# tiborcamargo/KinectPy

Measured on AMD Instinct MI355X. Metric: Mpoints/sec end-to-end (unproject+filter+ICP), 4-sensor frame, higher is better.
Workload: dtype f64 decisions / f32 storage

## Files before the change

### include/kinectpx.h

```cpp
#ifndef KINECTPX_H
#define KINECTPX_H

#include <stddef.h>
#include <stdint.h>

#ifdef __cplusplus
extern "C" {
#endif

#define KPX_VERSION 100

typedef enum {
    KPX_OK = 0,
    KPX_ERR_INVALID = -1,
    KPX_ERR_WORKSPACE = -2,
    KPX_ERR_RANGE = -3,
    KPX_ERR_HIP = -4,
    KPX_RETRY = 1
} kpx_status;

const char *kpx_last_error(void);
int kpx_version(void);


int kpx_unproject_u16(const uint16_t *depth, const float *xy_table, int64_t n_px, int32_t frames,
                      int16_t *xyz, void *stream);

size_t kpx_median_workspace_bytes(int32_t frames);
int kpx_median_i16(const int16_t *v, int64_t n, int64_t stride, int32_t frames, double *d_median,
                   void *ws, size_t ws_bytes, void *stream);

#define KPX_COMPACT_COLOR_MASK 1
#define KPX_COMPACT_DEPTH_GATE 2
size_t kpx_compact_workspace_bytes(int64_t n, int32_t frames);
int kpx_rgbd_compact(const int16_t *xyz, const uint8_t *rgb, int64_t n, int32_t frames, int32_t flags,
                     const double *d_median, double gate, float *pts, float *col, int32_t *idx,
                     int32_t *d_count, void *ws, size_t ws_bytes, void *stream);

size_t kpx_depth_to_cloud_workspace_bytes(int64_t n_px, int32_t frames);
int kpx_depth_to_cloud(const uint16_t *depth, const float *xy_table, const uint8_t *rgb, int64_t n_px,
                       int32_t frames, int32_t flags, double gate, float *pts, float *col, int32_t *idx,
                       int32_t *d_count, void *ws, size_t ws_bytes, void *stream);


int kpx_transform(const float *pts, int64_t n, const double *h_T, float *out, void *stream);
int kpx_rotate(const float *nrm, int64_t n, const double *h_T, float *out, void *stream);
int kpx_joints_affine_f64(const double *x, int64_t rows, const double *h_A, const double *h_t, double *out,
                          void *stream);

#define KPX_SELECT_GATHER 0
#define KPX_SELECT_INVERT 1
#define KPX_SELECT_MASK 2
size_t kpx_select_workspace_bytes(int64_t n);
int kpx_select_by_index(const float *a0, const float *a1, const float *a2, int64_t n, const int32_t *idx,
                        int64_t n_idx, int32_t invert, float *o0, float *o1, float *o2, int32_t *d_count,
                        void *ws, size_t ws_bytes, void *stream);

int kpx_select_by_index_bounds(const float *a0, const float *a1, const float *a2, int64_t n, const int32_t *idx, int64_t n_idx,
                               float *o0, float *o1, float *o2, double *d_bbox6, void *ws, size_t ws_bytes, void *stream);
size_t kpx_bounds_workspace_bytes(void);
int kpx_bounds(const float *pts, int64_t n, double *d_bbox6, void *ws, size_t ws_bytes, void *stream);

size_t kpx_sort_pairs_u32_workspace_bytes(int64_t n);
int kpx_sort_pairs_u32(const uint32_t *keys_in, const int32_t *vals_in, int64_t n, int32_t end_bit, uint32_t *keys_out,
                       int32_t *vals_out, void *ws, size_t ws_bytes, void *stream);

int kpx_halfspace_select(const float *pts, int64_t n, const double *h_plane, int32_t *idx, int32_t *d_count,
                         void *ws, size_t ws_bytes, void *stream);
int kpx_slab_split(const float *pts, int64_t n, double slab, int32_t *lower_idx, int32_t *d_lower,
                   int32_t *upper_idx, int32_t *d_upper, void *ws, size_t ws_bytes, void *stream);
int kpx_slab_split_bounded(const float *pts, int64_t n, double slab, const double *d_bbox6, int32_t *lower_idx, int32_t *d_lower,
                           int32_t *upper_idx, int32_t *d_upper, void *ws, size_t ws_bytes, void *stream);


size_t kpx_voxel_workspace_bytes(int64_t n);
int kpx_voxel_downsample(const float *pts, const float *col, const float *nrm, int64_t n, double voxel,
                         float *opts, float *ocol, float *onrm, int32_t *d_count, void *ws, size_t ws_bytes,
                         void *stream);

size_t kpx_voxel_batch_workspace_bytes(int32_t count, const int64_t *h_n);
int kpx_voxel_downsample_batch(int32_t count, const float *const *h_pts, const float *const *h_col, const int64_t *h_n,
                               double voxel, float *const *h_opts, float *const *h_ocol, int32_t *d_counts, void *ws,
                               size_t ws_bytes, void *stream);

size_t kpx_fuse_voxel_workspace_bytes(int64_t total_points);
int kpx_fuse_voxel_downsample(int32_t count, const float *const *h_pts, const float *const *h_col, const int64_t *h_n,
                              const double *h_T, double voxel, float *opts, float *ocol, int32_t *d_count, void *ws,
                              size_t ws_bytes, void *stream);

#define KPX_SOR_MAX_K 4096
#define KPX_SOR_LDS_K 288
size_t kpx_sor_workspace_bytes(int64_t n, int32_t nb_neighbors);
int kpx_sor(const float *pts, int64_t n, int32_t nb_neighbors, double std_ratio, int32_t *keep_idx,
            int32_t *d_count, double *d_stats, double *d_avg, void *ws, size_t ws_bytes, void *stream);

int kpx_sor_select(const float *pts, const float *attr, int64_t n, int32_t nb_neighbors, double std_ratio, float *out_pts,
                   float *out_attr, int32_t *keep_idx, int32_t *d_count, double *d_stats, void *ws, size_t ws_bytes, void *stream);

int kpx_sor_partial(const float *pts, int64_t n, int32_t nb_neighbors, int64_t q_begin, int64_t q_end, double *d_avg_sorted,
                    int32_t *d_order, void *ws, size_t ws_bytes, void *stream);
size_t kpx_sor_finish_workspace_bytes(int64_t n);
int kpx_sor_finish(const double *d_avg_sorted, const int32_t *d_order, int64_t n, double std_ratio, int32_t *keep_idx,
                   int32_t *d_count, double *d_stats, double *d_avg, void *ws, size_t ws_bytes, void *stream);

size_t kpx_dbscan_workspace_bytes(int64_t n);
int kpx_cluster_dbscan(const float *pts, int64_t n, double eps, int32_t min_points, int32_t *labels ,
                       int32_t *d_nclusters, void *ws, size_t ws_bytes, void *stream);

size_t kpx_radius_outlier_workspace_bytes(int64_t n);
int kpx_remove_radius_outlier(const float *pts, int64_t n, int32_t nb_points, double radius, int32_t *keep_idx,
                              int32_t *d_count, void *ws, size_t ws_bytes, void *stream);

size_t kpx_iss_workspace_bytes(int64_t n);
int kpx_iss_saliency(const float *pts, int64_t n, double salient_radius, double gamma_21, double gamma_32, int32_t min_neighbors,
                     double *saliency , void *ws, size_t ws_bytes, void *stream);
int kpx_iss_nonmax(const float *pts, int64_t n, const double *saliency , double non_max_radius, int32_t min_neighbors,
                   int32_t *keep_idx, int32_t *d_count, void *ws, size_t ws_bytes, void *stream);
int kpx_iss_keypoints(const float *pts, int64_t n, double salient_radius, double non_max_radius, double gamma_21, double gamma_32,
                      int32_t min_neighbors, double *saliency , int32_t *keep_idx, int32_t *d_count, void *ws, size_t ws_bytes,
                      void *stream);
int kpx_mean_nn_distance(const double *d2, const int32_t *count, int64_t m, int32_t stride, double *d_mean, void *ws, size_t ws_bytes,
                         void *stream);

#define KPX_FPS_BLOCK_THREADS 1024
#define KPX_FPS_REG_N 12288
#define KPX_FPS_LDS_N 19456
#define KPX_FPS_BLOCK_MAX_N 24576
#define KPX_FPS_BATCH_BLOCK_MAX_N 65536
#define KPX_FPS_BATCH_MIN_CLOUDS 4
size_t kpx_fps_workspace_bytes(int32_t count, int64_t n_max);
int kpx_farthest_point_sample(const float *pts, int64_t n, int32_t k, int32_t start_index, int32_t *sel ,
                              double *cover , void *ws, size_t ws_bytes, void *stream);
int kpx_farthest_point_sample_batch(int32_t count, const float *const *h_pts, const int64_t *h_n, int32_t k, int32_t start_index,
                                    int32_t *const *h_sel, double *const *h_cover, void *ws, size_t ws_bytes, void *stream);

#define KPX_NORMALS_MAX_NN 4096
#define KPX_NORMALS_LDS_NN 128
size_t kpx_normals_workspace_bytes(int64_t n, int32_t max_nn);
int kpx_estimate_normals(const float *pts, int64_t n, double radius, int32_t max_nn, float *normals,
                         void *ws, size_t ws_bytes, void *stream);
size_t kpx_covariances_workspace_bytes(int64_t n, int32_t max_nn);
int kpx_estimate_covariances(const float *pts, int64_t n, double radius, int32_t max_nn, double *cov,
                             void *ws, size_t ws_bytes, void *stream);

size_t kpx_search_index_bytes(int64_t n);
int kpx_search_index_build(const float *pts, int64_t n, void *index, size_t index_bytes, void *ws, size_t ws_bytes, void *stream);
size_t kpx_search_workspace_bytes(int64_t m, int32_t k);
int kpx_search_knn(const void *index, size_t index_bytes, const float *queries, int64_t m, int32_t k, double radius, int32_t *idx ,
                   double *d2 , int32_t *count , void *ws, size_t ws_bytes, void *stream);
int kpx_search_radius_count(const void *index, size_t index_bytes, const float *queries, int64_t m, double radius, int64_t *offsets ,
                            void *ws, size_t ws_bytes, void *stream);
int kpx_search_radius_fill(const void *index, size_t index_bytes, const float *queries, int64_t m, double radius, const int64_t *offsets,
                           int64_t total, int32_t *idx , double *d2 , void *ws, size_t ws_bytes, void *stream);

size_t kpx_segment_plane_workspace_bytes(int64_t n, int32_t ransac_n, int32_t num_iterations);
int kpx_segment_plane(const float *pts, int64_t n, double distance_threshold, int32_t ransac_n,
                      int32_t num_iterations, double probability, uint64_t seed, double *d_plane,
                      int32_t *inlier_idx, int32_t *d_count, void *ws, size_t ws_bytes, void *stream);


size_t kpx_nn_workspace_bytes(int64_t n_src, int64_t n_tgt);
int kpx_nn_search(const float *src, int64_t n_src, const float *tgt, int64_t n_tgt, const double *d_T,
                  int32_t *idx, double *d2, void *ws, size_t ws_bytes, void *stream);

size_t kpx_registration_eval_workspace_bytes(int64_t n_src, int64_t n_tgt);
int kpx_registration_eval(const float *src, int64_t n_src, const float *tgt, int64_t n_tgt, const double *d_T,
                          double max_dist, double *d_result, int32_t *idx, double *d2, void *ws, size_t ws_bytes,
                          void *stream);

size_t kpx_kabsch_workspace_bytes(int64_t n_corr);
int kpx_kabsch(const float *src, const float *tgt, const int32_t *corr, int64_t n_corr, double *d_T, void *ws,
               size_t ws_bytes, void *stream);

#define KPX_ICP_POINT_TO_POINT 0
#define KPX_ICP_POINT_TO_PLANE 1
#define KPX_ICP_FIXED 2
size_t kpx_icp_workspace_bytes(int64_t n_src, int64_t n_tgt);
int kpx_icp(const float *src, int64_t n_src, const float *tgt, const float *tgt_normals, int64_t n_tgt,
            double max_dist, const double *h_init, int32_t mode, int32_t max_iteration, double relative_fitness,
            double relative_rmse, int32_t poll_interval, double *d_result, int32_t *idx, double *d2, void *ws,
            size_t ws_bytes, void *stream);


size_t kpx_fpfh_workspace_bytes(int64_t n, int32_t max_nn);
int kpx_fpfh(const float *pts, const float *normals, int64_t n, double radius, int32_t max_nn, double *fpfh, void *ws,
             size_t ws_bytes, void *stream);

size_t kpx_feature_nn_workspace_bytes(int64_t na, int64_t nb);
int kpx_feature_nn(const double *fa, int64_t na, const double *fb, int64_t nb, int32_t *idx, void *ws, size_t ws_bytes,
                   void *stream);

size_t kpx_ransac_workspace_bytes(int64_t n_src, int64_t n_tgt);
int kpx_ransac_corres(const float *src, int64_t n_src, const float *tgt, int64_t n_tgt, const int32_t *corres, int64_t n_corres,
                      double max_dist, int32_t ransac_n, double edge_similarity, int32_t max_iteration, double confidence,
                      uint64_t seed, double *h_result, void *ws, size_t ws_bytes, void *stream);

size_t kpx_fgr_workspace_bytes(int64_t n_corres);
int kpx_fgr_tuple_test(const float *src, int64_t n_src, const float *tgt, int64_t n_tgt, const int32_t *corres, int64_t n_corres,
                       double tuple_scale, int32_t maximum_tuple_count, uint64_t seed, int32_t *d_pairs, int32_t *d_count,
                       void *ws, size_t ws_bytes, void *stream);
int kpx_fgr_optimize(const float *src, int64_t n_src, const float *tgt, int64_t n_tgt, const int32_t *corres, int64_t n_corres,
                     double division_factor, int32_t use_absolute_scale, int32_t decrease_mu, double maximum_correspondence_distance,
                     int32_t iteration_number, double *h_result, void *ws, size_t ws_bytes, void *stream);

size_t kpx_icp_batch_workspace_bytes(int32_t count, const int64_t *h_n_src, int64_t n_tgt);
int kpx_icp_batch(int32_t count, const float *const *h_src, const int64_t *h_n_src, const float *tgt,
                  const float *tgt_normals, int64_t n_tgt, double max_dist, const double *h_init, int32_t mode,
                  int32_t max_iteration, double relative_fitness, double relative_rmse, double *d_results, void *ws,
                  size_t ws_bytes, void *stream);

#define KPX_NN_ENGINE_CULLED 0
#define KPX_NN_ENGINE_DENSE 1
#define KPX_NN_ENGINE_DENSE_FP64 2
int kpx_nn_engine(int32_t engine);

size_t kpx_sample_workspace_bytes(int64_t n);
int kpx_sample_points(const float *pts, int64_t n, int64_t k, uint64_t seed, float *out_pts, int32_t *out_idx, void *ws,
                      size_t ws_bytes, void *stream);

size_t kpx_obb_workspace_bytes(int32_t count, int64_t n);
int kpx_obb_batch(const void *pts, int32_t pts_f64, int32_t count, int64_t n, double *d_obb, uint8_t *d_is_vertex, void *ws,
                  size_t ws_bytes, void *stream);

#define KPX_NORM_OBB 0
#define KPX_NORM_OBB_ROT_TRANS 1
#define KPX_NORM_TRANSLATE 2
#define KPX_NORM_OBB_ROT 3
int kpx_normalize_batch(const double *x, int32_t count, int64_t rows, const double *d_obb, int32_t mode, const double *h_M,
                        double *out, void *stream);

size_t kpx_color_gradient_workspace_bytes(int64_t n, int32_t max_nn);
int kpx_color_gradient(const float *pts, const float *normals, const float *colors, int64_t n, double radius, int32_t max_nn,
                       double *grad, void *ws, size_t ws_bytes, void *stream);
size_t kpx_colored_icp_workspace_bytes(int64_t n_src, int64_t n_tgt);
int kpx_colored_icp(const float *src, const float *src_colors, int64_t n_src, const float *tgt, const float *tgt_colors,
                    const float *tgt_normals, const double *tgt_gradient, int64_t n_tgt, double max_dist, const double *h_init,
                    double lambda_geometric, int32_t max_iteration, double relative_fitness, double relative_rmse,
                    int32_t poll_interval, double *d_result, void *ws, size_t ws_bytes, void *stream);

int kpx_gicp_covariances(const float *normals, int64_t n, double epsilon, double *cov, void *stream);
int kpx_rotate_covariances(const double *cov, int64_t n, const double *h_T, double *out, void *stream);
size_t kpx_generalized_icp_workspace_bytes(int64_t n_src, int64_t n_tgt);
int kpx_generalized_icp(const float *src, const double *src_cov, int64_t n_src, const float *tgt, const double *tgt_cov, int64_t n_tgt,
                        double max_dist, const double *h_init, int32_t max_iteration, double relative_fitness, double relative_rmse,
                        int32_t poll_interval, double *d_result, int32_t *idx, double *d2, void *ws, size_t ws_bytes, void *stream);

#define KPX_LOSS_L2 0
#define KPX_LOSS_L1 1
#define KPX_LOSS_HUBER 2
#define KPX_LOSS_CAUCHY 3
#define KPX_LOSS_GM 4
#define KPX_LOSS_TUKEY 5
int kpx_icp_robust(const float *src, int64_t n_src, const float *tgt, const float *tgt_normals, int64_t n_tgt,
                   double max_dist, const double *h_init, int32_t mode, int32_t max_iteration, double relative_fitness,
                   double relative_rmse, int32_t poll_interval, double *d_result, int32_t *idx, double *d2, void *ws,
                   size_t ws_bytes, void *stream, int32_t loss, double loss_k);
int kpx_colored_icp_robust(const float *src, const float *src_colors, int64_t n_src, const float *tgt, const float *tgt_colors,
                           const float *tgt_normals, const double *tgt_gradient, int64_t n_tgt, double max_dist, const double *h_init,
                           double lambda_geometric, int32_t max_iteration, double relative_fitness, double relative_rmse,
                           int32_t poll_interval, double *d_result, void *ws, size_t ws_bytes, void *stream, int32_t loss,
                           double loss_k);
int kpx_generalized_icp_robust(const float *src, const double *src_cov, int64_t n_src, const float *tgt, const double *tgt_cov,
                               int64_t n_tgt, double max_dist, const double *h_init, int32_t max_iteration, double relative_fitness,
                               double relative_rmse, int32_t poll_interval, double *d_result, int32_t *idx, double *d2, void *ws,
                               size_t ws_bytes, void *stream, int32_t loss, double loss_k);

int kpx_fuse_skeletons(const double *skeletons, int32_t cams, int64_t frames, int32_t joints, double alpha, double beta,
                       int32_t initial_frame, double *out, void *stream);

typedef struct {
    double reg_voxel;
    double icp_max_dist;
    double filt_voxel;
    double filt_ratio;
    double gate;
    int32_t normals_nn;
    int32_t icp_mode;
    int32_t icp_max_iteration;
    int32_t filt_k;
} kpx_frame_params;
size_t kpx_frame_step_workspace_bytes(int32_t sensors, int64_t n_px);
int kpx_frame_step(const uint16_t *depth, const uint8_t *rgb, const float *xy_table, int64_t n_px, int32_t sensors,
                   const double *h_init, const kpx_frame_params *params, float *out_pts, float *out_col, int32_t *h_count,
                   double *h_T, int32_t *h_info, void *ws, size_t ws_bytes, void *stream);
size_t kpx_frame_step_host_workspace_bytes(int32_t sensors, int64_t n_px);
int kpx_frame_step_host(const uint16_t *h_depth, const uint8_t *h_rgb, const float *xy_table, int64_t n_px, int32_t sensors,
                        const double *h_init, const kpx_frame_params *params, float *out_pts, float *out_col, int32_t *h_count,
                        double *h_T, int32_t *h_info, void *ws, size_t ws_bytes, void *stream);

typedef struct kpx_comm kpx_comm;
typedef int (*kpx_bcast_fn)(void *user, void *d_buf, size_t bytes, int32_t root, void *stream);
typedef int (*kpx_allgather_fn)(void *user, const void *d_send, void *d_recv, size_t bytes_per_rank, void *stream);
int kpx_rccl_load(const char *path);
int kpx_rccl_unique_id(void *id128);
int kpx_comm_create_rccl(const void *id128, int32_t rank, int32_t world, kpx_comm **out);
int kpx_comm_create_callbacks(int32_t rank, int32_t world, kpx_bcast_fn bcast, kpx_allgather_fn allgather, void *user, kpx_comm **out);
int kpx_comm_create_replay(int32_t rank, int32_t world, int32_t frames, int32_t first_frame, int32_t stride, int32_t per_frame,
                           const void *const *d_payloads, const size_t *bytes, kpx_comm **out);
int kpx_comm_destroy(kpx_comm *comm);
int kpx_comm_rank(const kpx_comm *comm);
int kpx_comm_world(const kpx_comm *comm);
int kpx_comm_broadcast(kpx_comm *comm, void *d_buf, size_t bytes, int32_t root, void *stream);
int kpx_comm_allgather(kpx_comm *comm, const void *d_send, void *d_recv, size_t bytes_per_rank, void *stream);
int kpx_copy_bytes(void *dst, const void *src, size_t bytes, void *stream, int32_t wait);

typedef struct kpx_order kpx_order;
int kpx_order_create(int32_t depth, kpx_order **out);
int kpx_order_destroy(kpx_order *order);
int kpx_order_submit(kpx_order *order, int64_t *frame);
int kpx_order_block(kpx_order *order, int64_t frame);
int kpx_order_turn_begin(kpx_order *order, int64_t frame, int32_t stage);
int kpx_order_turn_end(kpx_order *order, int64_t frame, int32_t stage);
int kpx_order_skip(kpx_order *order, int64_t frame, int32_t stage);
int kpx_order_finish(kpx_order *order, int64_t frame);
int kpx_order_log(kpx_order *order, int64_t *out, int64_t cap, int64_t *count);

size_t kpx_frame_step_sharded_workspace_bytes(int32_t sensors, int32_t rank, int32_t world, int64_t n_px, int32_t host_input);
int kpx_frame_step_sharded(kpx_comm *comm, kpx_order *order, int64_t frame, const uint16_t *depth, const uint8_t *rgb, int32_t host_input,
                           const float *xy_table, int64_t n_px, int32_t sensors, const double *h_init, const kpx_frame_params *params,
                           int32_t fused_filter, float *out_pts, float *out_col, int32_t *h_count, double *h_T, int32_t *h_info, void *ws,
                           size_t ws_bytes, void *stream);

typedef struct kpx_stream kpx_stream;
size_t kpx_stream_workspace_bytes(int32_t sensors, int32_t rank, int32_t world, int64_t n_px, int32_t depth);
int kpx_stream_create(const float *xy_table, int64_t n_px, int32_t sensors, const double *h_init, const kpx_frame_params *params,
                      int32_t depth, kpx_comm *const *comms, int32_t fused_filter, void *ws, size_t ws_bytes, kpx_stream **out);
int kpx_stream_submit(kpx_stream *stream, const void *depth, const void *rgb, int32_t host_input, float *out_pts, float *out_col);
int kpx_stream_pop(kpx_stream *stream, int32_t *h_count, double *h_T, int32_t *h_info);
int kpx_stream_pending(const kpx_stream *stream);
int kpx_stream_capacity(const kpx_stream *stream);
int kpx_stream_destroy(kpx_stream *stream);
int kpx_stream_stats(const kpx_stream *stream, uint64_t *h_out4);

int kpx_host_resources(uint64_t *h_out4);

#define KPX_PROF_NN_MFMA 0
#define KPX_PROF_SOR_KNN 1
#define KPX_PROF_PLANE_SCORE 2
#define KPX_PROF_COMPACT 3
#define KPX_PROF_NN_SCREEN 4
#define KPX_PROF_NN_LOCAL 5
#define KPX_PROF_KERNELS 6
int kpx_prof_begin(int32_t capacity);
int kpx_prof_stride(int32_t stride);
int kpx_prof_end(double *h_ms, int64_t *h_launches, double *h_work);
int kpx_prof_icp_phases(double *h_out8);
int kpx_prof_icp_waves(uint64_t *h_out, int64_t cap_waves, int64_t *h_count);
int kpx_icp_chain(int32_t on);
int kpx_prof_icp_cert(uint64_t *h_out8);
int kpx_prof_icp_chain(uint64_t *h_out3072);

#define KPX_TSDF_MAX_RESOLUTION 1024
#define KPX_TSDF_MAX_SENSORS 8
#define KPX_TSDF_COUNT_BLOCK 512
#define KPX_TSDF_SURFACE 0
#define KPX_TSDF_VOXELS 1
size_t kpx_tsdf_workspace_bytes(int32_t resolution);
int kpx_tsdf_integrate(float *volume, float *color, int32_t resolution, double voxel_length, const double *h_origin, double sdf_trunc,
                       int32_t count, const void *const *h_depth, int32_t depth_u16, double depth_scale, double depth_trunc,
                       const uint8_t *const *h_rgb, int32_t width, int32_t height, const double *h_intrinsic, const double *h_extrinsics,
                       void *stream);
int kpx_tsdf_extract_count(const float *volume, int32_t resolution, int32_t mode, int64_t *d_count, void *ws, size_t ws_bytes, void *stream);
int kpx_tsdf_extract_fill(const float *volume, const float *color, int32_t resolution, double voxel_length, const double *h_origin,
                          int32_t mode, int64_t total, float *pts, float *nrm, float *col, void *ws, size_t ws_bytes, void *stream);

#define KPX_TSDF_BLOCKS_MAX_RESOLUTION 32
size_t kpx_tsdf_blocks_touch_workspace_bytes(int32_t count, int32_t width, int32_t height, int32_t stride, double unit_length, double sdf_trunc);
int kpx_tsdf_blocks_touch(const int64_t *index_keys, const int32_t *index_slots, int64_t n_blocks, int32_t count, const void *const *h_depth,
                          int32_t depth_u16, double depth_scale, double depth_trunc, int32_t width, int32_t height, const double *h_intrinsic,
                          const double *h_poses, int32_t stride, double unit_length, double sdf_trunc, int64_t *d_counts, void *ws,
                          size_t ws_bytes, void *stream);
int kpx_tsdf_blocks_insert(const int64_t *index_keys, const int32_t *index_slots, int64_t n_blocks, int64_t n_new, int64_t *out_keys,
                           int32_t *out_slots, float *pool, float *color_pool, int64_t capacity, int32_t unit_resolution, int32_t count,
                           int32_t width, int32_t height, int32_t stride, double unit_length, double sdf_trunc, const void *ws, size_t ws_bytes,
                           void *stream);
int kpx_tsdf_blocks_integrate(float *pool, float *color_pool, int64_t capacity, int32_t unit_resolution, double voxel_length, double sdf_trunc,
                              int64_t n_touched, int32_t count, const void *const *h_depth, int32_t depth_u16, double depth_scale,
                              double depth_trunc, const uint8_t *const *h_rgb, int32_t width, int32_t height, const double *h_intrinsic,
                              const double *h_extrinsics, int32_t stride, const void *ws, size_t ws_bytes, void *stream);
size_t kpx_tsdf_blocks_extract_workspace_bytes(int64_t n_blocks, int32_t unit_resolution, int32_t mesh);
int kpx_tsdf_blocks_extract_count(const int64_t *index_keys, const int32_t *index_slots, int64_t n_blocks, const float *pool,
                                  int32_t unit_resolution, int32_t mode, int64_t *d_count, void *ws, size_t ws_bytes, void *stream);
int kpx_tsdf_blocks_extract_fill(const int64_t *index_keys, const int32_t *index_slots, int64_t n_blocks, const float *pool,
                                 const float *color_pool, int32_t unit_resolution, double voxel_length, int32_t mode, int64_t total, float *pts,
                                 float *nrm, float *col, void *ws, size_t ws_bytes, void *stream);
int kpx_tsdf_blocks_mesh_count(const int64_t *index_keys, const int32_t *index_slots, int64_t n_blocks, const float *pool,
                               int32_t unit_resolution, int64_t *d_counts, void *ws, size_t ws_bytes, void *stream);
int kpx_tsdf_blocks_mesh_fill(const int64_t *index_keys, const int32_t *index_slots, int64_t n_blocks, const float *pool,
                              const float *color_pool, int32_t unit_resolution, double voxel_length, int64_t n_vertices, int64_t n_triangles,
                              float *out_vertices, float *out_colors, int32_t *out_triangles, void *ws, size_t ws_bytes, void *stream);

size_t kpx_tsdf_mesh_workspace_bytes(int32_t resolution);
int kpx_tsdf_mesh_count(const float *volume, int32_t resolution, int64_t *d_counts, void *ws, size_t ws_bytes, void *stream);
int kpx_tsdf_mesh_fill(const float *volume, const float *color, int32_t resolution, double voxel_length, const double *h_origin,
                       int64_t n_vertices, int64_t n_triangles, float *out_vertices, float *out_colors, int32_t *out_triangles, void *ws,
                       size_t ws_bytes, void *stream);
size_t kpx_mesh_normals_workspace_bytes(int64_t n_vertices, int64_t n_triangles);
int kpx_mesh_normals(const float *vertices, int64_t n_vertices, const int32_t *triangles, int64_t n_triangles, int32_t normalized,
                     float *out_triangle_normals, float *out_vertex_normals, void *ws, size_t ws_bytes, void *stream);
int kpx_mesh_surface_area(const float *vertices, int64_t n_vertices, const int32_t *triangles, int64_t n_triangles, double *d_area, void *stream);

#define KPX_MESH_FLAG_REFERENCED 0
#define KPX_MESH_FLAG_DEGENERATE 1
#define KPX_MESH_FLAG_INDICES 2
#define KPX_MESH_SMOOTH_SIMPLE 0
#define KPX_MESH_SMOOTH_LAPLACIAN 1
#define KPX_MESH_SMOOTH_TAUBIN 2
size_t kpx_mesh_adjacency_workspace_bytes(int64_t n_vertices, int64_t n_triangles);
int kpx_mesh_adjacency(const int32_t *triangles, int64_t n_vertices, int64_t n_triangles, int32_t *out_offsets, int32_t *out_neighbours,
                       int32_t *d_count, void *ws, size_t ws_bytes, void *stream);
size_t kpx_mesh_edges_workspace_bytes(int64_t n_vertices, int64_t n_triangles);
int kpx_mesh_non_manifold_edges(const int32_t *triangles, int64_t n_vertices, int64_t n_triangles, int32_t allow_boundary_edges,
                                int32_t *out_edges, int32_t *d_count, void *ws, size_t ws_bytes, void *stream);
size_t kpx_mesh_cluster_workspace_bytes(int64_t n_vertices, int64_t n_triangles);
int kpx_mesh_cluster_triangles(const float *vertices, int64_t n_vertices, const int32_t *triangles, int64_t n_triangles, int32_t *out_clusters,
                               int32_t *out_n_triangles, double *out_area, int32_t *d_count, void *ws, size_t ws_bytes, void *stream);
int kpx_mesh_flags(int32_t kind, const int32_t *triangles, int64_t n_vertices, int64_t n_triangles, const int64_t *indices, int64_t n_indices,
                   uint8_t *out_flags, int64_t n_flags, void *stream);
size_t kpx_mesh_select_workspace_bytes(int64_t n_vertices, int64_t n_triangles);
int kpx_mesh_select_triangles(const int32_t *triangles, const float *triangle_normals, int64_t n_triangles, const uint8_t *flags, int32_t invert,
                              int32_t *out_triangles, float *out_triangle_normals, int32_t *d_count, void *ws, size_t ws_bytes, void *stream);
int kpx_mesh_select_vertices(const float *vertices, const float *colors, const float *normals, int64_t n_vertices, const int32_t *triangles,
                             const float *triangle_normals, int64_t n_triangles, const uint8_t *flags, int32_t invert, float *out_vertices,
                             float *out_colors, float *out_normals, int32_t *out_triangles, float *out_triangle_normals, int32_t *d_counts, void *ws,
                             size_t ws_bytes, void *stream);
size_t kpx_mesh_smooth_workspace_bytes(int64_t n_vertices);
int kpx_mesh_smooth(const float *vertices, const float *normals, const float *colors, int64_t n_vertices, const int32_t *offsets,
                    const int32_t *neighbours, int64_t n_neighbours, int32_t method, int32_t iterations, double lambda_filter, double mu,
                    float *out_vertices, float *out_normals, float *out_colors, void *ws, size_t ws_bytes, void *stream);
size_t kpx_mesh_sample_workspace_bytes(int64_t n_triangles);
int kpx_mesh_sample_points(const float *vertices, const float *colors, const float *vertex_normals, const float *triangle_normals,
                           int64_t n_vertices, const int32_t *triangles, int64_t n_triangles, int64_t n_points, uint64_t seed, float *out_points,
                           float *out_colors, float *out_normals, double *d_total, void *ws, size_t ws_bytes, void *stream);

#define KPX_RAYSCENE_LEAF 4
#define KPX_RAYSCENE_FANOUT 4
#define KPX_RAY_CAST 0
#define KPX_RAY_OCCLUDED 1
#define KPX_RAY_COUNT 2
size_t kpx_rayscene_bytes(int64_t n_triangles);
size_t kpx_rayscene_workspace_bytes(int64_t n_triangles);
int kpx_rayscene_build(const float *vertices, int64_t n_vertices, const int32_t *triangles, int64_t n_triangles, const int32_t *triangle_ids,
                       void *scene, size_t scene_bytes, void *ws, size_t ws_bytes, void *stream);
int kpx_rayscene_rays(const void *scene, size_t scene_bytes, const float *rays, int64_t m, int32_t mode, double tnear, double tfar, int32_t brute,
                      double *out_t, float *out_t_hit, float *out_uvs, float *out_normals, int32_t *out_geometry_ids, int32_t *out_primitive_ids,
                      int32_t *out_count, void *stream);
// ... 126 lines not shown
```

### kinectpy_amd/_lib.py

```python
import ctypes as C
import threading
import weakref
import os

import torch

_HERE = os.path.dirname(os.path.abspath(__file__))
SO_PATH = os.environ.get("KPX_LIBRARY") or os.path.join(_HERE, "libkinectpx.so")

_i64, _i32, _f64, _u64, _vp, _sz = C.c_int64, C.c_int32, C.c_double, C.c_uint64, C.c_void_p, C.c_size_t

SIGNATURES = {
    "kpx_last_error": (C.c_char_p, []),
    "kpx_version": (C.c_int, []),
    "kpx_unproject_u16": (C.c_int, [_vp, _vp, _i64, _i32, _vp, _vp]),
    "kpx_median_workspace_bytes": (_sz, [_i32]),
    "kpx_median_i16": (C.c_int, [_vp, _i64, _i64, _i32, _vp, _vp, _sz, _vp]),
    "kpx_compact_workspace_bytes": (_sz, [_i64, _i32]),
    "kpx_rgbd_compact": (C.c_int, [_vp, _vp, _i64, _i32, _i32, _vp, _f64, _vp, _vp, _vp, _vp, _vp, _sz, _vp]),
    "kpx_depth_to_cloud_workspace_bytes": (_sz, [_i64, _i32]),
    "kpx_depth_to_cloud": (C.c_int, [_vp, _vp, _vp, _i64, _i32, _i32, _f64, _vp, _vp, _vp, _vp, _vp, _sz, _vp]),
    "kpx_transform": (C.c_int, [_vp, _i64, _vp, _vp, _vp]),
    "kpx_rotate": (C.c_int, [_vp, _i64, _vp, _vp, _vp]),
    "kpx_joints_affine_f64": (C.c_int, [_vp, _i64, _vp, _vp, _vp, _vp]),
    "kpx_select_workspace_bytes": (_sz, [_i64]),
    "kpx_select_by_index": (C.c_int, [_vp, _vp, _vp, _i64, _vp, _i64, _i32, _vp, _vp, _vp, _vp, _vp, _sz, _vp]),
    "kpx_halfspace_select": (C.c_int, [_vp, _i64, _vp, _vp, _vp, _vp, _sz, _vp]),
    "kpx_slab_split": (C.c_int, [_vp, _i64, _f64, _vp, _vp, _vp, _vp, _vp, _sz, _vp]),
    "kpx_slab_split_bounded": (C.c_int, [_vp, _i64, _f64, _vp, _vp, _vp, _vp, _vp, _vp, _sz, _vp]),
    "kpx_select_by_index_bounds": (C.c_int, [_vp, _vp, _vp, _i64, _vp, _i64, _vp, _vp, _vp, _vp, _vp, _sz, _vp]),
    "kpx_bounds_workspace_bytes": (C.c_size_t, []),
    "kpx_bounds": (C.c_int, [_vp, _i64, _vp, _vp, _sz, _vp]),
    "kpx_voxel_workspace_bytes": (_sz, [_i64]),
    "kpx_voxel_downsample": (C.c_int, [_vp, _vp, _vp, _i64, _f64, _vp, _vp, _vp, _vp, _vp, _sz, _vp]),
    "kpx_voxel_batch_workspace_bytes": (_sz, [_i32, _vp]),
    "kpx_voxel_downsample_batch": (C.c_int, [_i32, _vp, _vp, _vp, _f64, _vp, _vp, _vp, _vp, _sz, _vp]),
    "kpx_fuse_voxel_workspace_bytes": (_sz, [_i64]),
    "kpx_fuse_voxel_downsample": (C.c_int, [_i32, _vp, _vp, _vp, _vp, _f64, _vp, _vp, _vp, _vp, _sz, _vp]),
    "kpx_sor_workspace_bytes": (_sz, [_i64, _i32]),
    "kpx_sor": (C.c_int, [_vp, _i64, _i32, _f64, _vp, _vp, _vp, _vp, _vp, _sz, _vp]),
    "kpx_sor_partial": (C.c_int, [_vp, _i64, _i32, _i64, _i64, _vp, _vp, _vp, _sz, _vp]),
    "kpx_sor_finish_workspace_bytes": (_sz, [_i64]),
    "kpx_sor_finish": (C.c_int, [_vp, _vp, _i64, _f64, _vp, _vp, _vp, _vp, _vp, _sz, _vp]),
    "kpx_dbscan_workspace_bytes": (_sz, [_i64]),
    "kpx_cluster_dbscan": (C.c_int, [_vp, _i64, _f64, _i32, _vp, _vp, _vp, _sz, _vp]),
    "kpx_radius_outlier_workspace_bytes": (_sz, [_i64]),
    "kpx_remove_radius_outlier": (C.c_int, [_vp, _i64, _i32, _f64, _vp, _vp, _vp, _sz, _vp]),
    "kpx_iss_workspace_bytes": (_sz, [_i64]),
    "kpx_iss_saliency": (C.c_int, [_vp, _i64, _f64, _f64, _f64, _i32, _vp, _vp, _sz, _vp]),
    "kpx_iss_nonmax": (C.c_int, [_vp, _i64, _vp, _f64, _i32, _vp, _vp, _vp, _sz, _vp]),
    "kpx_iss_keypoints": (C.c_int, [_vp, _i64, _f64, _f64, _f64, _f64, _i32, _vp, _vp, _vp, _vp, _sz, _vp]),
    "kpx_mean_nn_distance": (C.c_int, [_vp, _vp, _i64, _i32, _vp, _vp, _sz, _vp]),
    "kpx_fps_workspace_bytes": (_sz, [_i32, _i64]),
    "kpx_farthest_point_sample": (C.c_int, [_vp, _i64, _i32, _i32, _vp, _vp, _vp, _sz, _vp]),
    "kpx_farthest_point_sample_batch": (C.c_int, [_i32, _vp, _vp, _i32, _i32, _vp, _vp, _vp, _sz, _vp]),
    "kpx_normals_workspace_bytes": (_sz, [_i64, _i32]),
    "kpx_estimate_normals": (C.c_int, [_vp, _i64, _f64, _i32, _vp, _vp, _sz, _vp]),
    "kpx_search_index_bytes": (_sz, [_i64]),
    "kpx_search_index_build": (C.c_int, [_vp, _i64, _vp, _sz, _vp, _sz, _vp]),
    "kpx_search_workspace_bytes": (_sz, [_i64, _i32]),
    "kpx_search_knn": (C.c_int, [_vp, _sz, _vp, _i64, _i32, _f64, _vp, _vp, _vp, _vp, _sz, _vp]),
    "kpx_search_radius_count": (C.c_int, [_vp, _sz, _vp, _i64, _f64, _vp, _vp, _sz, _vp]),
    "kpx_search_radius_fill": (C.c_int, [_vp, _sz, _vp, _i64, _f64, _vp, _i64, _vp, _vp, _vp, _sz, _vp]),
    "kpx_segment_plane_workspace_bytes": (_sz, [_i64, _i32, _i32]),
    "kpx_segment_plane": (C.c_int, [_vp, _i64, _f64, _i32, _i32, _f64, _u64, _vp, _vp, _vp, _vp, _sz, _vp]),
    "kpx_nn_workspace_bytes": (_sz, [_i64, _i64]),
    "kpx_nn_search": (C.c_int, [_vp, _i64, _vp, _i64, _vp, _vp, _vp, _vp, _sz, _vp]),
    "kpx_registration_eval_workspace_bytes": (_sz, [_i64, _i64]),
    "kpx_registration_eval": (C.c_int, [_vp, _i64, _vp, _i64, _vp, _f64, _vp, _vp, _vp, _vp, _sz, _vp]),
    "kpx_kabsch_workspace_bytes": (_sz, [_i64]),
    "kpx_kabsch": (C.c_int, [_vp, _vp, _vp, _i64, _vp, _vp, _sz, _vp]),
    "kpx_icp_workspace_bytes": (_sz, [_i64, _i64]),
    "kpx_icp": (C.c_int, [_vp, _i64, _vp, _vp, _i64, _f64, _vp, _i32, _i32, _f64, _f64, _i32, _vp, _vp, _vp, _vp, _sz, _vp]),
    "kpx_fpfh_workspace_bytes": (_sz, [_i64, _i32]),
    "kpx_fpfh": (C.c_int, [_vp, _vp, _i64, _f64, _i32, _vp, _vp, _sz, _vp]),
    "kpx_feature_nn_workspace_bytes": (_sz, [_i64, _i64]),
    "kpx_feature_nn": (C.c_int, [_vp, _i64, _vp, _i64, _vp, _vp, _sz, _vp]),
    "kpx_ransac_workspace_bytes": (_sz, [_i64, _i64]),
    "kpx_ransac_corres": (C.c_int, [_vp, _i64, _vp, _i64, _vp, _i64, _f64, _i32, _f64, _i32, _f64, _u64, _vp, _vp, _sz, _vp]),
    "kpx_fgr_workspace_bytes": (_sz, [_i64]),
    "kpx_fgr_tuple_test": (C.c_int, [_vp, _i64, _vp, _i64, _vp, _i64, _f64, _i32, _u64, _vp, _vp, _vp, _sz, _vp]),
    "kpx_fgr_optimize": (C.c_int, [_vp, _i64, _vp, _i64, _vp, _i64, _f64, _i32, _i32, _f64, _i32, _vp, _vp, _sz, _vp]),
    "kpx_sample_workspace_bytes": (_sz, [_i64]),
    "kpx_sample_points": (C.c_int, [_vp, _i64, _i64, _u64, _vp, _vp, _vp, _sz, _vp]),
    "kpx_obb_workspace_bytes": (_sz, [_i32, _i64]),
    "kpx_obb_batch": (C.c_int, [_vp, _i32, _i32, _i64, _vp, _vp, _vp, _sz, _vp]),
    "kpx_normalize_batch": (C.c_int, [_vp, _i32, _i64, _vp, _i32, _vp, _vp, _vp]),
    "kpx_color_gradient_workspace_bytes": (_sz, [_i64, _i32]),
    "kpx_color_gradient": (C.c_int, [_vp, _vp, _vp, _i64, _f64, _i32, _vp, _vp, _sz, _vp]),
    "kpx_colored_icp_workspace_bytes": (_sz, [_i64, _i64]),
    "kpx_colored_icp": (C.c_int, [_vp, _vp, _i64, _vp, _vp, _vp, _vp, _i64, _f64, _vp, _f64, _i32, _f64, _f64, _i32, _vp, _vp, _sz, _vp]),
    "kpx_covariances_workspace_bytes": (_sz, [_i64, _i32]),
    "kpx_estimate_covariances": (C.c_int, [_vp, _i64, _f64, _i32, _vp, _vp, _sz, _vp]),
    "kpx_gicp_covariances": (C.c_int, [_vp, _i64, _f64, _vp, _vp]),
    "kpx_rotate_covariances": (C.c_int, [_vp, _i64, _vp, _vp, _vp]),
    "kpx_generalized_icp_workspace_bytes": (_sz, [_i64, _i64]),
    "kpx_generalized_icp": (C.c_int, [_vp, _vp, _i64, _vp, _vp, _i64, _f64, _vp, _i32, _f64, _f64, _i32, _vp, _vp, _vp, _vp, _sz, _vp]),
    "kpx_icp_robust": (C.c_int, [_vp, _i64, _vp, _vp, _i64, _f64, _vp, _i32, _i32, _f64, _f64, _i32, _vp, _vp, _vp, _vp, _sz, _vp, _i32, _f64]),
    "kpx_colored_icp_robust": (C.c_int, [_vp, _vp, _i64, _vp, _vp, _vp, _vp, _i64, _f64, _vp, _f64, _i32, _f64, _f64, _i32, _vp, _vp, _sz, _vp,
                                         _i32, _f64]),
    "kpx_generalized_icp_robust": (C.c_int, [_vp, _vp, _i64, _vp, _vp, _i64, _f64, _vp, _i32, _f64, _f64, _i32, _vp, _vp, _vp, _vp, _sz, _vp,
                                             _i32, _f64]),
    "kpx_fuse_skeletons": (C.c_int, [_vp, _i32, _i64, _i32, _f64, _f64, _i32, _vp, _vp]),
    "kpx_nn_engine": (C.c_int, [_i32]),
    "kpx_icp_batch_workspace_bytes": (_sz, [_i32, _vp, _i64]),
    "kpx_icp_batch": (C.c_int, [_i32, _vp, _vp, _vp, _vp, _i64, _f64, _vp, _i32, _i32, _f64, _f64, _vp, _vp, _sz, _vp]),
    "kpx_prof_begin": (C.c_int, [_i32]),
    "kpx_prof_stride": (C.c_int, [_i32]),
    "kpx_frame_step_workspace_bytes": (_sz, [_i32, _i64]),
    "kpx_frame_step": (C.c_int, [_vp, _vp, _vp, _i64, _i32, _vp, _vp, _vp, _vp, _vp, _vp, _vp, _vp, _sz, _vp]),
    "kpx_frame_step_host_workspace_bytes": (_sz, [_i32, _i64]),
    "kpx_frame_step_host": (C.c_int, [_vp, _vp, _vp, _i64, _i32, _vp, _vp, _vp, _vp, _vp, _vp, _vp, _vp, _sz, _vp]),
    "kpx_rccl_load": (C.c_int, [_vp]),
    "kpx_rccl_unique_id": (C.c_int, [_vp]),
    "kpx_comm_create_rccl": (C.c_int, [_vp, _i32, _i32, _vp]),
    "kpx_comm_create_callbacks": (C.c_int, [_i32, _i32, _vp, _vp, _vp, _vp]),
    "kpx_comm_create_replay": (C.c_int, [_i32, _i32, _i32, _i32, _i32, _i32, _vp, _vp, _vp]),
    "kpx_comm_destroy": (C.c_int, [_vp]),
    "kpx_comm_rank": (C.c_int, [_vp]),
    "kpx_comm_world": (C.c_int, [_vp]),
    "kpx_comm_broadcast": (C.c_int, [_vp, _vp, _sz, _i32, _vp]),
    "kpx_comm_allgather": (C.c_int, [_vp, _vp, _vp, _sz, _vp]),
    "kpx_copy_bytes": (C.c_int, [_vp, _vp, _sz, _vp, _i32]),
    "kpx_order_create": (C.c_int, [_i32, _vp]),
    "kpx_order_destroy": (C.c_int, [_vp]),
    "kpx_order_submit": (C.c_int, [_vp, _vp]),
    "kpx_order_block": (C.c_int, [_vp, _i64]),
    "kpx_order_turn_begin": (C.c_int, [_vp, _i64, _i32]),
    "kpx_order_turn_end": (C.c_int, [_vp, _i64, _i32]),
    "kpx_order_skip": (C.c_int, [_vp, _i64, _i32]),
    "kpx_order_finish": (C.c_int, [_vp, _i64]),
    "kpx_order_log": (C.c_int, [_vp, _vp, _i64, _vp]),
    "kpx_frame_step_sharded_workspace_bytes": (_sz, [_i32, _i32, _i32, _i64, _i32]),
    "kpx_frame_step_sharded": (C.c_int, [_vp, _vp, _i64, _vp, _vp, _i32, _vp, _i64, _i32, _vp, _vp, _i32, _vp, _vp, _vp, _vp, _vp, _vp, _sz, _vp]),
    "kpx_stream_workspace_bytes": (_sz, [_i32, _i32, _i32, _i64, _i32]),
    "kpx_stream_create": (C.c_int, [_vp, _i64, _i32, _vp, _vp, _i32, _vp, _i32, _vp, _sz, _vp]),
    "kpx_stream_submit": (C.c_int, [_vp, _vp, _vp, _i32, _vp, _vp]),
    "kpx_stream_pop": (C.c_int, [_vp, _vp, _vp, _vp]),
    "kpx_stream_pending": (C.c_int, [_vp]),
    "kpx_stream_capacity": (C.c_int, [_vp]),
    "kpx_stream_destroy": (C.c_int, [_vp]),
    "kpx_stream_stats": (C.c_int, [_vp, _vp]),
    "kpx_host_resources": (C.c_int, [_vp]),
    "kpx_sor_select": (C.c_int, [_vp, _vp, C.c_int64, C.c_int32, C.c_double, _vp, _vp, _vp, _vp, _vp, _vp, C.c_size_t, _vp]),
    "kpx_sort_pairs_u32_workspace_bytes": (C.c_size_t, [C.c_int64]),
    "kpx_sort_pairs_u32": (C.c_int, [_vp, _vp, C.c_int64, C.c_int32, _vp, _vp, _vp, C.c_size_t, _vp]),
    "kpx_prof_icp_phases": (C.c_int, [_vp]),
    "kpx_prof_icp_waves": (C.c_int, [_vp, C.c_int64, _vp]),
    "kpx_icp_chain": (C.c_int, [C.c_int32]),
    "kpx_prof_icp_cert": (C.c_int, [_vp]),
    "kpx_prof_icp_chain": (C.c_int, [_vp]),
    "kpx_prof_end": (C.c_int, [_vp, _vp, _vp]),
    "kpx_tsdf_workspace_bytes": (_sz, [_i32]),
    "kpx_tsdf_integrate": (C.c_int, [_vp, _vp, _i32, _f64, _vp, _f64, _i32, _vp, _i32, _f64, _f64, _vp, _i32, _i32, _vp, _vp, _vp]),
    "kpx_tsdf_extract_count": (C.c_int, [_vp, _i32, _i32, _vp, _vp, _sz, _vp]),
    "kpx_tsdf_extract_fill": (C.c_int, [_vp, _vp, _i32, _f64, _vp, _i32, _i64, _vp, _vp, _vp, _vp, _sz, _vp]),
    "kpx_tsdf_mesh_workspace_bytes": (_sz, [_i32]),
    "kpx_tsdf_mesh_count": (C.c_int, [_vp, _i32, _vp, _vp, _sz, _vp]),
    "kpx_tsdf_mesh_fill": (C.c_int, [_vp, _vp, _i32, _f64, _vp, _i64, _i64, _vp, _vp, _vp, _vp, _sz, _vp]),
    "kpx_tsdf_blocks_touch_workspace_bytes": (_sz, [_i32, _i32, _i32, _i32, _f64, _f64]),
    "kpx_tsdf_blocks_touch": (C.c_int, [_vp, _vp, _i64, _i32, _vp, _i32, _f64, _f64, _i32, _i32, _vp, _vp, _i32, _f64, _f64, _vp, _vp, _sz, _vp]),
    "kpx_tsdf_blocks_insert": (C.c_int, [_vp, _vp, _i64, _i64, _vp, _vp, _vp, _vp, _i64, _i32, _i32, _i32, _i32, _i32, _f64, _f64, _vp, _sz, _vp]),
    "kpx_tsdf_blocks_integrate": (C.c_int, [_vp, _vp, _i64, _i32, _f64, _f64, _i64, _i32, _vp, _i32, _f64, _f64, _vp, _i32, _i32, _vp, _vp, _i32, _vp, _sz,
                                            _vp]),
    "kpx_tsdf_blocks_extract_workspace_bytes": (_sz, [_i64, _i32, _i32]),
    "kpx_tsdf_blocks_extract_count": (C.c_int, [_vp, _vp, _i64, _vp, _i32, _i32, _vp, _vp, _sz, _vp]),
    "kpx_tsdf_blocks_extract_fill": (C.c_int, [_vp, _vp, _i64, _vp, _vp, _i32, _f64, _i32, _i64, _vp, _vp, _vp, _vp, _sz, _vp]),
    "kpx_tsdf_blocks_mesh_count": (C.c_int, [_vp, _vp, _i64, _vp, _i32, _vp, _vp, _sz, _vp]),
    "kpx_tsdf_blocks_mesh_fill": (C.c_int, [_vp, _vp, _i64, _vp, _vp, _i32, _f64, _i64, _i64, _vp, _vp, _vp, _vp, _sz, _vp]),
    "kpx_mesh_normals_workspace_bytes": (_sz, [_i64, _i64]),
    "kpx_mesh_normals": (C.c_int, [_vp, _i64, _vp, _i64, _i32, _vp, _vp, _vp, _sz, _vp]),
    "kpx_mesh_surface_area": (C.c_int, [_vp, _i64, _vp, _i64, _vp, _vp]),
    "kpx_mesh_adjacency_workspace_bytes": (_sz, [_i64, _i64]),
    "kpx_mesh_adjacency": (C.c_int, [_vp, _i64, _i64, _vp, _vp, _vp, _vp, _sz, _vp]),
    "kpx_mesh_edges_workspace_bytes": (_sz, [_i64, _i64]),
    "kpx_mesh_non_manifold_edges": (C.c_int, [_vp, _i64, _i64, _i32, _vp, _vp, _vp, _sz, _vp]),
    "kpx_mesh_cluster_workspace_bytes": (_sz, [_i64, _i64]),
    "kpx_mesh_cluster_triangles": (C.c_int, [_vp, _i64, _vp, _i64, _vp, _vp, _vp, _vp, _vp, _sz, _vp]),
    "kpx_mesh_flags": (C.c_int, [_i32, _vp, _i64, _i64, _vp, _i64, _vp, _i64, _vp]),
    "kpx_mesh_select_workspace_bytes": (_sz, [_i64, _i64]),
    "kpx_mesh_select_triangles": (C.c_int, [_vp, _vp, _i64, _vp, _i32, _vp, _vp, _vp, _vp, _sz, _vp]),
    "kpx_mesh_select_vertices": (C.c_int, [_vp, _vp, _vp, _i64, _vp, _vp, _i64, _vp, _i32, _vp, _vp, _vp, _vp, _vp, _vp, _vp, _sz, _vp]),
    "kpx_mesh_smooth_workspace_bytes": (_sz, [_i64]),
    "kpx_mesh_smooth": (C.c_int, [_vp, _vp, _vp, _i64, _vp, _vp, _i64, _i32, _i32, _f64, _f64, _vp, _vp, _vp, _vp, _sz, _vp]),
    "kpx_mesh_sample_workspace_bytes": (_sz, [_i64]),
    "kpx_mesh_sample_points": (C.c_int, [_vp, _vp, _vp, _vp, _i64, _vp, _i64, _i64, _u64, _vp, _vp, _vp, _vp, _vp, _sz, _vp]),
    "kpx_rayscene_bytes": (_sz, [_i64]),
    "kpx_rayscene_workspace_bytes": (_sz, [_i64]),
    "kpx_rayscene_build": (C.c_int, [_vp, _i64, _vp, _i64, _vp, _vp, _sz, _vp, _sz, _vp]),
    "kpx_rayscene_rays": (C.c_int, [_vp, _sz, _vp, _i64, _i32, _f64, _f64, _i32, _vp, _vp, _vp, _vp, _vp, _vp, _vp, _vp]),
    "kpx_rayscene_closest": (C.c_int, [_vp, _sz, _vp, _i64, _i32, _vp, _vp, _vp, _vp, _vp, _vp]),
    "kpx_mesh_links_workspace_bytes": (_sz, [_i64, _i64]),
    "kpx_mesh_non_manifold_vertices": (C.c_int, [_vp, _i64, _i64, _vp, _vp, _vp, _sz, _vp]),
    "kpx_mesh_orientation_workspace_bytes": (_sz, [_i64, _i64]),
    "kpx_mesh_orientation": (C.c_int, [_vp, _i64, _i64, _vp, _vp, _vp, _vp, _vp, _sz, _vp]),
    "kpx_mesh_volume_workspace_bytes": (_sz, [_i64]),
    "kpx_mesh_volume": (C.c_int, [_vp, _i64, _vp, _i64, _vp, _vp, _sz, _vp]),
    "kpx_mesh_edge_count": (C.c_int, [_vp, _i64, _i64, _vp, _vp, _sz, _vp]),
    "kpx_rayscene_triangle_pairs_count": (C.c_int, [_vp, _sz, _vp, _i64, _vp, _i64, _i32, _i32, _i32, _vp, _vp, _vp]),
    "kpx_rayscene_triangle_pairs_workspace_bytes": (_sz, [_i64]),
    "kpx_rayscene_triangle_pairs_fill": (C.c_int, [_vp, _sz, _vp, _i64, _vp, _i64, _i32, _i32, _vp, _i64, _vp, _vp, _sz, _vp]),
    "kpx_voxelgrid_from_cloud_workspace_bytes": (_sz, [_i64]),
    "kpx_voxelgrid_from_cloud": (C.c_int, [_vp, _vp, _i64, _f64, _vp, _vp, _vp, _vp, _vp, _vp, _sz, _vp]),
    "kpx_voxelgrid_dense": (C.c_int, [_i32, _i32, _i32, _vp, _vp, _vp, _vp]),
    "kpx_voxelgrid_carve_workspace_bytes": (_sz, [_i64]),
    "kpx_voxelgrid_carve": (C.c_int, [_vp, _vp, _i64, _vp, _f64, _i32, _i32, _vp, _i32, _f64, _f64, _i32, _i32, _vp, _vp, _i32, _i32, _vp, _vp, _vp,
                                      _vp, _sz, _vp]),
    "kpx_voxelgrid_included": (C.c_int, [_vp, _i32, _i64, _vp, _i64, _vp, _f64, _vp, _vp]),
    "kpx_image_workspace_bytes": (_sz, [_i32, _i32, _i32]),
    "kpx_image_filter": (C.c_int, [_vp, _vp, _i32, _i32, _i32, _i32, _vp, _sz, _vp]),
    "kpx_image_downsample": (C.c_int, [_vp, _vp, _i32, _i32, _i32, _vp]),
    "kpx_odometry_workspace_bytes": (_sz, [_i32, _i32, _i32, _i32]),
    "kpx_odometry_correspondence": (C.c_int, [_vp, _vp, _i32, _i32, _vp, _vp, _f64, _vp, _vp, _vp, _sz, _vp]),
    "kpx_rgbd_odometry": (C.c_int, [_i32, _vp, _vp, _vp, _vp, _i32, _vp, _vp, _f64, _f64, _i32, _i32, _vp, _vp, _i32, _i32, _vp, _f64, _f64, _f64,
                                    _vp, _vp, _sz, _vp]),
    "kpx_odometry_iteration": (C.c_int, [_vp, _vp, _vp, _vp, _vp, _vp, _vp, _vp, _i32, _i32, _vp, _vp, _i32, _f64, _vp, _vp, _sz, _vp]),
    "kpx_orient_normals": (C.c_int, [_vp, _vp, _i64, _i32, _vp, _vp]),
    "kpx_emst_workspace_bytes": (_sz, [_i64, _i32]),
    "kpx_emst": (C.c_int, [_vp, _i64, _i32, _vp, _vp, _vp, _sz, _vp]),
    "kpx_orient_normals_tangent_workspace_bytes": (_sz, [_i64, _i32]),
    "kpx_orient_normals_tangent": (C.c_int, [_vp, _vp, _i64, _i32, _vp, _vp, _vp, _vp, _sz, _vp]),
    "kpx_pointnet_workspace_bytes": (_sz, [_i32, _i64, _i32]),
    "kpx_pointnet_forward": (C.c_int, [_vp, _i64, _vp, _i32, _i64, _i32, _vp, _vp, _vp, _vp, _vp, _vp, _vp, _sz, _vp]),
    "kpx_joint_metrics": (C.c_int, [_vp, _vp, _i64, _vp, _i32, _vp, _vp, _vp]),
    "kpx_pointnet_train_floats": (C.c_int, [_i32, _vp, _vp]),
    "kpx_pointnet_train_workspace_bytes": (_sz, [_i32, _i64, _i32]),
    "kpx_pointnet_grad": (C.c_int, [_vp, _i64, _vp, _vp, _i32, _i64, _i32, _u64, _u64, _i32, _vp, _vp] + [_vp] * 9 + [_vp, _sz, _vp]),
    "kpx_adam_step": (C.c_int, [_vp, _vp, _vp, _vp, _i64, _f64, _f64, _f64, _f64, _i64, _vp]),
    "kpx_pointnet_train_step": (C.c_int, [_vp, _i64, _vp, _vp, _i32, _i64, _i32, _u64, _u64, _i32, _vp, _vp, _vp, _vp, _f64, _f64, _f64, _f64, _i64,
                                          _vp, _sz, _vp]),
    "kpx_xy_table": (C.c_int, [_vp, _i32, _i32, _vp, _vp]),
    "kpx_color_to_depth": (C.c_int, [_vp, _vp, _vp, _i64, _i32, _i32, _i32, _i32, _vp, _i32, _i32, _vp, _vp]),
    "kpx_depth_to_color_workspace_bytes": (_sz, [_i32, _i32, _i32]),
    "kpx_depth_to_color": (C.c_int, [_vp, _vp, _i32, _i32, _i32, _i32, _i32, _vp, _i32, _f64, _vp, _vp, _sz, _vp]),
    "kpx_color_to_depth_visible": (C.c_int, [_vp, _vp, _vp, _i64, _i32, _i32, _i32, _i32, _vp, _i32, _i32, _vp, _f64, _vp, _vp]),
    "kpx_undistort_map": (C.c_int, [_vp, _vp, _i32, _i32, _vp, _vp]),
    "kpx_remap_u8": (C.c_int, [_vp, _vp, _i32, _i32, _i32, _i32, _i32, _i32, _i32, _i32, _vp, _vp]),
    "kpx_remap_depth": (C.c_int, [_vp, _vp, _i32, _i32, _i32, _i32, _i32, _i32, _i32, _f64, _vp, _vp]),
}

_lib = None


class KinectPxError(RuntimeError):
    pass


def load():
    global _lib
    if _lib is None:
        if not os.path.exists(SO_PATH):
            raise KinectPxError(
                f"{SO_PATH} is missing: build it with `python -c 'import __graft_entry__ as g; g.build()'` "
                "(make -C kinectpy_amd/csrc).  There is no CPU fallback.")
        lib = C.CDLL(SO_PATH)
        for name, (res, args) in SIGNATURES.items():
            fn = getattr(lib, name)
            fn.restype, fn.argtypes = res, args
        _lib = lib
    return _lib


BCAST_FN = C.CFUNCTYPE(C.c_int, C.c_void_p, C.c_void_p, C.c_size_t, C.c_int32, C.c_void_p)
ALLGATHER_FN = C.CFUNCTYPE(C.c_int, C.c_void_p, C.c_void_p, C.c_void_p, C.c_size_t, C.c_void_p)
RETRY = 1


def check(rc):
    if rc != 0:
        msg = load().kpx_last_error().decode() or f"kpx error {rc}"
        raise KinectPxError(msg)


_gpu_checked = False


def device():
    global _gpu_checked
    if not _gpu_checked:
        if not torch.cuda.is_available():
            raise KinectPxError("no ROCm device visible: the kinectpx hot path runs on MI355X only (no CPU fallback)")
        torch.cuda.current_device()
        _gpu_checked = True
    return torch.device("cuda", torch._C._cuda_getDevice())


def _raw_stream():
    device()
    return torch._C._cuda_getCurrentRawStream(torch._C._cuda_getDevice())


def stream_ptr():
    return C.c_void_p(_raw_stream())


def ptr(t):
    if t is None:
        return None
    assert t.is_cuda and t.is_contiguous(), "kinectpx needs contiguous device tensors"
    return C.c_void_p(t.data_ptr())


def hptr(a):
    return a.ctypes.data_as(C.c_void_p)


class Workspace:

    def __init__(self):
        self.buf = None

    def get(self, nbytes):
        nbytes = int(nbytes)
        if self.buf is None or self.buf.numel() < nbytes:
            self.buf = torch.empty(max(nbytes, 1 << 20), dtype=torch.uint8, device=device())
        return C.c_void_p(self.buf.data_ptr()), C.c_size_t(self.buf.numel())


_ws = {}
_ws_lock = threading.Lock()


def workspace(nbytes):
    stream = _raw_stream()
    key = (torch._C._cuda_getDevice(), stream, threading.get_ident() if not stream else 0)
    with _ws_lock:
        ws = _ws.get(key)
        if ws is None:
            ws = _ws[key] = Workspace()
            if not stream:
                token = getattr(_tls, "token", None)
                if token is None:
                    token = _tls.token = _ThreadToken()
                weakref.finalize(token, _drop_key, key)
        return ws.get(nbytes)


class _ThreadToken:
    """lives in a thread's local storage; collected when the thread ends"""


_tls = threading.local()


def _drop_key(key):
    with _ws_lock:
        _ws.pop(key, None)


def release_workspace(stream_handle, dev=None):
    with _ws_lock:
        _ws.pop((torch._C._cuda_getDevice() if dev is None else dev, int(stream_handle), 0), None)
```

### kinectpy_amd/csrc/kpx_common.h

```cpp
#pragma once
#include <stdlib.h>
#include <functional>
#include <hip/hip_runtime.h>
#include <stdint.h>
#include <stdio.h>
#include <string.h>

#include "../../include/kinectpx.h"

#define KPX_EXPORT extern "C" __attribute__((visibility("default")))

namespace kpx {

extern thread_local char g_err[512];
int fail(int code, const char *fmt, ...);

#define KPX_HIP(call)                                                                              \
    do {                                                                                           \
        hipError_t e__ = (call);                                                                   \
        if (e__ != hipSuccess)                                                                     \
            return kpx::fail(KPX_ERR_HIP, "%s failed: %s (%s:%d)", #call, hipGetErrorString(e__),  \
                             __FILE__, __LINE__);                                                  \
    } while (0)
#define KPX_LAUNCH_CHECK() KPX_HIP(hipGetLastError())
#define KPX_REQUIRE(cond, ...)                                                                     \
    do {                                                                                           \
        if (!(cond)) return kpx::fail(KPX_ERR_INVALID, __VA_ARGS__);                               \
    } while (0)

struct Arena {
    char *base;
    size_t off, cap;
    bool dry;
    explicit Arena(void *p, size_t bytes) : base((char *)p), off(0), cap(bytes), dry(p == nullptr) {}
    template <class T> T *get(size_t count)
    {
        size_t bytes = (count * sizeof(T) + 255) & ~(size_t)255;
        T *r = dry ? nullptr : (T *)(base + off);
        off += bytes;
        return r;
    }
    bool ok() const { return dry || off <= cap; }
};
#define KPX_ARENA_CHECK(a)                                                                         \
    do {                                                                                           \
        if (!(a).ok())                                                                             \
            return kpx::fail(KPX_ERR_WORKSPACE, "workspace too small: need %zu bytes, have %zu",   \
                             (a).off, (a).cap);                                                    \
    } while (0)

static inline int64_t cdiv(int64_t a, int64_t b) { return (a + b - 1) / b; }

constexpr unsigned kMemoSort = 0x4000u, kMemoGridScan = 0x8000u;
size_t memo_bytes(unsigned what, int64_t n, const std::function<size_t()> &query);

typedef unsigned int kpx_u4 __attribute__((ext_vector_type(4)));
template <class V> __device__ __forceinline__ V stream_load16(const V *p)
{
    static_assert(sizeof(V) == 16, "16-byte vectors only");
#ifdef KPX_STREAM_PLAIN
    return *p;
#else
    const kpx_u4 r = __builtin_nontemporal_load(reinterpret_cast<const kpx_u4 *>(p));
    V v;
    __builtin_memcpy(&v, &r, 16);
    return v;
#endif
}
template <class V> __device__ __forceinline__ void stream_store16(const V &v, V *p)
{
    static_assert(sizeof(V) == 16, "16-byte vectors only");
#ifdef KPX_STREAM_PLAIN
    *p = v;
#else
    kpx_u4 r;
    __builtin_memcpy(&r, &v, 16);
    __builtin_nontemporal_store(r, reinterpret_cast<kpx_u4 *>(p));
#endif
}
#define KPX_STREAM_LOAD(p) stream_load16(p)
#define KPX_STREAM_STORE(v, p) stream_store16((v), (p))

bool prof_armed();
struct ProfScope {
    int slot;
    hipStream_t st;
    ProfScope(int kernel_id, double work, hipStream_t stream);
    ~ProfScope();
};

constexpr int kWave = 64;

__device__ __forceinline__ int lane_id() { return threadIdx.x & 63; }
__device__ __forceinline__ int wave_id() { return threadIdx.x >> 6; }

template <class T> __device__ __forceinline__ T wave_sum(T v)
{
#pragma unroll
    for (int o = 32; o > 0; o >>= 1) v += __shfl_down(v, o, 64);
    return v;
}
template <class T> __device__ __forceinline__ T wave_min(T v)
{
#pragma unroll
    for (int o = 32; o > 0; o >>= 1) { T t = __shfl_down(v, o, 64); v = t < v ? t : v; }
    return v;
}
template <class T> __device__ __forceinline__ T wave_max(T v)
{
#pragma unroll
    for (int o = 32; o > 0; o >>= 1) { T t = __shfl_down(v, o, 64); v = t > v ? t : v; }
    return v;
}

__device__ __forceinline__ void wave_lds_fence()
{
    __builtin_amdgcn_fence(__ATOMIC_SEQ_CST, "wavefront");
    __builtin_amdgcn_wave_barrier();
}

__device__ __forceinline__ void philox4x32_10(uint32_t c0, uint32_t c1, uint32_t c2, uint32_t c3, uint32_t k0, uint32_t k1, uint32_t out[4])
{
#pragma unroll
    for (int r = 0; r < 10; ++r) {
        uint64_t p0 = (uint64_t)0xD2511F53u * c0;
        uint64_t p1 = (uint64_t)0xCD9E8D57u * c2;
        uint32_t n0 = (uint32_t)(p1 >> 32) ^ c1 ^ k0;
        uint32_t n1 = (uint32_t)p1;
        uint32_t n2 = (uint32_t)(p0 >> 32) ^ c3 ^ k1;
        uint32_t n3 = (uint32_t)p0;
        c0 = n0; c1 = n1; c2 = n2; c3 = n3;
        k0 += 0x9E3779B9u; k1 += 0xBB67AE85u;
    }
    out[0] = c0; out[1] = c1; out[2] = c2; out[3] = c3;
}

template <class T> __device__ __forceinline__ T block_sum(T v, T *sh)
{
    v = wave_sum(v);
    __syncthreads();
    if (lane_id() == 0) sh[wave_id()] = v;
    __syncthreads();
    T r = T(0);
    if (threadIdx.x == 0) {
        int nw = (blockDim.x + 63) >> 6;
        for (int w = 0; w < nw; ++w) r += sh[w];
    }
    return r;
}

__device__ __forceinline__ int wave_incl_scan(int v)
{
    int l = lane_id();
#pragma unroll
    for (int o = 1; o < 64; o <<= 1) { int t = __shfl_up(v, o, 64); if (l >= o) v += t; }
    return v;
}
__device__ __forceinline__ int block_excl_scan(int v, int *sh, int *total)
{
    int incl = wave_incl_scan(v);
    int nw = (blockDim.x + 63) >> 6;
    __syncthreads();
    if (lane_id() == 63) sh[wave_id()] = incl;
    __syncthreads();
    if (threadIdx.x == 0) {
        int run = 0;
        for (int w = 0; w < nw; ++w) { int t = sh[w]; sh[w] = run; run += t; }
        sh[nw] = run;
    }
    __syncthreads();
    int base = sh[wave_id()];
    *total = sh[nw];
    return base + incl - v;
}

}
```

### kinectpy_amd/csrc/kpx_gridknn.h

```cpp
#pragma once
#include <initializer_list>

#include "kpx_internal.h"

namespace kpx {

__device__ __forceinline__ int cell_coord(double v, double org, double h, int dim)
{
    int c = (int)floor((v - org) / h);
    return c < 0 ? 0 : (c >= dim ? dim - 1 : c);
}

struct HeapD {
    double *h; int stride, k, sz;
    static __device__ HeapD make(double *h, int32_t *, int stride, int k) { return HeapD{ h, stride, k, 0 }; }
    __device__ bool full() const { return sz == k; }
    __device__ double worst() const { return h[0]; }
    __device__ void push(double d, int)
    {
        if (sz < k) {
            int c = sz++;
            while (c > 0) {
                int p = (c - 1) >> 1;
                double hp = h[p * stride];
                if (hp < d) { h[c * stride] = hp; c = p; } else break;
            }
            h[c * stride] = d;
        } else if (d < h[0]) {
            int c = 0;
            for (;;) {
                int l = 2 * c + 1, r = l + 1;
                if (l >= k) break;
                double hl = h[l * stride];
                int b = l; double hb = hl;
                if (r < k) { double hr = h[r * stride]; if (hr > hl) { b = r; hb = hr; } }
                if (hb > d) { h[c * stride] = hb; c = b; } else break;
            }
            h[c * stride] = d;
        }
    }
};
struct HeapDI {
    double *h; int32_t *ix; int stride, k, sz;
    static __device__ HeapDI make(double *h, int32_t *ix, int stride, int k) { return HeapDI{ h, ix, stride, k, 0 }; }
    __device__ bool full() const { return sz == k; }
    __device__ double worst() const { return h[0]; }
    static __device__ bool less(double a, int32_t ai, double b, int32_t bi) { return a < b || (a == b && ai < bi); }
    __device__ void push(double d, int j)
    {
        if (sz < k) {
            int c = sz++;
            while (c > 0) {
                int p = (c - 1) >> 1;
                double hp = h[p * stride]; int32_t ip = ix[p * stride];
                if (less(hp, ip, d, j)) { h[c * stride] = hp; ix[c * stride] = ip; c = p; } else break;
            }
            h[c * stride] = d; ix[c * stride] = j;
        } else if (less(d, j, h[0], ix[0])) {
            int c = 0;
            for (;;) {
                int l = 2 * c + 1, r = l + 1;
                if (l >= k) break;
                int b = l; double hb = h[l * stride]; int32_t ib = ix[l * stride];
                if (r < k) { double hr = h[r * stride]; int32_t ir = ix[r * stride]; if (less(hb, ib, hr, ir)) { b = r; hb = hr; ib = ir; } }
                if (less(d, j, hb, ib)) { h[c * stride] = hb; ix[c * stride] = ib; c = b; } else break;
            }
            h[c * stride] = d; ix[c * stride] = j;
        }
    }
};

template <class Heap>
__device__ __forceinline__ void grid_knn_scan(const GridParams &g, const uint32_t *__restrict__ cell_start,
                                              const float *__restrict__ spts, const int32_t *__restrict__ sidx, double qx,
                                              double qy, double qz, double r2max, Heap &heap)
{
    const double q[3] = { qx, qy, qz };
    int c[3];
#pragma unroll
    for (int a = 0; a < 3; ++a) c[a] = cell_coord(q[a], g.org[a], g.h, g.dim[a]);
    int maxr = g.dim[0] > g.dim[1] ? g.dim[0] : g.dim[1];
    if (g.dim[2] > maxr) maxr = g.dim[2];
    double gate = heap.full() ? heap.worst() : INFINITY;
    for (int r = 0; r <= maxr; ++r) {
        if (r > 0) {
            double dcov = INFINITY;
#pragma unroll
            for (int a = 0; a < 3; ++a) {
                double lo = g.org[a] + (double)(c[a] - (r - 1)) * g.h;
                double hi = g.org[a] + (double)(c[a] + r) * g.h;
                double dl = (c[a] - (r - 1) <= 0) ? INFINITY : q[a] - lo;
                double dh = (c[a] + r >= g.dim[a]) ? INFINITY : hi - q[a];
                dcov = fmin(dcov, fmin(dl, dh));
            }
            if (dcov == INFINITY) break;
            if (dcov < 0.0) dcov = 0.0;
            double cov2 = dcov * dcov * (1.0 - 1e-12);
            if (heap.full() && heap.worst() < cov2) break;
            if (r2max >= 0.0 && cov2 >= r2max) break;
        }
        const int x0 = c[0] - r, x1 = c[0] + r, y0 = c[1] - r, y1 = c[1] + r, z0 = c[2] - r, z1 = c[2] + r;
        const int xa = x0 < 0 ? 0 : x0, xb = x1 >= g.dim[0] ? g.dim[0] - 1 : x1;
        const int ya = y0 < 0 ? 0 : y0, yb = y1 >= g.dim[1] ? g.dim[1] - 1 : y1;
        const int za = z0 < 0 ? 0 : z0, zb = z1 >= g.dim[2] ? g.dim[2] - 1 : z1;
        for (int x = xa; x <= xb; ++x)
            for (int y = ya; y <= yb; ++y) {
                const bool shell_xy = (x == x0) | (x == x1) | (y == y0) | (y == y1);
                const int64_t col = ((int64_t)x * g.dim[1] + y) * g.dim[2];
                for (int part = 0; part < 2; ++part) {
                    int zs, ze;
                    if (shell_xy) { if (part) break; zs = za; ze = zb; }
                    else {
                        if (part == 0) { if (z0 < 0) continue; zs = ze = z0; }
                        else { if (z1 >= g.dim[2] || r == 0) continue; zs = ze = z1; }
                    }
                    uint32_t s0 = cell_start[col + zs], s1 = cell_start[col + ze + 1];
                    for (uint32_t sb = s0; sb < s1; sb += 8) {
                        float cx[8], cy[8], cz[8];
#pragma unroll
                        for (int e = 0; e < 8; ++e) {
                            const uint32_t s = sb + e < s1 ? sb + e : s1 - 1;
                            cx[e] = spts[3 * s]; cy[e] = spts[3 * s + 1]; cz[e] = spts[3 * s + 2];
                        }
#pragma unroll
                        for (int e = 0; e < 8; ++e) {
                            if (sb + e >= s1) break;
                            const double dx = qx - (double)cx[e], dy = qy - (double)cy[e], dz = qz - (double)cz[e];
                            const double d = fma(dz, dz, fma(dy, dy, dx * dx));
                            if (r2max >= 0.0 && !(d < r2max)) continue;
                            if (d > gate) continue;
                            heap.push(d, sidx ? sidx[sb + e] : 0);
                            gate = heap.full() ? heap.worst() : INFINITY;
                        }
                    }
                }
            }
    }
}

template <class Visit>
__device__ __forceinline__ void grid_radius_scan(const GridParams &g, const uint32_t *__restrict__ cell_start,
                                                 const float *__restrict__ spts, const double q[3], double eps, double r2, Visit &&visit)
{
    int lo[3], hi[3];
#pragma unroll
    for (int a = 0; a < 3; ++a) {
        const double e = eps * (1.0 + 1e-9) + 1e-12 * (fabs(q[a]) + fabs(g.org[a]) + g.h);
        lo[a] = cell_coord(q[a] - e, g.org[a], g.h, g.dim[a]);
        hi[a] = cell_coord(q[a] + e, g.org[a], g.h, g.dim[a]);
    }
    for (int x = lo[0]; x <= hi[0]; ++x)
        for (int y = lo[1]; y <= hi[1]; ++y) {
            const int64_t col = ((int64_t)x * g.dim[1] + y) * g.dim[2];
            const uint32_t s0 = cell_start[col + lo[2]], s1 = cell_start[col + hi[2] + 1];
            for (uint32_t s = s0; s < s1; ++s) {
                const float *p = spts + 3 * (int64_t)s;
                const double dx = q[0] - (double)p[0], dy = q[1] - (double)p[1], dz = q[2] - (double)p[2];
                const double d = fma(dz, dz, fma(dy, dy, dx * dx));
                if (d < r2 && visit(s, d)) return;
            }
        }
}

__device__ __forceinline__ unsigned long long wave_all_max_u64(unsigned long long v)
{
#pragma unroll
    for (int o = 32; o > 0; o >>= 1) { const unsigned long long t = __shfl_xor(v, o, 64); v = t > v ? t : v; }
    return v;
}
__device__ __forceinline__ double block_cover2(const GridParams &g, const double q[3], const int c[3], int r)
{
    double dcov = INFINITY;
#pragma unroll
    for (int a = 0; a < 3; ++a) {
        const double lo = g.org[a] + (double)(c[a] - r) * g.h;
        const double hi = g.org[a] + (double)(c[a] + r + 1) * g.h;
        const double dl = (c[a] - r <= 0) ? INFINITY : q[a] - lo;
        const double dh = (c[a] + r + 1 >= g.dim[a]) ? INFINITY : hi - q[a];
        dcov = fmin(dcov, fmin(dl, dh));
    }
    if (dcov == INFINITY) return INFINITY;
    if (dcov < 0.0) dcov = 0.0;
    return dcov * dcov * (1.0 - 1e-12);
}

struct WaveKnnScratch {
    double *vals;
    uint32_t *pos;
    uint32_t *run_s0;
    int32_t *run_off;
    int cap;
    uint32_t *hist;
};
constexpr int kKnnBuckets = 256;

template <class KeyF>
__device__ __forceinline__ unsigned wave_count_select(KeyF key, int m, unsigned a, unsigned range, int rank, uint32_t *__restrict__ hist, bool &exact)
{
    const int lane = threadIdx.x & 63;
    exact = false;
    while (range > 0u) {
        const int shift = range >= 256u ? 24 - __builtin_clz(range) : 0;
        uint4 *hz = reinterpret_cast<uint4 *>(hist + 4 * lane);
        hz[0] = make_uint4(0u, 0u, 0u, 0u);
        wave_lds_fence();
        for (int t = lane; t < m; t += 64) {
            unsigned kv;
            if (key(t, kv) && kv - a <= range) __hip_atomic_fetch_add(hist + ((kv - a) >> shift), 1u, __ATOMIC_RELAXED, __HIP_MEMORY_SCOPE_WORKGROUP);
        }
        wave_lds_fence();
        const uint4 t4 = hz[0];
        const int hv[4] = { (int)t4.x, (int)t4.y, (int)t4.z, (int)t4.w };
        const int lsum = hv[0] + hv[1] + hv[2] + hv[3];
        int incl = lsum;
#pragma unroll
        for (int o = 1; o < 64; o <<= 1) { const int t2 = __shfl_up(incl, o, 64); if (lane >= o) incl += t2; }
        const int excl = incl - lsum;
        const bool mine = rank > excl && rank <= incl;
        int B = -1, cb = 0, hb = 0;
        if (mine) {
            int cum = excl;
#pragma unroll
            for (int w = 0; w < 4; ++w) {
                if (B < 0 && rank <= cum + hv[w]) { B = 4 * lane + w; cb = cum; hb = hv[w]; }
                cum += hv[w];
            }
        }
        const unsigned long long bm = __builtin_amdgcn_ballot_w64(mine);
        if (bm == 0ull) return a;
        const int owner = __builtin_ctzll(bm);
        B = __shfl(B, owner, 64); cb = __shfl(cb, owner, 64); hb = __shfl(hb, owner, 64);
        const unsigned wend = a + range, bstart = a + ((unsigned)B << shift), bspan = (1u << shift) - 1u;
        const unsigned bend = wend - bstart < bspan ? wend : bstart + bspan;
        if (rank - cb == hb) { exact = true; return bend; }
        if (shift == 0) return bstart;
        rank -= cb; a = bstart; range = bend - bstart;
    }
    return a;
}
__device__ __forceinline__ unsigned wave_all_min_u32(unsigned v)
{
#pragma unroll
    for (int o = 32; o > 0; o >>= 1) { const unsigned t = (unsigned)__shfl_xor((int)v, o, 64); v = t < v ? t : v; }
    return v;
}
__device__ __forceinline__ unsigned wave_all_max_u32(unsigned v)
{
#pragma unroll
    for (int o = 32; o > 0; o >>= 1) { const unsigned t = (unsigned)__shfl_xor((int)v, o, 64); v = t > v ? t : v; }
    return v;
}
__device__ __forceinline__ int wave_all_sum_i32(int v)
{
#pragma unroll
    for (int o = 32; o > 0; o >>= 1) v += __shfl_xor(v, o, 64);
    return v;
}
__device__ __forceinline__ unsigned long long wave_kth_pattern(const double *__restrict__ vals, int m, int kk, uint32_t *__restrict__ hist)
{
    const int lane = threadIdx.x & 63;
    const uint32_t *w32 = reinterpret_cast<const uint32_t *>(vals);
    unsigned vmin = 0xFFFFFFFFu, vmax = 0u;
    int zeros = 0;
    for (int t = lane; t < m; t += 64) {
        const unsigned h = w32[2 * t + 1];
        zeros += h == 0u ? 1 : 0;
        const unsigned nz = h == 0u ? 0xFFFFFFFFu : h;
        vmin = nz < vmin ? nz : vmin; vmax = h > vmax ? h : vmax;
    }
    vmin = wave_all_min_u32(vmin); vmax = wave_all_max_u32(vmax); zeros = wave_all_sum_i32(zeros);
    unsigned P = 0u;
    bool exact = false;
    if (kk > zeros) {
        P = vmin;
        if (vmin < vmax)
            P = wave_count_select([&](int t, unsigned &kv) { kv = w32[2 * t + 1]; return kv != 0u; }, m, vmin, vmax - vmin, kk - zeros, hist, exact);
        if (exact) return ((unsigned long long)P << 32) | 0xFFFFFFFFull;
    }
    int c_less = 0, c_eq = 0;
    unsigned lmin = 0xFFFFFFFFu, lmax = 0u;
    for (int t = lane; t < m; t += 64) {
        const unsigned h = w32[2 * t + 1];
        c_less += h < P ? 1 : 0;
        if (h == P) { const unsigned l = w32[2 * t]; ++c_eq; lmin = l < lmin ? l : lmin; lmax = l > lmax ? l : lmax; }
    }
    c_less = wave_all_sum_i32(c_less); c_eq = wave_all_sum_i32(c_eq);
    const int r2 = kk - c_less;
    if (r2 >= c_eq) return ((unsigned long long)P << 32) | 0xFFFFFFFFull;
    lmin = wave_all_min_u32(lmin); lmax = wave_all_max_u32(lmax);
    unsigned Q = lmin;
    if (lmin < lmax)
        Q = wave_count_select([&](int t, unsigned &kv) { kv = w32[2 * t]; return w32[2 * t + 1] == P; }, m, lmin, lmax - lmin, r2, hist, exact);
    return ((unsigned long long)P << 32) | Q;
}
struct WaveKnnResult {
    int m;
    int kk;
    int cnt;
    unsigned long long thr;
    double top;
};
template <bool POS>
__device__ __forceinline__ bool wave_knn_select(const GridParams &g, const uint32_t *__restrict__ cell_start, const float *__restrict__ spts,
                                                const double q[3], int k, double r2max, const WaveKnnScratch &sc, WaveKnnResult &out)
{
    const int lane = threadIdx.x & 63;
    int c[3];
#pragma unroll
    for (int a = 0; a < 3; ++a) c[a] = cell_coord(q[a], g.org[a], g.h, g.dim[a]);
    int maxr = g.dim[0] > g.dim[1] ? g.dim[0] : g.dim[1];
    if (g.dim[2] > maxr) maxr = g.dim[2];
    bool truncated = false;
    auto gather_block = [&](int r, double tau) -> int {
        const int xa = c[0] - r < 0 ? 0 : c[0] - r, xb = c[0] + r >= g.dim[0] ? g.dim[0] - 1 : c[0] + r;
        const int ya = c[1] - r < 0 ? 0 : c[1] - r, yb = c[1] + r >= g.dim[1] ? g.dim[1] - 1 : c[1] + r;
        const int za = c[2] - r < 0 ? 0 : c[2] - r, zb = c[2] + r >= g.dim[2] ? g.dim[2] - 1 : c[2] + r;
        const int ny = yb - ya + 1, ncols = (xb - xa + 1) * ny;
        int m = 0;
        truncated = false;
        for (int c0 = 0; c0 < ncols && !truncated; c0 += 64) {
            const int nruns = ncols - c0 < 64 ? ncols - c0 : 64;
            uint32_t s0 = 0;
            int len = 0;
            if (lane < nruns) {
                const int x = xa + (c0 + lane) / ny, y = ya + (c0 + lane) % ny;
                const int64_t col = ((int64_t)x * g.dim[1] + y) * g.dim[2];
                s0 = cell_start[col + za];
                len = (int)(cell_start[col + zb + 1] - s0);
            }
            const int incl = wave_incl_scan(len);
            const int mc = __shfl(incl, 63, 64);
            if (mc == 0) continue;
            sc.run_s0[lane] = s0;
            sc.run_off[lane] = incl - len;
            wave_lds_fence();
            for (int t0 = 0; t0 < mc; t0 += 64) {
                const int t = t0 + lane;
                double d = INFINITY;
                uint32_t sp = 0;
                if (t < mc) {
                    int lo = 0, hi = nruns - 1;
                    while (lo < hi) {
                        const int mid = (lo + hi + 1) >> 1;
                        if (sc.run_off[mid] <= t) lo = mid; else hi = mid - 1;
                    }
                    sp = sc.run_s0[lo] + (uint32_t)(t - sc.run_off[lo]);
                    const float *pp = spts + 3 * (int64_t)sp;
                    const double dx = q[0] - (double)pp[0], dy = q[1] - (double)pp[1], dz = q[2] - (double)pp[2];
                    d = fma(dz, dz, fma(dy, dy, dx * dx));
                }
                const bool keep = t < mc && d <= tau && d < r2max;
                const unsigned long long km = __builtin_amdgcn_ballot_w64(keep);
                const int pos = m + __builtin_popcountll(km & ((1ull << lane) - 1ull));
                if (keep && pos < sc.cap) {
                    sc.vals[pos] = d;
                    if (POS) sc.pos[pos] = sp;
                }
                m += __builtin_popcountll(km);
                if (m >= sc.cap) { m = sc.cap; truncated = true; break; }
            }
            wave_lds_fence();
        }
        return m;
    };

    double tau = INFINITY;
    int r = 1;
    for (int round = 0; round <= 24; ++round) {
        const int m = gather_block(r, tau);
        wave_lds_fence();
        const double cov2 = block_cover2(g, q, c, r);
        const bool whole = cov2 == INFINITY || cov2 >= r2max;
        if (!truncated && m < k && !whole) {
            const double f = cbrt((double)(k + 1) / (double)(m > 0 ? m : 1));
            int rn = (int)((double)r * (f < 4.0 ? f : 4.0)) + 1;
            r = rn > r ? rn : r + 1;
            if (r > maxr) r = maxr;
            continue;
        }
        const int kk = m < k ? m : k;
        unsigned long long lo = 0ull;
        if (m > k) lo = wave_kth_pattern(sc.vals, m, kk, sc.hist);
        else if (m > 0) {
            for (int t = lane; t < m; t += 64) {
                const unsigned long long p = (unsigned long long)__double_as_longlong(sc.vals[t]);
                lo = p > lo ? p : lo;
            }
            lo = wave_all_max_u64(lo);
        }
        double top = 0.0;
        int cnt = 0;
        for (int t0 = 0; t0 < m; t0 += 64) {
            const int t = t0 + lane;
            const bool le = t < m && (unsigned long long)__double_as_longlong(sc.vals[t]) <= lo;
            if (le) top = fmax(top, sc.vals[t]);
            cnt += __builtin_popcountll(__builtin_amdgcn_ballot_w64(le));
        }
#pragma unroll
        for (int o = 32; o > 0; o >>= 1) top = fmax(top, __shfl_xor(top, o, 64));
        if (!truncated && (whole || top < cov2)) {
            out.m = m; out.kk = kk; out.cnt = cnt; out.thr = lo; out.top = top;
            return true;
        }
        if (truncated && top >= tau) return false;
        tau = top;
        int rn = (int)(sqrt(top) / g.h) + 1;
        if (rn > maxr) rn = maxr;
        r = rn;
        wave_lds_fence();
    }
    return false;
}


__device__ __forceinline__ int32_t wave_knn_tie_threshold(const WaveKnnScratch &sc, const WaveKnnResult &res, const int32_t *__restrict__ sidx)
{
    if (res.cnt <= res.kk) return INT_MAX;
    const int lane = threadIdx.x & 63;
    const unsigned long long topp = (unsigned long long)__double_as_longlong(res.top);
    int ntied = 0;
    for (int t0 = 0; t0 < res.m; t0 += 64) {
        const int t = t0 + lane;
        const bool tie = t < res.m && (unsigned long long)__double_as_longlong(sc.vals[t]) == topp;
        ntied += __builtin_popcountll(__builtin_amdgcn_ballot_w64(tie));
    }
    const int need = res.kk - (res.cnt - ntied);
    int32_t last = -1;
    for (int round = 0; round < need; ++round) {
        int32_t cand = INT_MAX;
        for (int t = lane; t < res.m; t += 64)
            if ((unsigned long long)__double_as_longlong(sc.vals[t]) == topp) {
                const int32_t oi = sidx[sc.pos[t]];
                if (oi > last && oi < cand) cand = oi;
            }
#pragma unroll
        for (int o = 32; o > 0; o >>= 1) { const int32_t t2 = __shfl_xor(cand, o, 64); cand = t2 < cand ? t2 : cand; }
        last = cand;
    }
    return last;
}
__device__ __forceinline__ bool wave_knn_is_selected(const WaveKnnScratch &sc, const WaveKnnResult &res, const int32_t *__restrict__ sidx,
                                                     int32_t idx_thr, int t)
{
    const unsigned long long p = (unsigned long long)__double_as_longlong(sc.vals[t]);
    const unsigned long long topp = (unsigned long long)__double_as_longlong(res.top);
    if (p > res.thr) return false;
    if (p < topp || res.cnt == res.kk) return true;
    return p == topp && sidx[sc.pos[t]] <= idx_thr;
}

template <class Op, int WAVES>
__global__ __launch_bounds__(WAVES * 64) void knn_wave_kernel(const GridParams *__restrict__ gp, const uint32_t *__restrict__ cell_start,
                                                              const float *__restrict__ spts, int64_t q0, int64_t q1, int k, int cap, Op op,
                                                              const int32_t *__restrict__ in_list, const int32_t *__restrict__ in_count,
                                                              int32_t *__restrict__ fb_list, int32_t *__restrict__ fb_count)
{
    extern __shared__ __align__(16) double lds[];
    __shared__ uint32_t run_s0[WAVES][64];
    __shared__ int32_t run_off[WAVES][64];
    __shared__ __align__(16) uint32_t knn_hist[WAVES][kKnnBuckets];
    const int wave = threadIdx.x >> 6, lane = threadIdx.x & 63;
    uint32_t *pos = nullptr;
    if constexpr (Op::kPos) pos = reinterpret_cast<uint32_t *>(lds + (size_t)WAVES * cap) + (size_t)wave * cap;
    const WaveKnnScratch sc{ lds + (size_t)wave * cap, pos, run_s0[wave], run_off[wave], cap, knn_hist[wave] };
    const GridParams g = *gp;
    const int64_t nq = in_list ? (int64_t)*in_count : q1 - q0;
    for (int64_t e = (int64_t)blockIdx.x * WAVES + wave; e < nq; e += (int64_t)gridDim.x * WAVES) {
        const int64_t s = in_list ? (int64_t)in_list[e] : q0 + e;
        const double q[3] = { (double)spts[3 * s], (double)spts[3 * s + 1], (double)spts[3 * s + 2] };
        WaveKnnResult res;
        if (!wave_knn_select<Op::kPos>(g, cell_start, spts, q, k, op.r2max(false), sc, res)) {
            if (lane == 0) { fb_list[atomicAdd(fb_count, 1)] = (int32_t)s; op.defer(s); }
            continue;
        }
        op.wave(sc, res, s, spts);
        wave_lds_fence();
    }
}
template <class Op, bool ALT>
__global__ void knn_heap_kernel(const GridParams *__restrict__ gp, const uint32_t *__restrict__ cell_start, const float *__restrict__ spts,
                                int64_t q0, int64_t q1, int k, Op op, const int32_t *__restrict__ list, const int32_t *__restrict__ list_count,
                                double *__restrict__ gheap, int32_t *__restrict__ gix)
{
    extern __shared__ __align__(16) double lds[];
    const GridParams g = *gp;
    const int64_t total = list ? (int64_t)*list_count : q1 - q0;
    int32_t *ilds = reinterpret_cast<int32_t *>(lds + (size_t)k * blockDim.x);
    const size_t gt = (size_t)blockIdx.x * blockDim.x + threadIdx.x;
    for (int64_t t = (int64_t)blockIdx.x * blockDim.x + threadIdx.x; t < total; t += (int64_t)gridDim.x * blockDim.x) {
        const int64_t s = list ? (int64_t)list[t] : q0 + t;
        typename Op::Heap heap = Op::Heap::make(gheap ? gheap + gt : lds + threadIdx.x, gheap ? gix + gt : ilds + threadIdx.x,
                                                gheap ? (int)(gridDim.x * blockDim.x) : (int)blockDim.x, k);
        grid_knn_scan(g, cell_start, spts, Op::kPos ? op.sidx : (const int32_t *)nullptr, (double)spts[3 * s], (double)spts[3 * s + 1],
                      (double)spts[3 * s + 2], op.r2max(true), heap);
        if constexpr (ALT) op.heap_alt(s, heap);
        else op.heap(s, heap);
    }
}

struct KnnHeaps {
    bool global;
    int blocks, threads;
    size_t lds;
    double *gheap;
    int32_t *gix;
};
static inline KnnHeaps knn_heaps_carve(Arena &a, int k, int lds_k, bool with_idx, int lds_threads)
{
    KnnHeaps hp{ k > lds_k, 256, lds_threads, 0, nullptr, nullptr };
    if (hp.global) {
        while (hp.blocks > 8 && (size_t)hp.blocks * 64 * (size_t)k * sizeof(double) > ((size_t)256 << 20)) hp.blocks >>= 1;
        hp.threads = 64;
        hp.gheap = a.get<double>((size_t)hp.blocks * 64 * (size_t)k);
        if (with_idx) hp.gix = a.get<int32_t>((size_t)hp.blocks * 64 * (size_t)k);
    } else {
        hp.lds = (size_t)k * hp.threads * (sizeof(double) + (with_idx ? sizeof(int32_t) : 0));
    }
    return hp;
}
template <auto Kernel, int Bytes> int knn_lds_limit()
{
    static const hipError_t e = hipFuncSetAttribute((const void *)Kernel, hipFuncAttributeMaxDynamicSharedMemorySize, Bytes);
    if (e != hipSuccess) return fail(KPX_ERR_HIP, "hipFuncSetAttribute(MaxDynamicSharedMemorySize) failed: %s", hipGetErrorString(e));
    return KPX_OK;
}
template <class Op> struct KnnWavePass {
    void (*kernel)(const GridParams *, const uint32_t *, const float *, int64_t, int64_t, int, int, Op, const int32_t *, const int32_t *, int32_t *, int32_t *);
    int rc, waves, cap, max_blocks;
    int32_t *fb_list;
    bool on;
};
template <class Op, int WAVES> KnnWavePass<Op> knn_wave_pass(int cap, int max_blocks, int32_t *fb_list, bool on = true)
{
    return { knn_wave_kernel<Op, WAVES>, knn_lds_limit<knn_wave_kernel<Op, WAVES>, 96 * 1024>(), WAVES, cap, max_blocks, fb_list, on };
}
template <class Op> struct KnnHeapPass {
    void (*kernel)(const GridParams *, const uint32_t *, const float *, int64_t, int64_t, int, Op, const int32_t *, const int32_t *, double *, int32_t *);
    int rc;
};
template <class Op, bool ALT = false> KnnHeapPass<Op> knn_heap_pass() { return { knn_heap_kernel<Op, ALT>, knn_lds_limit<knn_heap_kernel<Op, ALT>, 160 * 1024>() }; }
template <class Op>
int knn_cascade(const Grid &g, int k, const Op &op, int64_t q0, int64_t q1, const int32_t *list, const int32_t *count,
                std::initializer_list<KnnWavePass<Op>> passes, int32_t *counters, const KnnHeapPass<Op> &heap, const KnnHeaps &hp, hipStream_t st)
{
    const int64_t nq = q1 - q0;
    if (nq <= 0) return KPX_OK;
    for (const KnnWavePass<Op> &p : passes) {
        int32_t *fb_count = counters++;
        if (p.rc) return p.rc;
        if (!p.on) continue;
        const int64_t blocks = cdiv(nq, p.waves) > p.max_blocks ? p.max_blocks : cdiv(nq, p.waves);
        hipLaunchKernelGGL(p.kernel, dim3((unsigned)blocks), dim3(64 * p.waves), (size_t)p.waves * p.cap * (sizeof(double) + (Op::kPos ? sizeof(uint32_t) : 0)),
                           st, g.params, g.cell_start, g.sorted_pts, q0, q1, k, p.cap, op, list, count, p.fb_list, fb_count);
        list = p.fb_list; count = fb_count;
    }
    if (heap.rc) return heap.rc;
    hipLaunchKernelGGL(heap.kernel, dim3(hp.blocks), dim3(hp.threads), hp.lds, st, g.params, g.cell_start, g.sorted_pts, q0, q1, k, op, list, count,
                       hp.gheap, hp.gix);
    return KPX_OK;
}

}
```

### kinectpy_amd/csrc/kpx_knn.hip

```cpp
#include <hipcub/hipcub.hpp>

#include "kpx_compact.h"
#include "kpx_gridknn.h"
#include "kpx_morton.h"
#include "kpx_linalg.h"

namespace kpx {

__device__ __forceinline__ void grid_dims(const double ext[3], double &h, int32_t cell_cap, int dim[3])
{
    for (;;) {
        double tot = 1.0;
        for (int a = 0; a < 3; ++a) {
            double d = floor(ext[a] / h) + 1.0;
            if (d > 1000000.0) d = 1000000.0;
            dim[a] = (int)d; tot *= d;
        }
        if (tot <= (double)cell_cap) break;
        h *= 1.26;
    }
}
__device__ __forceinline__ GridParams grid_params_of(const double *__restrict__ bbox, int64_t n, double target, int32_t cell_cap,
                                                     const unsigned long long *__restrict__ sumsq, double fixed_h)
{
    GridParams gp;
    double ext[3], vol = 1.0;
    for (int a = 0; a < 3; ++a) { ext[a] = bbox[3 + a] - bbox[a]; if (!(ext[a] > 1e-9)) ext[a] = 1e-9; vol *= ext[a]; }
    const double nn = (double)(n > 0 ? n : 1);
    const double h3 = cbrt(vol * target / nn);
    const double area = ext[0] * ext[1] + ext[1] * ext[2] + ext[0] * ext[2];
    const double h2 = sqrt(area * target / nn) * 0.5;
    double h = h3 > h2 ? h3 : h2;
    if (!(h > 0.0)) h = 1.0;
    if (fixed_h > h) h = fixed_h;
    int dim[3];
    grid_dims(ext, h, cell_cap, dim);
    if (sumsq && !(fixed_h > 0.0)) {
        const double occ = (double)*sumsq / nn;
        double f = pow(target / (occ > 1.0 ? occ : 1.0), 1.0 / 2.3);
        f = f < 0.125 ? 0.125 : (f > 8.0 ? 8.0 : f);
        h *= f;
        grid_dims(ext, h, cell_cap, dim);
    }
    gp.h = h;
    for (int a = 0; a < 3; ++a) { gp.org[a] = bbox[a]; gp.dim[a] = dim[a]; }
    gp.ncell = dim[0] * dim[1] * dim[2];
    return gp;
}
__global__ __launch_bounds__(256) void grid_occupancy_kernel(const uint32_t *__restrict__ cell_count, const GridParams *__restrict__ gp,
                                                             unsigned long long *__restrict__ sumsq)
{
    __shared__ unsigned long long sh[4];
    const int ncell = gp->ncell;
    unsigned long long c = 0;
    for (int i = blockIdx.x * blockDim.x + threadIdx.x; i < ncell; i += gridDim.x * blockDim.x) {
        unsigned long long v = cell_count[i];
        c += v * v;
    }
    c = block_sum(c, sh);
    if (threadIdx.x == 0 && c) atomicAdd(sumsq, c);
}
__global__ __launch_bounds__(256) void grid_cell_kernel(const float *__restrict__ pts, int64_t n, const double *__restrict__ bbox, double target,
                                                        int32_t cell_cap, const unsigned long long *__restrict__ sumsq, GridParams *gp,
                                                        uint32_t *__restrict__ keys, int32_t *__restrict__ vals, uint32_t *__restrict__ cell_count,
                                                        double fixed_h)
{
    __shared__ GridParams sg;
    if (threadIdx.x == 0) {
        sg = grid_params_of(bbox, n, target, cell_cap, sumsq, fixed_h);
        if (blockIdx.x == 0) *gp = sg;
    }
    __syncthreads();
    const GridParams g = sg;
    for (int64_t i = (int64_t)blockIdx.x * blockDim.x + threadIdx.x; i < n; i += (int64_t)gridDim.x * blockDim.x) {
        int cx = cell_coord(pts[3 * i], g.org[0], g.h, g.dim[0]);
        int cy = cell_coord(pts[3 * i + 1], g.org[1], g.h, g.dim[1]);
        int cz = cell_coord(pts[3 * i + 2], g.org[2], g.h, g.dim[2]);
        uint32_t cell = (uint32_t)((cx * g.dim[1] + cy) * g.dim[2] + cz);
        keys[i] = cell;
        vals[i] = (int32_t)i;
        atomicAdd(&cell_count[cell], 1u);
    }
}
__global__ __launch_bounds__(256) void grid_gather_kernel(const float *__restrict__ pts, int64_t n, const int32_t *__restrict__ order,
                                                          float *__restrict__ sorted_pts)
{
    for (int64_t s = (int64_t)blockIdx.x * blockDim.x + threadIdx.x; s < n; s += (int64_t)gridDim.x * blockDim.x) {
        int64_t i = order[s];
        sorted_pts[3 * s] = pts[3 * i]; sorted_pts[3 * s + 1] = pts[3 * i + 1]; sorted_pts[3 * s + 2] = pts[3 * i + 2];
    }
}
__global__ __launch_bounds__(256) void grid_place_kernel(const uint32_t *__restrict__ cell_of, int64_t n, const uint32_t *__restrict__ cell_start,
                                                         uint32_t *__restrict__ cursor, int32_t *__restrict__ slot_idx)
{
    for (int64_t i = (int64_t)blockIdx.x * blockDim.x + threadIdx.x; i < n; i += (int64_t)gridDim.x * blockDim.x) {
        const uint32_t c = cell_of[i];
        slot_idx[cell_start[c] + atomicAdd(&cursor[c], 1u)] = (int32_t)i;
    }
}
__global__ __launch_bounds__(256) void grid_rank_kernel(const float *__restrict__ pts, int64_t n, const uint32_t *__restrict__ cell_of,
                                                        const uint32_t *__restrict__ cell_start, const int32_t *__restrict__ slot_idx,
                                                        int32_t *__restrict__ sorted_idx, float *__restrict__ sorted_pts)
{
    for (int64_t s = (int64_t)blockIdx.x * blockDim.x + threadIdx.x; s < n; s += (int64_t)gridDim.x * blockDim.x) {
        const int32_t i = slot_idx[s];
        const uint32_t c = cell_of[i];
        const int64_t s0 = cell_start[c], s1 = cell_start[c + 1];
        int rank = 0;
        for (int64_t t = s0; t < s1; ++t) rank += slot_idx[t] < i ? 1 : 0;
        const int64_t d = s0 + rank;
        sorted_idx[d] = i;
        sorted_pts[3 * d] = pts[3 * (int64_t)i]; sorted_pts[3 * d + 1] = pts[3 * (int64_t)i + 1]; sorted_pts[3 * d + 2] = pts[3 * (int64_t)i + 2];
    }
}

constexpr int kGridScanItems = 8, kGridScanTile = 256 * kGridScanItems;
constexpr int kGridScanWords = 2 * ((kGridMaxCells + 1 + kGridScanTile - 1) / kGridScanTile) + 2;
__global__ __launch_bounds__(256) void grid_scan_kernel(const uint32_t *__restrict__ counts, int64_t len, uint32_t *__restrict__ out,
                                                        unsigned long long *__restrict__ states)
{
    __shared__ int sh[256 / 64 + 2];
    const int64_t base = (int64_t)blockIdx.x * kGridScanTile + (int64_t)threadIdx.x * kGridScanItems;
    uint32_t v[kGridScanItems];
    int c = 0;
#pragma unroll
    for (int k = 0; k < kGridScanItems; ++k) { v[k] = base + k < len ? counts[base + k] : 0u; c += (int)v[k]; }
    int tot;
    const int ex = block_excl_scan(c, sh, &tot);
    __syncthreads();
    const int before = lookback_exclusive(states, blockIdx.x, tot, sh + 256 / 64 + 1);
    uint32_t run = (uint32_t)(before + ex);
#pragma unroll
    for (int k = 0; k < kGridScanItems; ++k) {
        if (base + k < len) out[base + k] = run;
        run += v[k];
    }
}

int grid_build(const float *pts, int64_t n, double target_per_cell, Arena &a, Grid *g, hipStream_t st, double fixed_h)
{
    const size_t nn = (size_t)(n > 0 ? n : 1);
    g->params = a.get<GridParams>(1);
    uint32_t *zero = a.get<uint32_t>(3 * ((size_t)kGridMaxCells + 1) + 32 + kGridExtraWords + kGridScanWords);
    g->cell_start = a.get<uint32_t>((size_t)kGridMaxCells + 1);
    g->sorted_pts = a.get<float>(nn * 3);
    g->sorted_idx = a.get<int32_t>(nn);
    double *part = a.get<double>((size_t)kBboxBlocks * 6 + 8);
    size_t scan_bytes = memo_bytes(kMemoGridScan, kGridMaxCells + 1, [&] { size_t b = 0; (void)hipcub::DeviceScan::ExclusiveSum(nullptr, b, zero, g->cell_start, kGridMaxCells + 1, st); return b; });
    DeviceSort<uint32_t> sort;
    SortOptions o;
    o.vals_out = false;
    o.radix = kRadixAndVendor;
    o.tmp_floor = scan_bytes;
    dsort_carve(a, n, 22, o, &sort);
    sort.vals_out = g->sorted_idx;
    g->sorted_keys = sort.keys_out;
    if (a.dry) return KPX_OK;
    KPX_ARENA_CHECK(a);
    double *bbox = part + (size_t)kBboxBlocks * 6;
    int rc = bbox_f32(pts, n, bbox, part, st);
    if (rc) return rc;
    int32_t cell_cap = 65536;
    while (cell_cap < kGridMaxCells && (int64_t)cell_cap < 16 * n) cell_cap <<= 1;
    g->spare = reinterpret_cast<int32_t *>(zero);
    unsigned long long *sumsq = reinterpret_cast<unsigned long long *>(zero + 16);
    g->extra = reinterpret_cast<int32_t *>(zero + 32);
    unsigned long long *scan_states = reinterpret_cast<unsigned long long *>(zero + 32 + kGridExtraWords);
    uint32_t *count1 = zero + 32 + kGridExtraWords + kGridScanWords, *count2 = count1 + (size_t)cell_cap + 1, *cursor = count2 + (size_t)cell_cap + 1;
    KPX_HIP(hipMemsetAsync(zero, 0, (32 + kGridExtraWords + kGridScanWords + 3 * ((size_t)cell_cap + 1)) * sizeof(uint32_t), st));
    int nb = (int)(cdiv(n, 256) > 4096 ? 4096 : cdiv(n, 256));
    hipLaunchKernelGGL(grid_cell_kernel, dim3(nb), dim3(256), 0, st, pts, n, bbox, target_per_cell, cell_cap, (const unsigned long long *)nullptr, g->params,
                       sort.keys_in, sort.vals_in, count1, fixed_h);
    hipLaunchKernelGGL(grid_occupancy_kernel, dim3(1024), dim3(256), 0, st, count1, g->params, sumsq);
    hipLaunchKernelGGL(grid_cell_kernel, dim3(nb), dim3(256), 0, st, pts, n, bbox, target_per_cell, cell_cap, (const unsigned long long *)sumsq, g->params,
                       sort.keys_in, sort.vals_in, count2, fixed_h);
    static const bool vendor_scan = [] { const char *e = getenv("KPX_GRID_SCAN"); return e && e[0] == '0'; }();
    if (vendor_scan) KPX_HIP(hipcub::DeviceScan::ExclusiveSum(sort.tmp, scan_bytes, count2, g->cell_start, cell_cap + 1, st));
    else
        hipLaunchKernelGGL(grid_scan_kernel, dim3((unsigned)cdiv((int64_t)cell_cap + 1, kGridScanTile)), dim3(256), 0, st, count2, (int64_t)cell_cap + 1, g->cell_start,
                           scan_states);
    static const bool force_sort = [] { const char *e = getenv("KPX_GRID_SORT"); return e && e[0] == '1'; }();
    const bool by_sort = force_sort || n > 65536;
    if (by_sort) {
        rc = dsort_run(sort, n, 22, st);
        if (rc) return rc;
        hipLaunchKernelGGL(grid_gather_kernel, dim3(nb), dim3(256), 0, st, pts, n, g->sorted_idx, g->sorted_pts);
    } else {
        hipLaunchKernelGGL(grid_place_kernel, dim3(nb), dim3(256), 0, st, sort.keys_in, n, g->cell_start, cursor, sort.vals_in);
        hipLaunchKernelGGL(grid_rank_kernel, dim3(nb), dim3(256), 0, st, pts, n, sort.keys_in, g->cell_start, sort.vals_in, g->sorted_idx, g->sorted_pts);
    }
    KPX_LAUNCH_CHECK();
    return KPX_OK;
}

struct SorOp {
    static constexpr bool kPos = false;
    using Heap = HeapD;
    const int32_t *sidx;
    int64_t q0;
    double *avg;
    __device__ double r2max(bool heap_walk) const { return heap_walk ? -1.0 : INFINITY; }
    __device__ void defer(int64_t) const {}
    __device__ void wave(const WaveKnnScratch &sc, const WaveKnnResult &res, int64_t s, const float *) const
    {
        const int lane = threadIdx.x & 63;
        double sum = 0.0;
        for (int t = lane; t < res.m; t += 64) {
            const double d = sc.vals[t];
            if ((unsigned long long)__double_as_longlong(d) <= res.thr) sum += sqrt(d);
        }
#pragma unroll
        for (int o = 32; o > 0; o >>= 1) sum += __shfl_xor(sum, o, 64);
        const double total = sum - (double)(res.cnt - res.kk) * sqrt(res.top);
        if (lane == 0) avg[sidx ? (int64_t)sidx[s] : s - q0] = res.kk > 0 ? total / (double)res.kk : -1.0;
    }
    __device__ void heap(int64_t s, const HeapD &heap) const
    {
        double sum = 0.0;
        for (int e = 0; e < heap.sz; ++e) sum += sqrt(heap.h[e * heap.stride]);
        avg[sidx ? (int64_t)sidx[s] : s - q0] = heap.sz > 0 ? sum / (double)heap.sz : -1.0;
    }
};

__device__ __forceinline__ int dppi(int v, int ctrl_sel)
{
    switch (ctrl_sel) {
    case 1: return __builtin_amdgcn_update_dpp(v, v, 0x121, 0xF, 0xF, false);
    case 2: return __builtin_amdgcn_update_dpp(v, v, 0x122, 0xF, 0xF, false);
    case 4: return __builtin_amdgcn_update_dpp(v, v, 0x124, 0xF, 0xF, false);
    default: return __builtin_amdgcn_update_dpp(v, v, 0x128, 0xF, 0xF, false);
    }
}
__device__ __forceinline__ int wave_sum_i(int v)
{
    v += dppi(v, 1); v += dppi(v, 2); v += dppi(v, 4); v += dppi(v, 8);
    v += __shfl_xor(v, 16, 64);
    v += __shfl_xor(v, 32, 64);
    return v;
}
__device__ __forceinline__ unsigned wave_min_u(unsigned v)
{
    unsigned o;
    o = (unsigned)dppi((int)v, 1); v = o < v ? o : v; o = (unsigned)dppi((int)v, 2); v = o < v ? o : v;
    o = (unsigned)dppi((int)v, 4); v = o < v ? o : v; o = (unsigned)dppi((int)v, 8); v = o < v ? o : v;
    o = (unsigned)__shfl_xor((int)v, 16, 64); v = o < v ? o : v;
    o = (unsigned)__shfl_xor((int)v, 32, 64); v = o < v ? o : v;
    return v;
}
__device__ __forceinline__ unsigned wave_max_u(unsigned v)
{
    unsigned o;
    o = (unsigned)dppi((int)v, 1); v = o > v ? o : v; o = (unsigned)dppi((int)v, 2); v = o > v ? o : v;
    o = (unsigned)dppi((int)v, 4); v = o > v ? o : v; o = (unsigned)dppi((int)v, 8); v = o > v ? o : v;
    o = (unsigned)__shfl_xor((int)v, 16, 64); v = o > v ? o : v;
    o = (unsigned)__shfl_xor((int)v, 32, 64); v = o > v ? o : v;
    return v;
}
constexpr int kSorBuckets = 256;
constexpr int kSorTieRoom = 32;
constexpr int kBlkQueries = 64, kBlkWaves = 4;
#ifndef KPX_SOR_BLOCK_MINB
#define KPX_SOR_BLOCK_MINB 4
#endif
template <int S>
__global__ __launch_bounds__(64 * kBlkWaves, KPX_SOR_BLOCK_MINB) void sor_block_kernel(
    const GridParams *__restrict__ gp, const uint32_t *__restrict__ cell_start, const float *__restrict__ spts, const int32_t *__restrict__ sidx,
    int64_t q0, int64_t q1, int k, int kbuf, double *__restrict__ avg, int32_t *__restrict__ fb_list, int32_t *__restrict__ fb_count)
{
    constexpr int CAP = 64 * S, W = kBlkWaves, T = 64 * kBlkWaves;
    extern __shared__ __align__(16) double lds[];
    __shared__ uint32_t run_s0[32];
    __shared__ int32_t run_off[32];
    __shared__ float qf[3][kBlkQueries];
    __shared__ int32_t qc[3][kBlkQueries];
    __shared__ int32_t qcell[kBlkQueries], qsidx[kBlkQueries];
    __shared__ uint8_t qstate[kBlkQueries];
    __shared__ int32_t s_m;
    const int tid = threadIdx.x, wave = tid >> 6, lane = tid & 63;
    float *cand = reinterpret_cast<float *>(lds);
    uint32_t *hist = reinterpret_cast<uint32_t *>(lds + (size_t)(CAP * 3) / 2) + (size_t)wave * kSorBuckets;
    double *selbuf = lds + (size_t)(CAP * 3) / 2 + (size_t)W * kSorBuckets / 2 + (size_t)wave * kbuf;
    const GridParams g = *gp;
    const int64_t nq = q1 - q0;
    for (int64_t chunk = blockIdx.x; chunk * kBlkQueries < nq; chunk += gridDim.x) {
        const int64_t base = q0 + chunk * kBlkQueries;
        const int nqc = (int)(q1 - base < kBlkQueries ? q1 - base : kBlkQueries);
        if (tid < nqc) {
            const float *qp = spts + 3 * (base + tid);
            int c[3];
#pragma unroll
            for (int a = 0; a < 3; ++a) { const float v = qp[a]; qf[a][tid] = v; c[a] = cell_coord((double)v, g.org[a], g.h, g.dim[a]); qc[a][tid] = c[a]; }
            qcell[tid] = (int32_t)(((int64_t)c[0] * g.dim[1] + c[1]) * g.dim[2] + c[2]);
            qsidx[tid] = sidx ? sidx[base + tid] : (int32_t)(base + tid - q0);
            qstate[tid] = 0;
        }
        __syncthreads();
        const int mycell = lane < nqc ? qcell[lane] : -1;
        const int prevcell = __shfl_up(mycell, 1, 64);
        unsigned long long segs = __builtin_amdgcn_ballot_w64(lane < nqc && (lane == 0 || mycell != prevcell));
        while (segs != 0ull) {
            const int pos = __builtin_ctzll(segs);
            segs &= segs - 1ull;
            const int len = (segs ? __builtin_ctzll(segs) : nqc) - pos;
            const int cx = qc[0][pos], cy = qc[1][pos], cz = qc[2][pos];
            for (int rad = 1; rad <= 2; ++rad) {
                if (rad == 2 && __builtin_amdgcn_ballot_w64(lane < len && qstate[pos + lane] == 0) == 0ull) break;
                const int side = 2 * rad + 1, nruns = side * side;
                if (wave == 0) {
                    uint32_t s0 = 0u;
                    int ln = 0;
                    if (lane < nruns) {
                        const int x = cx + lane / side - rad, y = cy + lane % side - rad;
                        if (x >= 0 && x < g.dim[0] && y >= 0 && y < g.dim[1]) {
                            const int64_t col = ((int64_t)x * g.dim[1] + y) * g.dim[2];
                            const int za = cz - rad < 0 ? 0 : cz - rad, zb = cz + rad >= g.dim[2] ? g.dim[2] - 1 : cz + rad;
                            s0 = cell_start[col + za];
                            ln = (int)(cell_start[col + zb + 1] - s0);
                        }
                    }
                    const int incl = wave_incl_scan(ln);
                    if (lane < 32) { run_s0[lane] = s0; run_off[lane] = lane < nruns ? incl - ln : INT_MAX; }
                    if (lane == 63) s_m = incl;
                }
                __syncthreads();
                const int m = s_m;
                if (m <= CAP) {
#pragma unroll
                    for (int tr = 0; tr < CAP / T; ++tr) {
                        const int jn = tr * T + tid;
                        if (jn < m) {
                            int r = 0;
#pragma unroll
                            for (int st = 16; st > 0; st >>= 1) { const int cr = r + st; if (cr < nruns && run_off[cr] <= jn) r = cr; }
                            const float *pp = spts + 3 * (int64_t)(run_s0[r] + (uint32_t)(jn - run_off[r]));
                            cand[3 * jn] = pp[0]; cand[3 * jn + 1] = pp[1]; cand[3 * jn + 2] = pp[2];
                        }
                    }
                }
                __syncthreads();
                if (m <= CAP) {
                    const int c[3] = { cx, cy, cz };
                    for (int qi = pos + wave; qi < pos + len; qi += W) {
                        if (qstate[qi] != 0) continue;
                        const double q[3] = { (double)qf[0][qi], (double)qf[1][qi], (double)qf[2][qi] };
                        const double cov2 = block_cover2(g, q, c, rad);
                        const bool whole = cov2 == INFINITY;
                        const unsigned ch = (unsigned)((unsigned long long)__double_as_longlong(cov2) >> 32);
                        unsigned hi[S], lo[S];
                        int cnt = 0, zeros = 0;
                        unsigned vmin = 0xFFFFFFFFu;
                        int vmax = -1;
#pragma unroll
                        for (int sl = 0; sl < S; ++sl) {
                            hi[sl] = 0xFFFFFFFFu; lo[sl] = 0xFFFFFFFFu;
                            const int jn = sl * 64 + lane;
                            if (sl * 64 < m && jn < m) {
                                const double dx = q[0] - (double)cand[3 * jn], dy = q[1] - (double)cand[3 * jn + 1], dz = q[2] - (double)cand[3 * jn + 2];
                                const double d2 = fma(dz, dz, fma(dy, dy, dx * dx));
                                const unsigned long long pat = (unsigned long long)__double_as_longlong(d2);
                                hi[sl] = (unsigned)(pat >> 32); lo[sl] = (unsigned)pat;
                                cnt += d2 < cov2 ? 1 : 0;
                                zeros += hi[sl] == 0u ? 1 : 0;
                                const unsigned nz = hi[sl] == 0u ? 0xFFFFFFFFu : hi[sl];
                                vmin = nz < vmin ? nz : vmin;
                                vmax = (int)hi[sl] > vmax ? (int)hi[sl] : vmax;
                            }
                        }
                        cnt = wave_sum_i(cnt);
                        zeros = wave_sum_i(zeros);
                        const int kk = whole ? (m < k ? m : k) : k;
                        bool ok = cnt >= kk;
                        unsigned a = wave_min_u(vmin);
                        unsigned b = wave_max_u((unsigned)(vmax < 0 ? 0 : vmax));
                        if (!whole && b > ch) b = ch;
                        bool exact = false;
                        {
                            constexpr int BPL = kSorBuckets / 64;
                            int need_k = kk - zeros;
                            if (need_k <= 0) a = b = 0u;
                            unsigned range = b - a;
                            bool run = ok && a < b;
                            while (run) {
                                const int shift = range >= 256u ? 24 - __builtin_clz(range) : 0;
                                uint4 *hz = reinterpret_cast<uint4 *>(hist + lane * BPL);
                                hz[0] = make_uint4(0u, 0u, 0u, 0u);
                                wave_lds_fence();
#pragma unroll
                                for (int sl = 0; sl < S; ++sl)
                                    if (sl * 64 < m) {
                                        const unsigned rel = hi[sl] - a;
                                        if (rel <= range) __hip_atomic_fetch_add(hist + (rel >> shift), 1u, __ATOMIC_RELAXED, __HIP_MEMORY_SCOPE_WORKGROUP);
                                    }
                                wave_lds_fence();
                                const uint4 t4 = hz[0];
                                const int hv[BPL] = { (int)t4.x, (int)t4.y, (int)t4.z, (int)t4.w };
                                const int lsum = hv[0] + hv[1] + hv[2] + hv[3];
                                const int incl = wave_incl_scan(lsum), excl = incl - lsum;
                                const bool mine = need_k > excl && need_k <= incl;
                                int B = -1, cb = 0, hb = 0;
                                if (mine) {
                                    int cum = excl;
#pragma unroll
                                    for (int w = 0; w < BPL; ++w) {
                                        if (B < 0 && need_k <= cum + hv[w]) { B = lane * BPL + w; cb = cum; hb = hv[w]; }
                                        cum += hv[w];
                                    }
                                }
                                const unsigned long long bm = __builtin_amdgcn_ballot_w64(mine);
                                const int owner = bm ? __builtin_ctzll(bm) : 0;
                                B = __shfl(B, owner, 64); cb = __shfl(cb, owner, 64); hb = __shfl(hb, owner, 64);
                                const unsigned wend = a + range, bstart = a + ((unsigned)(B < 0 ? 0 : B) << shift), bspan = (1u << shift) - 1u;
                                const unsigned bend = wend - bstart < bspan ? wend : bstart + bspan;
                                if (B < 0) { ok = false; run = false; }
                                else if (need_k - cb == hb) { a = bend; exact = true; run = false; }
                                else if (shift == 0) { a = bstart; run = false; }
                                else { need_k -= cb; a = bstart; range = bend - bstart; }
                            }
                        }
                        const unsigned P = a;
                        unsigned Q = 0xFFFFFFFFu;
                        int n_le = kk;
                        if (ok && !exact) {
                            int c_less = 0, c_eq = 0;
#pragma unroll
                            for (int sl = 0; sl < S; ++sl) if (sl * 64 < m) { c_less += hi[sl] < P ? 1 : 0; c_eq += hi[sl] == P ? 1 : 0; }
                            c_less = wave_sum_i(c_less); c_eq = wave_sum_i(c_eq);
                            n_le = c_less + c_eq;
                            const int r2 = kk - c_less;
                            if (n_le > kk) {
                                unsigned lmin = 0xFFFFFFFFu, lmax = 0u;
#pragma unroll
                                for (int sl = 0; sl < S; ++sl) if (hi[sl] == P) { lmin = lo[sl] < lmin ? lo[sl] : lmin; lmax = lo[sl] > lmax ? lo[sl] : lmax; }
                                unsigned a2 = wave_min_u(lmin), b2 = wave_max_u(lmax);
                                while (a2 < b2) {
                                    const unsigned mid = a2 + ((b2 - a2) >> 1);
                                    int c2 = 0;
#pragma unroll
                                    for (int sl = 0; sl < S; ++sl) c2 += (hi[sl] == P && lo[sl] <= mid) ? 1 : 0;
                                    c2 = wave_sum_i(c2);
                                    if (c2 >= r2) b2 = mid; else a2 = mid + 1;
                                }
                                int c3 = 0;
#pragma unroll
                                for (int sl = 0; sl < S; ++sl) c3 += (hi[sl] == P && lo[sl] <= a2) ? 1 : 0;
                                c3 = wave_sum_i(c3);
                                Q = a2; n_le = c_less + c3;
                            }
                        }
                        const bool tied_out = ok && n_le > kk + kSorTieRoom;
                        if (tied_out) ok = false;
                        if (ok) {
                            int wbase = 0;
#pragma unroll
                            for (int sl = 0; sl < S; ++sl)
                                if (sl * 64 < m) {
                                    const bool sel = hi[sl] < P || (hi[sl] == P && lo[sl] <= Q);
                                    const unsigned long long bm = __builtin_amdgcn_ballot_w64(sel);
                                    if (sel)
                                        selbuf[wbase + (int)__builtin_amdgcn_mbcnt_hi((unsigned)(bm >> 32), __builtin_amdgcn_mbcnt_lo((unsigned)bm, 0u))] =
                                            __longlong_as_double((long long)(((unsigned long long)hi[sl] << 32) | lo[sl]));
                                    wbase += __builtin_popcountll(bm);
                                }
                            wave_lds_fence();
                            double acc = 0.0;
                            for (int t = lane; t < n_le; t += 64) acc += sqrt(selbuf[t]);
#pragma unroll
                            for (int o = 32; o > 0; o >>= 1) acc += __shfl_down(acc, o, 64);
                            if (lane == 0) {
                                const double top = __longlong_as_double((long long)(((unsigned long long)P << 32) | Q));
                                const double total = n_le > kk ? acc - (double)(n_le - kk) * sqrt(top) : acc;
                                avg[qsidx[qi]] = kk > 0 ? total / (double)kk : -1.0;
                            }
                            wave_lds_fence();
                        }
                        if (lane == 0 && (ok || tied_out)) qstate[qi] = ok ? 1 : 2;
                    }
                }
                __syncthreads();
            }
        }
        if (wave == 0) {
            const bool fb = lane < nqc && qstate[lane] != 1;
            const unsigned long long fm = __builtin_amdgcn_ballot_w64(fb);
            if (fm != 0ull) {
                int fb_base = 0;
                if (lane == 0) fb_base = atomicAdd(fb_count, __builtin_popcountll(fm));
                fb_base = __shfl(fb_base, 0, 64);
                if (fb) fb_list[fb_base + __builtin_popcountll(fm & ((1ull << lane) - 1ull))] = (int32_t)(base + lane);
            }
        }
        __syncthreads();
    }
}

__global__ __launch_bounds__(256) void sor_sum_kernel(const double *__restrict__ avg, int64_t n, const double *__restrict__ stats,
                                                      int pass, double *__restrict__ part)
{
    __shared__ double sh[4];
    double mean = pass ? stats[0] : 0.0, acc = 0.0;
    for (int64_t i = (int64_t)blockIdx.x * blockDim.x + threadIdx.x; i < n; i += (int64_t)gridDim.x * blockDim.x) {
        double v = avg[i];
        if (v > 0.0) acc += pass ? (v - mean) * (v - mean) : v;
    }
    acc = block_sum(acc, sh);
    if (threadIdx.x == 0) part[blockIdx.x] = acc;
}
__global__ void sor_final_kernel(const double *__restrict__ part, int nb, int64_t n, double std_ratio, int pass, double *stats)
{
    if (threadIdx.x || blockIdx.x) return;
    double s = 0.0;
    for (int b = 0; b < nb; ++b) s += part[b];
    if (pass == 0) stats[0] = s / (double)n;
    else { stats[1] = sqrt(s / (double)(n - 1)); stats[2] = stats[0] + std_ratio * stats[1]; }
}
struct SorPred {
    const double *avg; const double *stats;
    __device__ bool operator()(int64_t i, int) const { double v = avg[i]; return v > 0.0 && v < stats[2]; }
};
struct IdxEmit {
    int32_t *idx;
    __device__ void operator()(int64_t i, int, int32_t dst) const { idx[dst] = (int32_t)i; }
};
struct SorGather {
    const float *a0, *a1;
    float *o0, *o1;
};
__global__ __launch_bounds__(256) void sor_gather_kernel(SorGather g, const int32_t *__restrict__ idx, const int32_t *__restrict__ d_count,
                                                         int32_t *__restrict__ count_out)
{
    const int64_t n = *d_count;
    if (blockIdx.x == 0 && threadIdx.x == 0) *count_out = (int32_t)n;
    for (int64_t k = (int64_t)blockIdx.x * blockDim.x + threadIdx.x; k < n; k += (int64_t)gridDim.x * blockDim.x) {
        const int64_t s = idx[k];
        if (g.a0) { g.o0[3 * k] = g.a0[3 * s]; g.o0[3 * k + 1] = g.a0[3 * s + 1]; g.o0[3 * k + 2] = g.a0[3 * s + 2]; }
        if (g.a1) { g.o1[3 * k] = g.a1[3 * s]; g.o1[3 * k + 1] = g.a1[3 * s + 1]; g.o1[3 * k + 2] = g.a1[3 * s + 2]; }
    }
}

static int sor_block_threads(int k)
{
    if (k <= 32) return 256;
    if (k <= 80) return 128;
    return 64;
}

__global__ __launch_bounds__(1024) void sor_stats_small_kernel(const double *__restrict__ avg, int64_t n, int nb, double std_ratio, double *__restrict__ stats)
{
    __shared__ double part[64];
    __shared__ double sh[4][4];
    __shared__ double s_mean;
    const int vb = threadIdx.x >> 8, t = threadIdx.x & 255;
    for (int pass = 0; pass < 2; ++pass) {
        const double mean = pass ? s_mean : 0.0;
        for (int b0 = 0; b0 < nb; b0 += 4) {
            const int b = b0 + vb;
            double acc = 0.0;
            if (b < nb)
                for (int64_t i0 = (int64_t)b * 256 + t; i0 < n; i0 += 8 * (int64_t)nb * 256) {
                    double v[8];
#pragma unroll
                    for (int u = 0; u < 8; ++u) {
                        const int64_t i = i0 + (int64_t)u * nb * 256;
                        v[u] = i < n ? avg[i] : 0.0;
                    }
#pragma unroll
                    for (int u = 0; u < 8; ++u)
                        if (v[u] > 0.0) acc += pass ? (v[u] - mean) * (v[u] - mean) : v[u];
                }
            acc = wave_sum(acc);
            if ((t & 63) == 0) sh[vb][t >> 6] = acc;
            __syncthreads();
            if (t == 0 && b < nb) part[b] = ((sh[vb][0] + sh[vb][1]) + sh[vb][2]) + sh[vb][3];
            __syncthreads();
        }
        if (threadIdx.x == 0) {
            double s = 0.0;
            for (int b = 0; b < nb; ++b) s += part[b];
            if (pass == 0) { stats[0] = s / (double)n; s_mean = stats[0]; }
            else { stats[1] = sqrt(s / (double)(n - 1)); stats[2] = stats[0] + std_ratio * stats[1]; }
        }
        __syncthreads();
    }
}

static int sor_stats_compact(const double *avg, int64_t n, double std_ratio, double *part, int32_t *counts, int32_t *keep_idx,
                             int32_t *d_count, double *d_stats, hipStream_t st, const SorGather *ga = nullptr, bool state_is_clear = false)
{
    int nb = (int)(cdiv(n, 256 * 8) < 1 ? 1 : (cdiv(n, 256 * 8) > 1024 ? 1024 : cdiv(n, 256 * 8)));
    if (nb <= 64) {
        hipLaunchKernelGGL(sor_stats_small_kernel, dim3(1), dim3(1024), 0, st, avg, n, nb, std_ratio, d_stats);
    } else {
        for (int pass = 0; pass < 2; ++pass) {
            hipLaunchKernelGGL(sor_sum_kernel, dim3(nb), dim3(256), 0, st, avg, n, d_stats, pass, part);
            hipLaunchKernelGGL(sor_final_kernel, dim3(1), dim3(1), 0, st, part, nb, n, std_ratio, pass, d_stats);
        }
    }
    KPX_LAUNCH_CHECK();
    int32_t *dev_count = reinterpret_cast<int32_t *>(part + 1023);
    const int rc = compact(SorPred{ avg, d_stats }, IdxEmit{ keep_idx }, n, 1, counts, ga ? dev_count : d_count, st, state_is_clear);
    if (rc || !ga) return rc;
    const int64_t gb = cdiv(n, 256);
    hipLaunchKernelGGL(sor_gather_kernel, dim3((unsigned)(gb < 1 ? 1 : (gb > 4096 ? 4096 : gb))), dim3(256), 0, st, *ga, keep_idx, dev_count, d_count);
    KPX_LAUNCH_CHECK();
    return KPX_OK;
}

__global__ __launch_bounds__(256) void sor_unsort_kernel(const double *__restrict__ avg_sorted, const int32_t *__restrict__ order, int64_t n,
                                                         double *__restrict__ avg)
{
    for (int64_t s = (int64_t)blockIdx.x * blockDim.x + threadIdx.x; s < n; s += (int64_t)gridDim.x * blockDim.x) avg[order[s]] = avg_sorted[s];
}

static int sor_impl(const float *pts, int64_t n, int k, double std_ratio, int32_t *keep_idx, int32_t *d_count, double *d_stats,
                    double *d_avg, Arena &a, hipStream_t st, bool full = true, int64_t q0 = 0, int64_t q1 = 0, int32_t *d_order = nullptr,
                    const SorGather *ga = nullptr)
{
    Grid g;
    if (full) { q0 = 0; q1 = n; }
    int kk = (int64_t)k < n ? k : (int)(n > 0 ? n : 1);
    static const double occ_factor = [] { const char *e = getenv("KPX_SOR_OCC"); const double v = e ? atof(e) : 0.0; return v > 0.0 ? v : 0.4; }();
    double occ = occ_factor * (double)kk;
    occ = occ < 6.0 ? 6.0 : (occ > 240.0 ? 240.0 : occ);
    int rc = grid_build(pts, n, occ, a, &g, st);
    if (rc) return rc;
    double *avg = a.get<double>((size_t)(n > 0 ? n : 1));
    double *part = a.get<double>(1024);
    int32_t *counts = a.get<int32_t>((size_t)compact_ws_ints(n));
    int32_t *fb_list = a.get<int32_t>((size_t)(n > 0 ? n : 1) + 1);
    int32_t *fb_list2 = a.get<int32_t>((size_t)(n > 0 ? n : 1) + 1);
    int32_t *fb_list0 = a.get<int32_t>((size_t)(n > 0 ? n : 1) + 1);
    const KnnHeaps hp = knn_heaps_carve(a, kk, KPX_SOR_LDS_K, false, sor_block_threads(kk));
    if (a.dry) return KPX_OK;
    KPX_ARENA_CHECK(a);
    if (d_avg) avg = d_avg;
    const int32_t *out_idx = full ? g.sorted_idx : nullptr;
    const int64_t nq = q1 - q0;
    int32_t *fb_count0 = g.spare + 2;
    {
        ProfScope prof(KPX_PROF_SOR_KNN, 12.0 * (double)n + 8.0 * (double)n, st);
        static const int cell_mode = [] { const char *e = getenv("KPX_SOR_CELL"); return e ? (e[0] == '0' ? 0 : 2) : 1; }();
        const bool cell_on = (cell_mode == 2 || (cell_mode == 1 && kk > 32)) && kk <= 1024;
        const int32_t *list0 = nullptr, *count0 = nullptr;
        if (cell_on && nq > 0) {
            const int kbuf = kk + kSorTieRoom;
            const int64_t bchunks = cdiv(nq, kBlkQueries);
            const int S = kk <= 32 ? 4 : (kk <= 64 ? 8 : (kk <= 128 ? 16 : 32));
            const auto kernel = S == 4 ? sor_block_kernel<4> : (S == 8 ? sor_block_kernel<8> : (S == 16 ? sor_block_kernel<16> : sor_block_kernel<32>));
            hipLaunchKernelGGL(kernel, dim3((unsigned)(bchunks > 16384 ? 16384 : bchunks)), dim3(64 * kBlkWaves),
                               ((size_t)(64 * S * 3) / 2 + (size_t)kBlkWaves * kSorBuckets / 2 + (size_t)kBlkWaves * kbuf) * 8, st, g.params, g.cell_start,
                               g.sorted_pts, out_idx, q0, q1, kk, kbuf, avg, fb_list0, fb_count0);
            list0 = fb_list0; count0 = fb_count0;
        }
        rc = knn_cascade<SorOp>(g, kk, SorOp{ out_idx, q0, avg }, q0, q1, list0, count0,
                                { knn_wave_pass<SorOp, 4>(kk <= 32 ? 512 : 1024, list0 ? 2048 : 8192, fb_list, kk <= 512),
                                  knn_wave_pass<SorOp, 1>(8192, 2048, fb_list2, kk <= 4096) },
                                g.spare, knn_heap_pass<SorOp>(), hp, st);
        if (rc) return rc;
    }
    if (!full) {
        if (d_order) KPX_HIP(hipMemcpyAsync(d_order, g.sorted_idx, (size_t)n * sizeof(int32_t), hipMemcpyDeviceToDevice, st));
        KPX_LAUNCH_CHECK();
        return KPX_OK;
    }
    const bool fits = compact_ws_ints(n) <= kGridExtraWords;
    return sor_stats_compact(avg, n, std_ratio, part, fits ? g.extra : counts, keep_idx, d_count, d_stats, st, ga, fits);
}

__device__ __forceinline__ void store_cov9(double *o, const double *cov)
{
    if (!cov) {
#pragma unroll
        for (int e = 0; e < 9; ++e) o[e] = (e % 4 == 0) ? 1.0 : 0.0;
        return;
    }
    o[0] = cov[0]; o[1] = cov[1]; o[2] = cov[2];
    o[3] = cov[1]; o[4] = cov[3]; o[5] = cov[4];
    o[6] = cov[2]; o[7] = cov[4]; o[8] = cov[5];
}
template <bool COV>
__device__ __forceinline__ void moments_finish(const double sums[9], double m, int64_t me, float *__restrict__ normals, double *__restrict__ out_cov)
{
    double cov[6], nrm[3] = { 0.0, 0.0, 1.0 };
    const bool enough = m >= 3.0;
    if (enough) cov6_from_moments(sums, m, cov);
    if constexpr (COV) {
        if (enough) store_cov9(out_cov + 9 * me, cov);
        else store_cov9(out_cov + 9 * me, nullptr);
    } else {
        if (enough) sym3_smallest_axis(cov, nrm);
        normals[3 * me] = (float)nrm[0]; normals[3 * me + 1] = (float)nrm[1]; normals[3 * me + 2] = (float)nrm[2];
    }
}
struct MomentsOp {
    static constexpr bool kPos = true;
    using Heap = HeapDI;
    const int32_t *sidx;
    const float *pts;
    double r2;
    double *covbuf;
    float *normals;
    double *out_cov;
    __device__ double r2max(bool) const { return r2; }
    __device__ void defer(int64_t s) const { covbuf[10 * s + 9] = -1.0; }
    __device__ void wave(const WaveKnnScratch &sc, const WaveKnnResult &res, int64_t s, const float *__restrict__ spts) const
    {
        const int lane = threadIdx.x & 63;
        const int32_t idx_thr = wave_knn_tie_threshold(sc, res, sidx);
        double c[9] = { 0, 0, 0, 0, 0, 0, 0, 0, 0 };
        for (int t = lane; t < res.m; t += 64) {
            if (wave_knn_is_selected(sc, res, sidx, idx_thr, t)) {
                const float *pp = spts + 3 * (int64_t)sc.pos[t];
                const double x = pp[0], y = pp[1], z = pp[2];
                c[0] += x; c[1] += y; c[2] += z;
                c[3] += x * x; c[4] += x * y; c[5] += x * z; c[6] += y * y; c[7] += y * z; c[8] += z * z;
            }
        }
#pragma unroll
        for (int a9 = 0; a9 < 9; ++a9)
#pragma unroll
            for (int o = 32; o > 0; o >>= 1) c[a9] += __shfl_xor(c[a9], o, 64);
        if (lane == 0) {
            double *o = covbuf + 10 * s;
#pragma unroll
            for (int a9 = 0; a9 < 9; ++a9) o[a9] = c[a9];
            o[9] = (double)res.kk;
        }
    }
    template <bool COV> __device__ void heap_finish(int64_t s, const HeapDI &heap) const
    {
        double c[9] = { 0, 0, 0, 0, 0, 0, 0, 0, 0 };
        if (heap.sz >= 3)
            for (int e = 0; e < heap.sz; ++e) {
                int64_t j = heap.ix[e * heap.stride];
                double x = pts[3 * j], y = pts[3 * j + 1], z = pts[3 * j + 2];
                c[0] += x; c[1] += y; c[2] += z;
                c[3] += x * x; c[4] += x * y; c[5] += x * z; c[6] += y * y; c[7] += y * z; c[8] += z * z;
            }
        moments_finish<COV>(c, (double)heap.sz, sidx[s], normals, out_cov);
    }
    __device__ void heap(int64_t s, const HeapDI &h) const { heap_finish<false>(s, h); }
    __device__ void heap_alt(int64_t s, const HeapDI &h) const { heap_finish<true>(s, h); }
};
template <bool COV>
__global__ __launch_bounds__(256) void normals_eigen_kernel(const double *__restrict__ covbuf, const int32_t *__restrict__ sidx, int64_t n,
                                                            float *__restrict__ normals, double *__restrict__ out_cov)
{
    const int64_t s = (int64_t)blockIdx.x * blockDim.x + threadIdx.x;
    if (s >= n) return;
    const double *in = covbuf + 10 * s;
    const double m = in[9];
    if (m < 0.0) return;
    moments_finish<COV>(in, m, sidx[s], normals, out_cov);
}

static int normals_impl(const float *pts, int64_t n, double radius, int max_nn, float *normals, Arena &a, hipStream_t st,
                        double *out_cov = nullptr)
{
    Grid g;
    int kk = (int64_t)max_nn < n ? max_nn : (int)(n > 0 ? n : 1);
    int rc = grid_build(pts, n, 8.0, a, &g, st);
    if (rc) return rc;
    int32_t *fb_list = a.get<int32_t>((size_t)(n > 0 ? n : 1) + 1);
    double *covbuf = a.get<double>((size_t)(n > 0 ? n : 1) * 10);
    const KnnHeaps hp = knn_heaps_carve(a, kk, KPX_NORMALS_LDS_NN, true, kk <= 48 ? 128 : 64);
    if (a.dry) return KPX_OK;
    KPX_ARENA_CHECK(a);
    const bool wave_pass = kk <= 512;
    rc = knn_cascade<MomentsOp>(g, kk, MomentsOp{ g.sorted_idx, pts, radius * radius, covbuf, normals, out_cov }, 0, n, nullptr, nullptr,
                                { knn_wave_pass<MomentsOp, 4>(kk <= 48 ? 512 : 1024, 8192, fb_list, wave_pass) }, g.spare,
                                out_cov ? knn_heap_pass<MomentsOp, true>() : knn_heap_pass<MomentsOp, false>(), hp, st);
    if (rc) return rc;
    const auto eigen_kernel = out_cov ? normals_eigen_kernel<true> : normals_eigen_kernel<false>;
    if (wave_pass) hipLaunchKernelGGL(eigen_kernel, dim3((unsigned)cdiv(n, 256)), dim3(256), 0, st, covbuf, g.sorted_idx, n, normals, out_cov);
    KPX_LAUNCH_CHECK();
    return KPX_OK;
}

}

using namespace kpx;

KPX_EXPORT size_t kpx_sor_workspace_bytes(int64_t n, int32_t nb_neighbors)
{
    Arena a(nullptr, 0);
    sor_impl(nullptr, n, nb_neighbors < 1 ? 1 : nb_neighbors, 1.0, nullptr, nullptr, nullptr, nullptr, a, nullptr);
    return a.off;
}
KPX_EXPORT int kpx_sor(const float *pts, int64_t n, int32_t nb_neighbors, double std_ratio, int32_t *keep_idx,
                       int32_t *d_count, double *d_stats, double *d_avg, void *ws, size_t ws_bytes, void *stream)
{
    KPX_REQUIRE(nb_neighbors >= 1 && std_ratio > 0.0, "remove_statistical_outlier: nb_neighbors and std_ratio must be positive");
    KPX_REQUIRE(nb_neighbors <= KPX_SOR_MAX_K, "remove_statistical_outlier: nb_neighbors > %d is not supported", KPX_SOR_MAX_K);
    KPX_REQUIRE(n >= 0 && n < ((int64_t)1 << 31), "kpx_sor: bad size");
    KPX_REQUIRE(d_count && d_stats && ws, "kpx_sor: null pointer");
    hipStream_t st = (hipStream_t)stream;
    if (n == 0) { KPX_HIP(hipMemsetAsync(d_count, 0, sizeof(int32_t), st)); return KPX_OK; }
    KPX_REQUIRE(pts && keep_idx, "kpx_sor: null pointer");
    Arena a(ws, ws_bytes);
    return sor_impl(pts, n, nb_neighbors, std_ratio, keep_idx, d_count, d_stats, d_avg, a, st);
}

KPX_EXPORT int kpx_sor_select(const float *pts, const float *attr, int64_t n, int32_t nb_neighbors, double std_ratio, float *out_pts,
                              float *out_attr, int32_t *keep_idx, int32_t *d_count, double *d_stats, void *ws, size_t ws_bytes, void *stream)
{
    KPX_REQUIRE(nb_neighbors >= 1 && std_ratio > 0.0, "remove_statistical_outlier: nb_neighbors and std_ratio must be positive");
    KPX_REQUIRE(nb_neighbors <= KPX_SOR_MAX_K, "remove_statistical_outlier: nb_neighbors > %d is not supported", KPX_SOR_MAX_K);
    KPX_REQUIRE(n >= 0 && n < ((int64_t)1 << 31), "kpx_sor_select: bad size");
    KPX_REQUIRE(d_count && d_stats && ws, "kpx_sor_select: null pointer");
    KPX_REQUIRE(!attr || out_attr, "kpx_sor_select: attributes without an output array");
    hipStream_t st = (hipStream_t)stream;
    if (n == 0) { KPX_HIP(hipMemsetAsync(d_count, 0, sizeof(int32_t), st)); return KPX_OK; }
    KPX_REQUIRE(pts && keep_idx && out_pts, "kpx_sor_select: null pointer");
    Arena a(ws, ws_bytes);
    const SorGather ga{ pts, attr, out_pts, out_attr };
    return sor_impl(pts, n, nb_neighbors, std_ratio, keep_idx, d_count, d_stats, nullptr, a, st, true, 0, 0, nullptr, &ga);
}

KPX_EXPORT int kpx_sor_partial(const float *pts, int64_t n, int32_t nb_neighbors, int64_t q_begin, int64_t q_end, double *d_avg_sorted,
                               int32_t *d_order, void *ws, size_t ws_bytes, void *stream)
{
    KPX_REQUIRE(nb_neighbors >= 1, "remove_statistical_outlier: nb_neighbors and std_ratio must be positive");
    KPX_REQUIRE(nb_neighbors <= KPX_SOR_MAX_K, "remove_statistical_outlier: nb_neighbors > %d is not supported", KPX_SOR_MAX_K);
    KPX_REQUIRE(n >= 1 && n < ((int64_t)1 << 31), "kpx_sor_partial: bad size");
    KPX_REQUIRE(q_begin >= 0 && q_begin <= q_end && q_end <= n, "kpx_sor_partial: bad query range");
    KPX_REQUIRE(pts && ws && (d_avg_sorted || q_begin == q_end), "kpx_sor_partial: null pointer");
    Arena a(ws, ws_bytes);
    return sor_impl(pts, n, nb_neighbors, 1.0, nullptr, nullptr, nullptr, d_avg_sorted, a, (hipStream_t)stream, false, q_begin, q_end, d_order);
}
struct SorFinishScratch { double *avg, *part; int32_t *counts; };
static void sor_finish_carve(Arena &a, int64_t n, SorFinishScratch *s)
{
    s->avg = a.get<double>((size_t)(n > 0 ? n : 1));
    s->part = a.get<double>(1024);
    s->counts = a.get<int32_t>((size_t)compact_ws_ints(n));
}
KPX_EXPORT size_t kpx_sor_finish_workspace_bytes(int64_t n)
{
    Arena a(nullptr, 0);
    SorFinishScratch s;
    sor_finish_carve(a, n, &s);
    return a.off;
}
KPX_EXPORT int kpx_sor_finish(const double *d_avg_sorted, const int32_t *d_order, int64_t n, double std_ratio, int32_t *keep_idx,
                              int32_t *d_count, double *d_stats, double *d_avg, void *ws, size_t ws_bytes, void *stream)
{
    KPX_REQUIRE(std_ratio > 0.0, "remove_statistical_outlier: nb_neighbors and std_ratio must be positive");
    KPX_REQUIRE(n >= 1 && n < ((int64_t)1 << 31), "kpx_sor_finish: bad size");
    KPX_REQUIRE(d_avg_sorted && d_order && keep_idx && d_count && d_stats && ws, "kpx_sor_finish: null pointer");
    hipStream_t st = (hipStream_t)stream;
    Arena a(ws, ws_bytes);
    SorFinishScratch s;
    sor_finish_carve(a, n, &s);
    KPX_ARENA_CHECK(a);
    double *avg = d_avg ? d_avg : s.avg;
    hipLaunchKernelGGL(sor_unsort_kernel, dim3((unsigned)(cdiv(n, 256) > 4096 ? 4096 : cdiv(n, 256))), dim3(256), 0, st, d_avg_sorted, d_order, n, avg);
    return sor_stats_compact(avg, n, std_ratio, s.part, s.counts, keep_idx, d_count, d_stats, st);
}

KPX_EXPORT size_t kpx_normals_workspace_bytes(int64_t n, int32_t max_nn)
{
    Arena a(nullptr, 0);
    normals_impl(nullptr, n, 1.0, max_nn < 1 ? 1 : max_nn, nullptr, a, nullptr);
    return a.off;
}
KPX_EXPORT int kpx_estimate_normals(const float *pts, int64_t n, double radius, int32_t max_nn, float *normals, void *ws,
                                    size_t ws_bytes, void *stream)
{
    KPX_REQUIRE(radius > 0.0 && max_nn >= 1, "estimate_normals: radius and max_nn must be positive");
    KPX_REQUIRE(max_nn <= KPX_NORMALS_MAX_NN, "estimate_normals: max_nn > %d is not supported", KPX_NORMALS_MAX_NN);
    KPX_REQUIRE(n >= 0 && n < ((int64_t)1 << 31), "kpx_estimate_normals: bad size");
    if (n == 0) return KPX_OK;
    KPX_REQUIRE(pts && normals && ws, "kpx_estimate_normals: null pointer");
    Arena a(ws, ws_bytes);
    return normals_impl(pts, n, radius, max_nn, normals, a, (hipStream_t)stream);
}

KPX_EXPORT size_t kpx_covariances_workspace_bytes(int64_t n, int32_t max_nn) { return kpx_normals_workspace_bytes(n, max_nn); }
KPX_EXPORT int kpx_estimate_covariances(const float *pts, int64_t n, double radius, int32_t max_nn, double *cov, void *ws, size_t ws_bytes,
                                        void *stream)
{
    KPX_REQUIRE(radius > 0.0 && max_nn >= 1, "estimate_covariances: radius and max_nn must be positive");
    KPX_REQUIRE(max_nn <= KPX_NORMALS_MAX_NN, "estimate_covariances: max_nn > %d is not supported", KPX_NORMALS_MAX_NN);
    KPX_REQUIRE(n >= 0 && n < ((int64_t)1 << 31), "kpx_estimate_covariances: bad size");
    if (n == 0) return KPX_OK;
    KPX_REQUIRE(pts && cov && ws, "kpx_estimate_covariances: null pointer");
    Arena a(ws, ws_bytes);
    return normals_impl(pts, n, radius, max_nn, nullptr, a, (hipStream_t)stream, cov);
}
```

### kinectpy_amd/csrc/kpx_voxel.hip

```cpp
#include "kpx_voxelsteps.h"

namespace kpx {

template <bool NRM>
__global__ __launch_bounds__(256) void voxel_mean_kernel(StoredLoad load, int64_t n, const int32_t *__restrict__ vals, const int32_t *__restrict__ seg_start,
                                                         int32_t *__restrict__ d_count, const int32_t *__restrict__ err, float *__restrict__ opts,
                                                         float *__restrict__ ocol, float *__restrict__ onrm)
{
    const int32_t m_total = *d_count;
    if (blockIdx.x == 0 && threadIdx.x == 0 && *err) *d_count = KPX_ERR_RANGE;
    for (int64_t m = (int64_t)blockIdx.x * blockDim.x + threadIdx.x; m < m_total; m += (int64_t)gridDim.x * blockDim.x) {
        const int64_t s0 = seg_start[m], s1 = (m + 1 < m_total) ? seg_start[m + 1] : n;
        double sp[3] = { 0, 0, 0 }, sc[3] = { 0, 0, 0 }, sn[3] = { 0, 0, 0 };
        voxel_segment_sum<NRM>(vals, s0, s1, load, sp, sc, sn);
        voxel_write_row(sp, sc, (double)(s1 - s0), opts + 3 * m, (load.col && ocol) ? ocol + 3 * m : nullptr);
        if (NRM && onrm) {
            double nn = sqrt(fma(sn[2], sn[2], fma(sn[1], sn[1], sn[0] * sn[0])));
#pragma unroll
            for (int a = 0; a < 3; ++a) onrm[3 * m + a] = (float)(nn > 0 ? sn[a] / nn : sn[a]);
        }
    }
}
static int voxel_impl(const float *pts, const float *col, const float *nrm, int64_t n, double voxel, float *opts,
                      float *ocol, float *onrm, int32_t *d_count, Arena &a, hipStream_t st)
{
    VoxelScratch s;
    voxel_carve(a, n, kPlainCarve, &s);
    KPX_ARENA_CHECK(a);
    int rc = bbox_f32(pts, n, s.bbox, s.part, st);
    if (rc) return rc;
    KPX_HIP(hipMemsetAsync(s.err, 0, sizeof(int32_t), st));
    int nb = (int)(cdiv(n, 256) > 4096 ? 4096 : cdiv(n, 256));
    CloudSet<1> one;
    one.pts[0] = pts; one.off[0] = 0; one.off[1] = n; one.count = 1;
    hipLaunchKernelGGL((voxel_key_kernel<CloudSet<1>, StoredPoint, FixedKeys>), dim3(nb), dim3(256), 0, st, one, (const double *)s.bbox, voxel,
                       FixedKeys{ s.sort.keys_in, s.err }, s.sort.vals_in);
    rc = voxel_sort_and_heads<uint64_t>(s, n, 63, d_count, st);
    if (rc) return rc;
    const StoredLoad load = { pts, col, nrm, 0 };
    const auto mean_kernel = nrm ? &voxel_mean_kernel<true> : &voxel_mean_kernel<false>;
    hipLaunchKernelGGL(mean_kernel, dim3(nb), dim3(256), 0, st, load, n, (const int32_t *)s.sort.vals_out,
                       (const int32_t *)s.seg_start, d_count, (const int32_t *)s.err, opts, ocol, onrm);
    KPX_LAUNCH_CHECK();
    return KPX_OK;
}

constexpr int kVoxelBatchMax = 8;
constexpr int kVoxelBatchBboxBlocks = 64;
constexpr VoxelCarve kBatchCarve = { kVoxelBatchMax, kVoxelBatchBboxBlocks, true, true, 64 };
struct VoxelBatch : CloudSet<kVoxelBatchMax> {
    const float *col[kVoxelBatchMax];
    float *opts[kVoxelBatchMax];
    float *ocol[kVoxelBatchMax];
    int32_t morton;
};
static VoxelBatch voxel_batch_of(const float *const *h_pts, const float *const *h_col, const int64_t *h_n, float *const *h_opts, float *const *h_ocol,
                                 int first, int count, bool morton)
{
    VoxelBatch b;
    b.count = count;
    b.morton = morton ? 1 : 0;
    b.off[0] = 0;
    for (int i = 0; i < kVoxelBatchMax; ++i) {
        const bool on = i < count;
        b.pts[i] = on ? h_pts[first + i] : nullptr;
        b.col[i] = (on && h_col) ? h_col[first + i] : nullptr;
        b.opts[i] = on ? h_opts[first + i] : nullptr;
        b.ocol[i] = (on && h_col && h_ocol) ? h_ocol[first + i] : nullptr;
        b.off[i + 1] = b.off[i] + (on ? h_n[first + i] : 0);
    }
    return b;
}
__device__ __forceinline__ void voxel_batch_axis_bits(const double d[3], int bits[3])
{
#pragma unroll
    for (int a = 0; a < 3; ++a) {
        const unsigned long long m = (unsigned long long)d[a] - 1ull;
        int n = 1;
        while (n < 21 && (m >> n) != 0ull) ++n;
        bits[a] = n;
    }
}
__device__ __forceinline__ unsigned long long voxel_hcode(unsigned long long x, unsigned long long y, unsigned long long z, int bits)
{
    unsigned long long X[3] = { x, y, z };
    const unsigned long long M = 1ull << (bits - 1);
    for (unsigned long long Q = M; Q > 1ull; Q >>= 1) {
        const unsigned long long P = Q - 1ull;
#pragma unroll
        for (int i = 0; i < 3; ++i) {
            if (X[i] & Q) X[0] ^= P;
            else { const unsigned long long t = (X[0] ^ X[i]) & P; X[0] ^= t; X[i] ^= t; }
        }
    }
    X[1] ^= X[0];
    X[2] ^= X[1];
    unsigned long long t = 0ull;
    for (unsigned long long Q = M; Q > 1ull; Q >>= 1)
        if (X[2] & Q) t ^= Q - 1ull;
    X[0] ^= t; X[1] ^= t; X[2] ^= t;
    unsigned long long k = 0ull;
    for (int b = bits - 1; b >= 0; --b) {
#pragma unroll
        for (int i = 0; i < 3; ++i) k = (k << 1) | ((X[i] >> b) & 1ull);
    }
    return k;
}
__device__ __forceinline__ int voxel_hilbert_cube_bits(const int ab[3], int cb)
{
    const int top = ab[0] > ab[1] ? (ab[0] > ab[2] ? ab[0] : ab[2]) : (ab[1] > ab[2] ? ab[1] : ab[2]);
    const int low = ab[0] < ab[1] ? (ab[0] < ab[2] ? ab[0] : ab[2]) : (ab[1] < ab[2] ? ab[1] : ab[2]);
    const int passes = (ab[0] + ab[1] + ab[2] + cb + 7) / 8;
    for (int m = top; m > low; --m) {
        int n = 3 * m + cb;
#pragma unroll
        for (int a = 0; a < 3; ++a) n += ab[a] > m ? ab[a] - m : 0;
        if (n <= 64 && (n + 7) / 8 <= passes) return m;
    }
    return low;
}
__device__ __forceinline__ int voxel_hilbert_key_bits(const int ab[3], int m)
{
    int n = 3 * m;
#pragma unroll
    for (int a = 0; a < 3; ++a) n += ab[a] > m ? ab[a] - m : 0;
    return n;
}
__device__ __forceinline__ unsigned long long voxel_hilbert_key(unsigned long long x, unsigned long long y, unsigned long long z, const int ab[3], int m)
{
    const unsigned long long mask = (1ull << m) - 1ull;
    const int ey = ab[1] > m ? ab[1] - m : 0, ez = ab[2] > m ? ab[2] - m : 0;
    const unsigned long long hi = (((x >> m) << ey | (y >> m)) << ez) | (z >> m);
    return (hi << (3 * m)) | voxel_hcode(x & mask, y & mask, z & mask, m);
}
__device__ __forceinline__ void voxel_batch_dims(const VoxelBatch &b, const double *__restrict__ bbox, double voxel, double d[3], int *overflow)
{
    d[0] = d[1] = d[2] = 1.0;
    for (int c = 0; c < b.count; ++c) {
        if (b.off[c + 1] == b.off[c]) continue;
        double f[3];
        (void)voxel_cell(bbox + 8 * c + 3, bbox + 8 * c, voxel, f);
        for (int a = 0; a < 3; ++a) {
            const double e = f[a] + 1.0;
            if (e > d[a] && e < kVoxelAxisCells) d[a] = e;
        }
    }
    *overflow = ((double)b.count * d[0]) * (d[1] * d[2]) >= 18446744073709551616.0 ? 1 : 0;
}
__device__ __forceinline__ int voxel_batch_key_bits(const VoxelBatch &b, const double d[3], int overflow)
{
    int n = 64;
    if (!overflow && b.morton) {
        int cb = 0, ab[3];
        while ((1 << cb) < b.count) ++cb;
        voxel_batch_axis_bits(d, ab);
        n = voxel_hilbert_key_bits(ab, voxel_hilbert_cube_bits(ab, cb)) + cb;
        n = n < 1 ? 1 : (n > 64 ? 64 : n);
    } else if (!overflow) {
        const unsigned long long range = (((unsigned long long)b.count * (unsigned long long)d[0]) * (unsigned long long)d[1]) * (unsigned long long)d[2];
        n = 1;
        while (n < 64 && (range >> n) != 0ull) ++n;
    }
    return n;
}
__global__ void voxel_batch_bits_kernel(VoxelBatch b, const double *__restrict__ bbox, double voxel, int32_t *__restrict__ bits)
{
    double d[3];
    int overflow;
    voxel_batch_dims(b, bbox, voxel, d, &overflow);
    *bits = voxel_batch_key_bits(b, d, overflow);
}
template <class Key> struct BatchKeys {
    struct Grid {
        uint64_t DX, DY, DZ;
        int overflow, morton, ab[3], m;
    };
    Key *keys;
    int32_t *err, *bits_out;
    __device__ __forceinline__ Grid grid(const VoxelBatch &b, const double *__restrict__ bbox, double voxel) const
    {
        __shared__ double dims[3];
        __shared__ int overflow, axis_bits[3], cube_bits;
        if (threadIdx.x == 0) {
            double d[3];
            int ov;
            voxel_batch_dims(b, bbox, voxel, d, &ov);
            if (bits_out && blockIdx.x == 0) *bits_out = voxel_batch_key_bits(b, d, ov);
            dims[0] = d[0]; dims[1] = d[1]; dims[2] = d[2];
            int ab[3], cb = 0;
            voxel_batch_axis_bits(d, ab);
            axis_bits[0] = ab[0]; axis_bits[1] = ab[1]; axis_bits[2] = ab[2];
            while ((1 << cb) < b.count) ++cb;
            cube_bits = voxel_hilbert_cube_bits(ab, cb);
            overflow = (ov || (b.morton && voxel_hilbert_key_bits(ab, cube_bits) + cb > 64)) ? 1 : 0;
        }
        __syncthreads();
        return Grid{ (uint64_t)dims[0], (uint64_t)dims[1], (uint64_t)dims[2], overflow, b.morton, { axis_bits[0], axis_bits[1], axis_bits[2] }, cube_bits };
    }
    __device__ __forceinline__ void put(const Grid &g, const double *__restrict__ bbox, double voxel, int64_t i, int c, const double q[3]) const
    {
        double f[3];
        const bool bad = voxel_cell(q, bbox + 8 * c, voxel, f) || g.overflow;
        if (bad) { err[c] = 1; f[0] = f[1] = f[2] = 0.0; }
        if (g.morton)
            keys[i] = (Key)(((uint64_t)c << voxel_hilbert_key_bits(g.ab, g.m)) | voxel_hilbert_key((uint64_t)f[0], (uint64_t)f[1], (uint64_t)f[2], g.ab, g.m));
        else keys[i] = (Key)((((uint64_t)c * g.DX + (uint64_t)f[0]) * g.DY + (uint64_t)f[1]) * g.DZ + (uint64_t)f[2]);
    }
};
__global__ __launch_bounds__(64) void voxel_batch_locate_kernel(VoxelBatch b, const int32_t *__restrict__ seg_start, const int32_t *__restrict__ d_total,
                                                                const int32_t *__restrict__ err, int32_t *__restrict__ head, int32_t *__restrict__ d_counts)
{
    __shared__ int32_t h[kVoxelBatchMax + 1];
    const int c = threadIdx.x;
    const int32_t m = *d_total;
    if (c <= b.count) {
        int32_t lo = 0, hi = m;
        const int64_t want = b.off[c];
        while (lo < hi) {
            const int32_t mid = lo + (hi - lo) / 2;
            if (seg_start[mid] < want) lo = mid + 1; else hi = mid;
        }
        h[c] = c == b.count ? m : lo;
        head[c] = h[c];
    }
    __syncthreads();
    if (c < b.count) d_counts[c] = err[c] ? KPX_ERR_RANGE : h[c + 1] - h[c];
}
__global__ __launch_bounds__(256) void voxel_batch_mean_kernel(VoxelBatch b, const int32_t *__restrict__ vals, const int32_t *__restrict__ seg_start,
                                                               const int32_t *__restrict__ d_total, const int32_t *__restrict__ head)
{
    const int32_t m_total = *d_total;
    const int64_t total = b.off[b.count];
    for (int64_t m = (int64_t)blockIdx.x * blockDim.x + threadIdx.x; m < m_total; m += (int64_t)gridDim.x * blockDim.x) {
        const int64_t s0 = seg_start[m], s1 = (m + 1 < m_total) ? seg_start[m + 1] : total;
        const int c = b.cloud_of(s0);
        const StoredLoad load = { b.pts[c], b.col[c], nullptr, b.off[c] };
        double sp[3] = { 0, 0, 0 }, sc[3] = { 0, 0, 0 }, sn[3];
        voxel_segment_sum<false>(vals, s0, s1, load, sp, sc, sn);
        const int64_t o = m - head[c];
        voxel_write_row(sp, sc, (double)(s1 - s0), b.opts[c] + 3 * o, (load.col && b.ocol[c]) ? b.ocol[c] + 3 * o : nullptr);
    }
}

static int voxel_batch_impl(const VoxelBatch &b, double voxel, int32_t *d_counts, Arena &a, hipStream_t st, int spec_bits = 0,
                            int32_t *d_bits = nullptr)
{
    const int64_t total = b.off[b.count];
    VoxelScratch s;
    voxel_carve(a, total, kBatchCarve, &s);
    KPX_ARENA_CHECK(a);
    BoxDst boxes;
    for (int c = 0; c < kVoxelBatchMax; ++c) boxes.box[c] = s.bbox + 8 * c;
    boxes.err = s.err;
    hipLaunchKernelGGL((cloud_bbox_partial_kernel<VoxelBatch, StoredPoint, float, kVoxelBatchBboxBlocks>), dim3(kVoxelBatchBboxBlocks, b.count), dim3(256), 0, st, b, s.part);
    hipLaunchKernelGGL(cloud_bbox_final_kernel<kVoxelBatchBboxBlocks>, dim3(b.count), dim3(64), 0, st, (const double *)s.part, boxes);
    const int nb = (int)(cdiv(total, 256) > 4096 ? 4096 : cdiv(total, 256));
    int end_bit = 64;
    int32_t *bits_out = nullptr;
    if (spec_bits > 0 && d_bits) {
        bits_out = d_bits;
        end_bit = spec_bits > 64 ? 64 : spec_bits;
    } else if (total > (int64_t)128 * 1024) {
        int32_t *h_bits = static_cast<int32_t *>(thread_resources().pinned(kPinVoxelBits, sizeof(int32_t)));
        if (!h_bits) return KPX_ERR_HIP;
        hipLaunchKernelGGL(voxel_batch_bits_kernel, dim3(1), dim3(1), 0, st, b, s.bbox, voxel, s.head);
        KPX_HIP(hipMemcpyAsync(h_bits, s.head, sizeof(int32_t), hipMemcpyDeviceToHost, st));
        if (d_bits) KPX_HIP(hipMemcpyAsync(d_bits, s.head, sizeof(int32_t), hipMemcpyDefault, st));
        KPX_HIP(hipStreamSynchronize(st));
        end_bit = *h_bits < 1 ? 1 : (*h_bits > 64 ? 64 : *h_bits);
    } else if (d_bits) {
        hipLaunchKernelGGL(voxel_batch_bits_kernel, dim3(1), dim3(1), 0, st, b, s.bbox, voxel, d_bits);
    }
    int rc;
    if (end_bit <= 32) {
        hipLaunchKernelGGL((voxel_key_kernel<VoxelBatch, StoredPoint, BatchKeys<uint32_t>>), dim3(nb), dim3(256), 0, st, b, (const double *)s.bbox, voxel,
                           BatchKeys<uint32_t>{ reinterpret_cast<uint32_t *>(s.sort.keys_in), s.err, bits_out }, s.sort.vals_in);
        rc = voxel_sort_and_heads<uint32_t>(s, total, end_bit, s.d_total, st);
    } else {
        hipLaunchKernelGGL((voxel_key_kernel<VoxelBatch, StoredPoint, BatchKeys<uint64_t>>), dim3(nb), dim3(256), 0, st, b, (const double *)s.bbox, voxel,
                           BatchKeys<uint64_t>{ s.sort.keys_in, s.err, bits_out }, s.sort.vals_in);
        rc = voxel_sort_and_heads<uint64_t>(s, total, end_bit, s.d_total, st);
    }
    if (rc) return rc;
    hipLaunchKernelGGL(voxel_batch_locate_kernel, dim3(1), dim3(64), 0, st, b, s.seg_start, s.d_total, s.err, s.head, d_counts);
    hipLaunchKernelGGL(voxel_batch_mean_kernel, dim3(nb), dim3(256), 0, st, b, s.sort.vals_out, s.seg_start, s.d_total, s.head);
    KPX_LAUNCH_CHECK();
    return KPX_OK;
}

constexpr int kFuseMax = 16;
constexpr int kFuseBboxBlocks = 32;
constexpr VoxelCarve kFuseCarve = { kFuseMax, kFuseBboxBlocks, false, true, 63 };
struct FuseBatch : CloudSet<kFuseMax> {
    const float *col[kFuseMax];
    double T[kFuseMax][12];
    const double *dT[kFuseMax];
};
__global__ __launch_bounds__(64) void fuse_bbox_final_kernel(const double *__restrict__ part, int rows, double *__restrict__ bbox, int32_t *__restrict__ err)
{
    const int lane = lane_id();
    double v[6] = { INFINITY, INFINITY, INFINITY, -INFINITY, -INFINITY, -INFINITY };
    for (int r = lane; r < rows; r += 64) {
#pragma unroll
        for (int a = 0; a < 3; ++a) { v[a] = fmin(v[a], part[(int64_t)r * 6 + a]); v[3 + a] = fmax(v[3 + a], part[(int64_t)r * 6 + 3 + a]); }
    }
    box_wave_fold(v, v + 3);
    if (lane == 0) {
        for (int a = 0; a < 6; ++a) bbox[a] = v[a];
        *err = 0;
    }
}
__device__ __forceinline__ int fuse_key_bits(const double *__restrict__ bbox, double voxel, double d[3], bool *sane_out)
{
    (void)voxel_cell(bbox + 3, bbox, voxel, d);
#pragma unroll
    for (int a = 0; a < 3; ++a) d[a] += 1.0;
    const bool sane = d[0] >= 1.0 && d[1] >= 1.0 && d[2] >= 1.0 && d[0] < kVoxelAxisCells && d[1] < kVoxelAxisCells && d[2] < kVoxelAxisCells;
    int bits = 64;
    if (sane && d[0] * d[1] * d[2] < 18446744073709551616.0) {
        const unsigned long long range = (unsigned long long)d[0] * (unsigned long long)d[1] * (unsigned long long)d[2];
        bits = 1;
        while (bits < 64 && (range >> bits) != 0ull) ++bits;
    }
    *sane_out = sane;
    return bits;
}
__global__ void fuse_bits_kernel(const double *__restrict__ bbox, double voxel, int32_t *__restrict__ bits_out)
{
    double d[3];
    bool sane;
    *bits_out = fuse_key_bits(bbox, voxel, d, &sane);
}
struct ExtentKeys32 {
    struct Grid {
        double d[3];
        unsigned long long DY, DZ;
    };
    uint32_t *keys;
    int32_t *bits_out;
    template <class Set> __device__ __forceinline__ Grid grid(const Set &, const double *__restrict__ bbox, double voxel) const
    {
        Grid g;
        bool sane;
        const int bits = fuse_key_bits(bbox, voxel, g.d, &sane);
        if (blockIdx.x == 0 && threadIdx.x == 0) *bits_out = bits;
        g.DY = sane ? (unsigned long long)g.d[1] : 1ull;
        g.DZ = sane ? (unsigned long long)g.d[2] : 1ull;
        return g;
    }
    __device__ __forceinline__ void put(const Grid &g, const double *__restrict__ bbox, double voxel, int64_t i, int, const double q[3]) const
    {
        double f[3];
        if (voxel_cell(q, bbox, voxel, f, g.d)) f[0] = f[1] = f[2] = 0.0;
        keys[i] = (uint32_t)(((unsigned long long)f[0] * g.DY + (unsigned long long)f[1]) * g.DZ + (unsigned long long)f[2]);
    }
};
struct MovedLoad {
    using Coord = double;
    const FuseBatch &b;
    __device__ __forceinline__ bool has_col() const { return true; }
    __device__ __forceinline__ void operator()(int64_t p, double v[3], float c[3], float *) const
    {
        const int cl = b.cloud_of(p);
        const int64_t j = p - b.off[cl];
        MovedPoint()(b, cl, j, v);
        const float *col = b.col[cl];
#pragma unroll
        for (int a = 0; a < 3; ++a) c[a] = col ? col[3 * j + a] : 0.0f;
    }
};
__global__ __launch_bounds__(256) void fuse_mean_kernel(FuseBatch b, const int32_t *__restrict__ vals, const int32_t *__restrict__ seg_start,
                                                        int32_t *__restrict__ d_count, const int32_t *__restrict__ err, float *__restrict__ opts,
                                                        float *__restrict__ ocol)
{
    const int32_t m_total = *d_count;
    if (blockIdx.x == 0 && threadIdx.x == 0 && *err) *d_count = KPX_ERR_RANGE;
    const int64_t total = b.off[b.count];
    for (int64_t m = (int64_t)blockIdx.x * blockDim.x + threadIdx.x; m < m_total; m += (int64_t)gridDim.x * blockDim.x) {
        const int64_t s0 = seg_start[m], s1 = (m + 1 < m_total) ? seg_start[m + 1] : total;
        double sp[3] = { 0, 0, 0 }, sc[3] = { 0, 0, 0 }, sn[3];
        voxel_segment_sum<false>(vals, s0, s1, MovedLoad{ b }, sp, sc, sn);
        voxel_write_row(sp, sc, (double)(s1 - s0), opts + 3 * m, ocol ? ocol + 3 * m : nullptr);
    }
}
static int fuse_voxel_impl(const FuseBatch &b, double voxel, float *opts, float *ocol, int32_t *d_count, Arena &a, hipStream_t st, int spec_bits = 0,
                           int32_t *d_bits = nullptr)
{
    const int64_t total = b.off[b.count];
    VoxelScratch s;
    voxel_carve(a, total, kFuseCarve, &s);
    KPX_ARENA_CHECK(a);
    hipLaunchKernelGGL((cloud_bbox_partial_kernel<FuseBatch, MovedPoint, double, kFuseBboxBlocks>), dim3(kFuseBboxBlocks, b.count), dim3(256), 0, st, b, s.part);
    hipLaunchKernelGGL(fuse_bbox_final_kernel, dim3(1), dim3(64), 0, st, s.part, b.count * kFuseBboxBlocks, s.bbox, s.err);
    const int nb = (int)(cdiv(total, 256) > 4096 ? 4096 : cdiv(total, 256));
    int rc;
    if (spec_bits > 0 && spec_bits <= 32 && d_bits && total <= kRadixMaxPairs) {
        hipLaunchKernelGGL((voxel_key_kernel<FuseBatch, MovedPoint, ExtentKeys32>), dim3(nb), dim3(256), 0, st, b, (const double *)s.bbox, voxel,
                           ExtentKeys32{ reinterpret_cast<uint32_t *>(s.sort.keys_in), d_bits }, s.sort.vals_in);
        rc = voxel_sort_and_heads<uint32_t>(s, total, spec_bits, d_count, st);
    } else {
        if (d_bits) hipLaunchKernelGGL(fuse_bits_kernel, dim3(1), dim3(1), 0, st, s.bbox, voxel, d_bits);
        hipLaunchKernelGGL((voxel_key_kernel<FuseBatch, MovedPoint, FixedKeys>), dim3(nb), dim3(256), 0, st, b, (const double *)s.bbox, voxel,
                           FixedKeys{ s.sort.keys_in, s.err }, s.sort.vals_in);
        rc = voxel_sort_and_heads<uint64_t>(s, total, 63, d_count, st);
    }
    if (rc) return rc;
    hipLaunchKernelGGL(fuse_mean_kernel, dim3(nb), dim3(256), 0, st, b, s.sort.vals_out, s.seg_start, d_count, s.err, opts, ocol);
    KPX_LAUNCH_CHECK();
    return KPX_OK;
}
}

using namespace kpx;

KPX_EXPORT size_t kpx_fuse_voxel_workspace_bytes(int64_t total)
{
    Arena a(nullptr, 0);
    VoxelScratch s;
    voxel_carve(a, total, kFuseCarve, &s);
    return a.off;
}
KPX_EXPORT int kpx_fuse_voxel_downsample(int32_t count, const float *const *h_pts, const float *const *h_col, const int64_t *h_n,
                                         const double *h_T, double voxel, float *opts, float *ocol, int32_t *d_count, void *ws,
                                         size_t ws_bytes, void *stream)
{
    return kpx::fuse_voxel_downsample_dev(count, h_pts, h_col, h_n, h_T, nullptr, voxel, opts, ocol, d_count, ws, ws_bytes, stream, 0, nullptr);
}
int kpx::fuse_voxel_downsample_dev(int32_t count, const float *const *h_pts, const float *const *h_col, const int64_t *h_n, const double *h_T,
                                   const double *const *h_dT, double voxel, float *opts, float *ocol, int32_t *d_count, void *ws, size_t ws_bytes,
                                   void *stream, int spec_bits, int32_t *d_bits)
{
    KPX_REQUIRE(voxel > 0.0, "voxel_size <= 0");
    KPX_REQUIRE(count >= 1 && count <= kFuseMax, "kpx_fuse_voxel_downsample: 1 .. %d clouds", kFuseMax);
    KPX_REQUIRE(h_pts && h_n && h_T && d_count && ws, "kpx_fuse_voxel_downsample: null pointer");
    hipStream_t st = (hipStream_t)stream;
    FuseBatch b;
    b.count = count;
    b.off[0] = 0;
    bool any_col = false, all_col = true;
    for (int i = 0; i < kFuseMax; ++i) {
        const bool on = i < count;
        if (on) {
            KPX_REQUIRE(h_n[i] >= 0 && (h_n[i] == 0 || h_pts[i]), "kpx_fuse_voxel_downsample: bad cloud %d", i);
            if (h_n[i] > 0) { const bool hc = h_col && h_col[i]; any_col |= hc; all_col &= hc; }
        }
        b.pts[i] = on ? h_pts[i] : nullptr;
        b.col[i] = (on && h_col) ? h_col[i] : nullptr;
        b.off[i + 1] = b.off[i] + (on ? h_n[i] : 0);
        for (int k = 0; k < 12; ++k) b.T[i][k] = on ? h_T[16 * i + k] : 0.0;
        b.dT[i] = (on && h_dT) ? h_dT[i] : nullptr;
    }
    const int64_t total = b.off[count];
    KPX_REQUIRE(total < ((int64_t)1 << 31), "kpx_fuse_voxel_downsample: bad size");
    KPX_REQUIRE(!ocol || !any_col || all_col, "kpx_fuse_voxel_downsample: colours on some clouds only");
    if (total == 0) { KPX_HIP(hipMemsetAsync(d_count, 0, sizeof(int32_t), st)); return KPX_OK; }
    KPX_REQUIRE(opts, "kpx_fuse_voxel_downsample: null pointer");
    Arena a(ws, ws_bytes);
    return fuse_voxel_impl(b, voxel, opts, (any_col && all_col) ? ocol : nullptr, d_count, a, st, spec_bits, d_bits);
}

KPX_EXPORT size_t kpx_voxel_workspace_bytes(int64_t n)
{
    return kpx_voxel_batch_workspace_bytes(1, &n);
}
KPX_EXPORT int kpx_voxel_downsample(const float *pts, const float *col, const float *nrm, int64_t n, double voxel,
                                    float *opts, float *ocol, float *onrm, int32_t *d_count, void *ws, size_t ws_bytes,
                                    void *stream)
{
    KPX_REQUIRE(voxel > 0.0, "voxel_size <= 0");
    KPX_REQUIRE(n >= 0 && n < ((int64_t)1 << 31), "kpx_voxel_downsample: bad size");
    KPX_REQUIRE(d_count && ws, "kpx_voxel_downsample: null pointer");
    hipStream_t st = (hipStream_t)stream;
    if (n == 0) { KPX_HIP(hipMemsetAsync(d_count, 0, sizeof(int32_t), st)); return KPX_OK; }
    KPX_REQUIRE(pts && opts, "kpx_voxel_downsample: null pointer");
    Arena a(ws, ws_bytes);
    static const bool single_batch = [] { const char *e = getenv("KPX_VOXEL_SINGLE"); return !(e && e[0] == '0'); }();
    if (!nrm && single_batch) {
        return voxel_batch_impl(voxel_batch_of(&pts, &col, &n, &opts, col ? &ocol : nullptr, 0, 1, false), voxel, d_count, a, st);
    }
    return voxel_impl(pts, col, nrm, n, voxel, opts, ocol, onrm, d_count, a, st);
}

KPX_EXPORT size_t kpx_voxel_batch_workspace_bytes(int32_t count, const int64_t *h_n)
{
    if (count < 1 || !h_n) return 0;
    Arena a(nullptr, 0), one(nullptr, 0);
    VoxelScratch s;
    int64_t total = 0;
    for (int i = 0; i < count; ++i) {
        voxel_carve(a, h_n[i], kPlainCarve, &s);
        total += h_n[i] > 0 ? h_n[i] : 0;
    }
    voxel_carve(one, total, kBatchCarve, &s);
    return a.off > one.off ? a.off : one.off;
}
KPX_EXPORT int kpx_voxel_downsample_batch(int32_t count, const float *const *h_pts, const float *const *h_col, const int64_t *h_n,
                                          double voxel, float *const *h_opts, float *const *h_ocol, int32_t *d_counts, void *ws,
                                          size_t ws_bytes, void *stream)
{
    return kpx::voxel_downsample_batch_spec(count, h_pts, h_col, h_n, voxel, h_opts, h_ocol, d_counts, ws, ws_bytes, stream, 0, nullptr, false);
}
int kpx::voxel_downsample_batch_spec(int32_t count, const float *const *h_pts, const float *const *h_col, const int64_t *h_n, double voxel,
                                     float *const *h_opts, float *const *h_ocol, int32_t *d_counts, void *ws, size_t ws_bytes, void *stream,
                                     int spec_bits, int32_t *d_bits, bool morton)
{
    KPX_REQUIRE(voxel > 0.0, "voxel_size <= 0");
    KPX_REQUIRE(count >= 1 && count <= 64 && h_pts && h_n && h_opts && d_counts && ws, "kpx_voxel_downsample_batch: bad arguments");
    for (int i = 0; i < count; ++i)
// ... 51 lines not shown
```

Measured before the change: 2552.

## Centralize wavefront reductions in a DPP/permlane-based header and compact sqrt work

Replaces scattered shuffle-based wave reductions, scans and broadcasts with a shared header that uses DPP row ops, permlane swaps and readlane on the VALU path, plus a fused nine-way covariance reduction. The per-point high-word min/max/zero stats are now gathered during candidate insertion instead of being rescanned from LDS. The mean-NN kernel compacts selected entries into a list so sqrt runs on dense lanes. It also adds a selftest entry point for verifying the primitives. The cost targeted is cross-lane traffic through LDS-backed shuffles, at the risk of subtle correctness bugs in the DPP bound and bank masks.

Result: faster. 2679, median of 6 (+5.0%).

```diff
diff --git a/include/kinectpx.h b/include/kinectpx.h
--- a/include/kinectpx.h
+++ b/include/kinectpx.h
@@ -142,6 +142,18 @@
 size_t kpx_covariances_workspace_bytes(int64_t n, int32_t max_nn);
 int kpx_estimate_covariances(const float *pts, int64_t n, double radius, int32_t max_nn, double *cov,
                              void *ws, size_t ws_bytes, void *stream);
+
+#define KPX_WAVE_SUM_I32 0
+#define KPX_WAVE_MIN_U32 1
+#define KPX_WAVE_MAX_U32 2
+#define KPX_WAVE_MAX_U64 3
+#define KPX_WAVE_MAX_F64 4
+#define KPX_WAVE_INCL_SCAN_I32 5
+#define KPX_WAVE_BCAST 6
+#define KPX_WAVE_SUM_DOWN_F64 7
+#define KPX_WAVE_SUM_DOWN_F32 8
+#define KPX_WAVE_SUM_DOWN_F64X9 9
+int kpx_wave_selftest(int32_t kind, const uint64_t *in, int64_t rows, uint64_t *out, void *stream);
 
 size_t kpx_search_index_bytes(int64_t n);
 int kpx_search_index_build(const float *pts, int64_t n, void *index, size_t index_bytes, void *ws, size_t ws_bytes, void *stream);
diff --git a/kinectpy_amd/_lib.py b/kinectpy_amd/_lib.py
--- a/kinectpy_amd/_lib.py
+++ b/kinectpy_amd/_lib.py
@@ -6,7 +6,9 @@
 import torch
 
 _HERE = os.path.dirname(os.path.abspath(__file__))
-SO_PATH = os.environ.get("KPX_LIBRARY") or os.path.join(_HERE, "libkinectpx.so")
+_DEFAULT_SO = os.path.join(_HERE, "libkinectpx.so")
+SO_PATH = os.environ.get("KPX_LIBRARY") or _DEFAULT_SO
+SELFTEST_ONLY = ("kpx_wave_selftest",)
 
 _i64, _i32, _f64, _u64, _vp, _sz = C.c_int64, C.c_int32, C.c_double, C.c_uint64, C.c_void_p, C.c_size_t
 
@@ -37,6 +39,7 @@
     "kpx_voxel_downsample_batch": (C.c_int, [_i32, _vp, _vp, _vp, _f64, _vp, _vp, _vp, _vp, _sz, _vp]),
     "kpx_fuse_voxel_workspace_bytes": (_sz, [_i64]),
     "kpx_fuse_voxel_downsample": (C.c_int, [_i32, _vp, _vp, _vp, _vp, _f64, _vp, _vp, _vp, _vp, _sz, _vp]),
+    "kpx_wave_selftest": (C.c_int, [_i32, _vp, _i64, _vp, _vp]),
     "kpx_sor_workspace_bytes": (_sz, [_i64, _i32]),
     "kpx_sor": (C.c_int, [_vp, _i64, _i32, _f64, _vp, _vp, _vp, _vp, _vp, _sz, _vp]),
     "kpx_sor_partial": (C.c_int, [_vp, _i64, _i32, _i64, _i64, _vp, _vp, _vp, _sz, _vp]),
@@ -255,6 +258,8 @@
                 "(make -C kinectpy_amd/csrc).  There is no CPU fallback.")
         lib = C.CDLL(SO_PATH)
         for name, (res, args) in SIGNATURES.items():
+            if name in SELFTEST_ONLY and SO_PATH != _DEFAULT_SO and not hasattr(lib, name):
+                continue
             fn = getattr(lib, name)
             fn.restype, fn.argtypes = res, args
         _lib = lib
diff --git a/kinectpy_amd/csrc/kpx_common.h b/kinectpy_amd/csrc/kpx_common.h
--- a/kinectpy_amd/csrc/kpx_common.h
+++ b/kinectpy_amd/csrc/kpx_common.h
@@ -7,6 +7,7 @@
 #include <string.h>
 
 #include "../../include/kinectpx.h"
+#include "kpx_wave.h"
 
 #define KPX_EXPORT extern "C" __attribute__((visibility("default")))
 
diff --git a/kinectpy_amd/csrc/kpx_gridknn.h b/kinectpy_amd/csrc/kpx_gridknn.h
--- a/kinectpy_amd/csrc/kpx_gridknn.h
+++ b/kinectpy_amd/csrc/kpx_gridknn.h
@@ -162,12 +162,7 @@
         }
 }
 
-__device__ __forceinline__ unsigned long long wave_all_max_u64(unsigned long long v)
-{
-#pragma unroll
-    for (int o = 32; o > 0; o >>= 1) { const unsigned long long t = __shfl_xor(v, o, 64); v = t > v ? t : v; }
-    return v;
-}
+
 __device__ __forceinline__ double block_cover2(const GridParams &g, const double q[3], const int c[3], int r)
 {
     double dcov = INFINITY;
@@ -212,10 +207,7 @@
         const uint4 t4 = hz[0];
         const int hv[4] = { (int)t4.x, (int)t4.y, (int)t4.z, (int)t4.w };
         const int lsum = hv[0] + hv[1] + hv[2] + hv[3];
-        int incl = lsum;
-#pragma unroll
-        for (int o = 1; o < 64; o <<= 1) { const int t2 = __shfl_up(incl, o, 64); if (lane >= o) incl += t2; }
-        const int excl = incl - lsum;
+        const int incl = wave_incl_scan_i32(lsum), excl = incl - lsum;
         const bool mine = rank > excl && rank <= incl;
         int B = -1, cb = 0, hb = 0;
         if (mine) {
@@ -229,7 +221,7 @@
         const unsigned long long bm = __builtin_amdgcn_ballot_w64(mine);
         if (bm == 0ull) return a;
         const int owner = __builtin_ctzll(bm);
-        B = __shfl(B, owner, 64); cb = __shfl(cb, owner, 64); hb = __shfl(hb, owner, 64);
+        B = wave_bcast(B, owner); cb = wave_bcast(cb, owner); hb = wave_bcast(hb, owner);
         const unsigned wend = a + range, bstart = a + ((unsigned)B << shift), bspan = (1u << shift) - 1u;
         const unsigned bend = wend - bstart < bspan ? wend : bstart + bspan;
         if (rank - cb == hb) { exact = true; return bend; }
@@ -238,37 +230,24 @@
     }
     return a;
 }
-__device__ __forceinline__ unsigned wave_all_min_u32(unsigned v)
-{
-#pragma unroll
-    for (int o = 32; o > 0; o >>= 1) { const unsigned t = (unsigned)__shfl_xor((int)v, o, 64); v = t < v ? t : v; }
-    return v;
-}
-__device__ __forceinline__ unsigned wave_all_max_u32(unsigned v)
-{
-#pragma unroll
-    for (int o = 32; o > 0; o >>= 1) { const unsigned t = (unsigned)__shfl_xor((int)v, o, 64); v = t > v ? t : v; }
-    return v;
-}
-__device__ __forceinline__ int wave_all_sum_i32(int v)
-{
-#pragma unroll
-    for (int o = 32; o > 0; o >>= 1) v += __shfl_xor(v, o, 64);
-    return v;
-}
-__device__ __forceinline__ unsigned long long wave_kth_pattern(const double *__restrict__ vals, int m, int kk, uint32_t *__restrict__ hist)
-{
-    const int lane = threadIdx.x & 63;
-    const uint32_t *w32 = reinterpret_cast<const uint32_t *>(vals);
-    unsigned vmin = 0xFFFFFFFFu, vmax = 0u;
-    int zeros = 0;
-    for (int t = lane; t < m; t += 64) {
-        const unsigned h = w32[2 * t + 1];
+struct WaveHighStats {
+    unsigned vmin, vmax;
+    int zeros;
+    __device__ void reset() { vmin = 0xFFFFFFFFu; vmax = 0u; zeros = 0; }
+    __device__ void add(double d)
+    {
+        const unsigned h = (unsigned)((unsigned long long)__double_as_longlong(d) >> 32);
         zeros += h == 0u ? 1 : 0;
         const unsigned nz = h == 0u ? 0xFFFFFFFFu : h;
         vmin = nz < vmin ? nz : vmin; vmax = h > vmax ? h : vmax;
     }
-    vmin = wave_all_min_u32(vmin); vmax = wave_all_max_u32(vmax); zeros = wave_all_sum_i32(zeros);
+};
+__device__ __forceinline__ unsigned long long wave_kth_pattern(const double *__restrict__ vals, int m, int kk, uint32_t *__restrict__ hist, const WaveHighStats &hs)
+{
+    const int lane = threadIdx.x & 63;
+    const uint32_t *w32 = reinterpret_cast<const uint32_t *>(vals);
+    const unsigned vmin = wave_min_u32(hs.vmin), vmax = wave_max_u32(hs.vmax);
+    const int zeros = wave_sum_i32(hs.zeros);
     unsigned P = 0u;
     bool exact = false;
     if (kk > zeros) {
@@ -284,10 +263,10 @@
         c_less += h < P ? 1 : 0;
         if (h == P) { const unsigned l = w32[2 * t]; ++c_eq; lmin = l < lmin ? l : lmin; lmax = l > lmax ? l : lmax; }
     }
-    c_less = wave_all_sum_i32(c_less); c_eq = wave_all_sum_i32(c_eq);
+    c_less = wave_sum_i32(c_less); c_eq = wave_sum_i32(c_eq);
     const int r2 = kk - c_less;
     if (r2 >= c_eq) return ((unsigned long long)P << 32) | 0xFFFFFFFFull;
-    lmin = wave_all_min_u32(lmin); lmax = wave_all_max_u32(lmax);
+    lmin = wave_min_u32(lmin); lmax = wave_max_u32(lmax);
     unsigned Q = lmin;
     if (lmin < lmax)
         Q = wave_count_select([&](int t, unsigned &kv) { kv = w32[2 * t]; return w32[2 * t + 1] == P; }, m, lmin, lmax - lmin, r2, hist, exact);
@@ -311,6 +290,8 @@
     int maxr = g.dim[0] > g.dim[1] ? g.dim[0] : g.dim[1];
     if (g.dim[2] > maxr) maxr = g.dim[2];
     bool truncated = false;
+    WaveHighStats hs;
+    hs.reset();
     auto gather_block = [&](int r, double tau) -> int {
         const int xa = c[0] - r < 0 ? 0 : c[0] - r, xb = c[0] + r >= g.dim[0] ? g.dim[0] - 1 : c[0] + r;
         const int ya = c[1] - r < 0 ? 0 : c[1] - r, yb = c[1] + r >= g.dim[1] ? g.dim[1] - 1 : c[1] + r;
@@ -318,6 +299,7 @@
         const int ny = yb - ya + 1, ncols = (xb - xa + 1) * ny;
         int m = 0;
         truncated = false;
+        hs.reset();
         for (int c0 = 0; c0 < ncols && !truncated; c0 += 64) {
             const int nruns = ncols - c0 < 64 ? ncols - c0 : 64;
             uint32_t s0 = 0;
@@ -328,8 +310,8 @@
                 s0 = cell_start[col + za];
                 len = (int)(cell_start[col + zb + 1] - s0);
             }
-            const int incl = wave_incl_scan(len);
-            const int mc = __shfl(incl, 63, 64);
+            const int incl = wave_incl_scan_i32(len);
+            const int mc = wave_bcast(incl, 63);
             if (mc == 0) continue;
             sc.run_s0[lane] = s0;
             sc.run_off[lane] = incl - len;
@@ -353,6 +335,7 @@
                 const unsigned long long km = __builtin_amdgcn_ballot_w64(keep);
                 const int pos = m + __builtin_popcountll(km & ((1ull << lane) - 1ull));
                 if (keep && pos < sc.cap) {
+                    hs.add(d);
                     sc.vals[pos] = d;
                     if (POS) sc.pos[pos] = sp;
                 }
@@ -380,13 +363,13 @@
         }
         const int kk = m < k ? m : k;
         unsigned long long lo = 0ull;
-        if (m > k) lo = wave_kth_pattern(sc.vals, m, kk, sc.hist);
+        if (m > k) lo = wave_kth_pattern(sc.vals, m, kk, sc.hist, hs);
         else if (m > 0) {
             for (int t = lane; t < m; t += 64) {
                 const unsigned long long p = (unsigned long long)__double_as_longlong(sc.vals[t]);
                 lo = p > lo ? p : lo;
             }
-            lo = wave_all_max_u64(lo);
+            lo = wave_max_u64(lo);
         }
         double top = 0.0;
         int cnt = 0;
@@ -396,8 +379,7 @@
             if (le) top = fmax(top, sc.vals[t]);
             cnt += __builtin_popcountll(__builtin_amdgcn_ballot_w64(le));
         }
-#pragma unroll
-        for (int o = 32; o > 0; o >>= 1) top = fmax(top, __shfl_xor(top, o, 64));
+        top = wave_max_f64(top);
         if (!truncated && (whole || top < cov2)) {
             out.m = m; out.kk = kk; out.cnt = cnt; out.thr = lo; out.top = top;
             return true;
@@ -433,9 +415,7 @@
                 const int32_t oi = sidx[sc.pos[t]];
                 if (oi > last && oi < cand) cand = oi;
             }
-#pragma unroll
-        for (int o = 32; o > 0; o >>= 1) { const int32_t t2 = __shfl_xor(cand, o, 64); cand = t2 < cand ? t2 : cand; }
-        last = cand;
+        last = (int32_t)wave_min_u32((unsigned)cand);
     }
     return last;
 }
diff --git a/kinectpy_amd/csrc/kpx_knn.hip b/kinectpy_amd/csrc/kpx_knn.hip
--- a/kinectpy_amd/csrc/kpx_knn.hip
+++ b/kinectpy_amd/csrc/kpx_knn.hip
@@ -204,13 +204,29 @@
     __device__ void wave(const WaveKnnScratch &sc, const WaveKnnResult &res, int64_t s, const float *) const
     {
         const int lane = threadIdx.x & 63;
+        int32_t *list = sc.run_off;
+        int listed = 0;
+        auto roots = [&](int n) {
+            wave_lds_fence();
+            if (lane < n) { const int t = list[lane]; sc.vals[t] = -sqrt(sc.vals[t]); }
+            wave_lds_fence();
+        };
+        for (int t0 = 0; t0 < res.m; t0 += 64) {
+            const int t = t0 + lane;
+            const bool sel = t < res.m && (unsigned long long)__double_as_longlong(sc.vals[t]) <= res.thr;
+            const unsigned long long bm = __builtin_amdgcn_ballot_w64(sel);
+            const int n = __builtin_popcountll(bm);
+            if (listed + n > 64) { roots(listed); listed = 0; }
+            if (sel) list[listed + (int)__builtin_amdgcn_mbcnt_hi((unsigned)(bm >> 32), __builtin_amdgcn_mbcnt_lo((unsigned)bm, 0u))] = t;
+            listed += n;
+        }
+        roots(listed);
         double sum = 0.0;
         for (int t = lane; t < res.m; t += 64) {
-            const double d = sc.vals[t];
-            if ((unsigned long long)__double_as_longlong(d) <= res.thr) sum += sqrt(d);
-        }
-#pragma unroll
-        for (int o = 32; o > 0; o >>= 1) sum += __shfl_xor(sum, o, 64);
+            const double v = sc.vals[t];
+            if (__double_as_longlong(v) < 0) sum += -v;
+        }
+        sum = wave_sum_down_f64(sum);
         const double total = sum - (double)(res.cnt - res.kk) * sqrt(res.top);
         if (lane == 0) avg[sidx ? (int64_t)sidx[s] : s - q0] = res.kk > 0 ? total / (double)res.kk : -1.0;
     }
@@ -222,40 +238,9 @@
     }
 };
 
-__device__ __forceinline__ int dppi(int v, int ctrl_sel)
-{
-    switch (ctrl_sel) {
-    case 1: return __builtin_amdgcn_update_dpp(v, v, 0x121, 0xF, 0xF, false);
-    case 2: return __builtin_amdgcn_update_dpp(v, v, 0x122, 0xF, 0xF, false);
-    case 4: return __builtin_amdgcn_update_dpp(v, v, 0x124, 0xF, 0xF, false);
-    default: return __builtin_amdgcn_update_dpp(v, v, 0x128, 0xF, 0xF, false);
-    }
-}
-__device__ __forceinline__ int wave_sum_i(int v)
-{
-    v += dppi(v, 1); v += dppi(v, 2); v += dppi(v, 4); v += dppi(v, 8);
-    v += __shfl_xor(v, 16, 64);
-    v += __shfl_xor(v, 32, 64);
-    return v;
-}
-__device__ __forceinline__ unsigned wave_min_u(unsigned v)
-{
-    unsigned o;
-    o = (unsigned)dppi((int)v, 1); v = o < v ? o : v; o = (unsigned)dppi((int)v, 2); v = o < v ? o : v;
-    o = (unsigned)dppi((int)v, 4); v = o < v ? o : v; o = (unsigned)dppi((int)v, 8); v = o < v ? o : v;
-    o = (unsigned)__shfl_xor((int)v, 16, 64); v = o < v ? o : v;
-    o = (unsigned)__shfl_xor((int)v, 32, 64); v = o < v ? o : v;
-    return v;
-}
-__device__ __forceinline__ unsigned wave_max_u(unsigned v)
-{
-    unsigned o;
-    o = (unsigned)dppi((int)v, 1); v = o > v ? o : v; o = (unsigned)dppi((int)v, 2); v = o > v ? o : v;
-    o = (unsigned)dppi((int)v, 4); v = o > v ? o : v; o = (unsigned)dppi((int)v, 8); v = o > v ? o : v;
-    o = (unsigned)__shfl_xor((int)v, 16, 64); v = o > v ? o : v;
-    o = (unsigned)__shfl_xor((int)v, 32, 64); v = o > v ? o : v;
-    return v;
-}
+__device__ __forceinline__ int wave_sum_i(int v) { return wave_sum_i32(v); }
+__device__ __forceinline__ unsigned wave_min_u(unsigned v) { return wave_min_u32(v); }
+__device__ __forceinline__ unsigned wave_max_u(unsigned v) { return wave_max_u32(v); }
 constexpr int kSorBuckets = 256;
 constexpr int kSorTieRoom = 32;
 constexpr int kBlkQueries = 64, kBlkWaves = 4;
@@ -318,7 +303,7 @@
                             ln = (int)(cell_start[col + zb + 1] - s0);
                         }
                     }
-                    const int incl = wave_incl_scan(ln);
+                    const int incl = wave_incl_scan_i32(ln);
                     if (lane < 32) { run_s0[lane] = s0; run_off[lane] = lane < nruns ? incl - ln : INT_MAX; }
                     if (lane == 63) s_m = incl;
                 }
@@ -395,7 +380,7 @@
                                 const uint4 t4 = hz[0];
                                 const int hv[BPL] = { (int)t4.x, (int)t4.y, (int)t4.z, (int)t4.w };
                                 const int lsum = hv[0] + hv[1] + hv[2] + hv[3];
-                                const int incl = wave_incl_scan(lsum), excl = incl - lsum;
+                                const int incl = wave_incl_scan_i32(lsum), excl = incl - lsum;
                                 const bool mine = need_k > excl && need_k <= incl;
                                 int B = -1, cb = 0, hb = 0;
                                 if (mine) {
@@ -408,7 +393,7 @@
                                 }
                                 const unsigned long long bm = __builtin_amdgcn_ballot_w64(mine);
                                 const int owner = bm ? __builtin_ctzll(bm) : 0;
-                                B = __shfl(B, owner, 64); cb = __shfl(cb, owner, 64); hb = __shfl(hb, owner, 64);
+                                B = wave_bcast(B, owner); cb = wave_bcast(cb, owner); hb = wave_bcast(hb, owner);
                                 const unsigned wend = a + range, bstart = a + ((unsigned)(B < 0 ? 0 : B) << shift), bspan = (1u << shift) - 1u;
                                 const unsigned bend = wend - bstart < bspan ? wend : bstart + bspan;
                                 if (B < 0) { ok = false; run = false; }
@@ -464,8 +449,7 @@
                             wave_lds_fence();
                             double acc = 0.0;
                             for (int t = lane; t < n_le; t += 64) acc += sqrt(selbuf[t]);
-#pragma unroll
-                            for (int o = 32; o > 0; o >>= 1) acc += __shfl_down(acc, o, 64);
+                            acc = wave_sum_down_f64(acc);
                             if (lane == 0) {
                                 const double top = __longlong_as_double((long long)(((unsigned long long)P << 32) | Q));
                                 const double total = n_le > kk ? acc - (double)(n_le - kk) * sqrt(top) : acc;
@@ -485,7 +469,7 @@
             if (fm != 0ull) {
                 int fb_base = 0;
                 if (lane == 0) fb_base = atomicAdd(fb_count, __builtin_popcountll(fm));
-                fb_base = __shfl(fb_base, 0, 64);
+                fb_base = wave_bcast(fb_base, 0);
                 if (fb) fb_list[fb_base + __builtin_popcountll(fm & ((1ull << lane) - 1ull))] = (int32_t)(base + lane);
             }
         }
@@ -715,10 +699,7 @@
                 c[3] += x * x; c[4] += x * y; c[5] += x * z; c[6] += y * y; c[7] += y * z; c[8] += z * z;
             }
         }
-#pragma unroll
-        for (int a9 = 0; a9 < 9; ++a9)
-#pragma unroll
-            for (int o = 32; o > 0; o >>= 1) c[a9] += __shfl_xor(c[a9], o, 64);
+        wave_sum_down_f64x9(c);
         if (lane == 0) {
             double *o = covbuf + 10 * s;
 #pragma unroll
diff --git a/kinectpy_amd/csrc/kpx_voxel.hip b/kinectpy_amd/csrc/kpx_voxel.hip
--- a/kinectpy_amd/csrc/kpx_voxel.hip
+++ b/kinectpy_amd/csrc/kpx_voxel.hip
@@ -81,28 +81,28 @@
         bits[a] = n;
     }
 }
-__device__ __forceinline__ unsigned long long voxel_hcode(unsigned long long x, unsigned long long y, unsigned long long z, int bits)
-{
-    unsigned long long X[3] = { x, y, z };
-    const unsigned long long M = 1ull << (bits - 1);
-    for (unsigned long long Q = M; Q > 1ull; Q >>= 1) {
-        const unsigned long long P = Q - 1ull;
+template <class Word> __device__ __forceinline__ Word voxel_hcode(Word x, Word y, Word z, int bits)
+{
+    Word X[3] = { x, y, z };
+    const Word M = (Word)1 << (bits - 1);
+    for (Word Q = M; Q > (Word)1; Q >>= 1) {
+        const Word P = Q - (Word)1;
 #pragma unroll
         for (int i = 0; i < 3; ++i) {
             if (X[i] & Q) X[0] ^= P;
-            else { const unsigned long long t = (X[0] ^ X[i]) & P; X[0] ^= t; X[i] ^= t; }
+            else { const Word t = (X[0] ^ X[i]) & P; X[0] ^= t; X[i] ^= t; }
         }
     }
     X[1] ^= X[0];
     X[2] ^= X[1];
-    unsigned long long t = 0ull;
-    for (unsigned long long Q = M; Q > 1ull; Q >>= 1)
-        if (X[2] & Q) t ^= Q - 1ull;
+    Word t = 0;
+    for (Word Q = M; Q > (Word)1; Q >>= 1)
+        if (X[2] & Q) t ^= Q - (Word)1;
     X[0] ^= t; X[1] ^= t; X[2] ^= t;
-    unsigned long long k = 0ull;
+    Word k = 0;
     for (int b = bits - 1; b >= 0; --b) {
 #pragma unroll
-        for (int i = 0; i < 3; ++i) k = (k << 1) | ((X[i] >> b) & 1ull);
+        for (int i = 0; i < 3; ++i) k = (k << 1) | ((X[i] >> b) & (Word)1);
     }
     return k;
 }
@@ -126,12 +126,12 @@
     for (int a = 0; a < 3; ++a) n += ab[a] > m ? ab[a] - m : 0;
     return n;
 }
-__device__ __forceinline__ unsigned long long voxel_hilbert_key(unsigned long long x, unsigned long long y, unsigned long long z, const int ab[3], int m)
-{
-    const unsigned long long mask = (1ull << m) - 1ull;
+template <class Word> __device__ __forceinline__ Word voxel_hilbert_key(Word x, Word y, Word z, const int ab[3], int m)
+{
+    const Word mask = ((Word)1 << m) - (Word)1;
     const int ey = ab[1] > m ? ab[1] - m : 0, ez = ab[2] > m ? ab[2] - m : 0;
-    const unsigned long long hi = (((x >> m) << ey | (y >> m)) << ez) | (z >> m);
-    return (hi << (3 * m)) | voxel_hcode(x & mask, y & mask, z & mask, m);
+    const Word hi = (((x >> m) << ey | (y >> m)) << ez) | (z >> m);
+    return (hi << (3 * m)) | voxel_hcode<Word>(x & mask, y & mask, z & mask, m);
 }
 __device__ __forceinline__ void voxel_batch_dims(const VoxelBatch &b, const double *__restrict__ bbox, double voxel, double d[3], int *overflow)
 {
@@ -174,13 +174,15 @@
     struct Grid {
         uint64_t DX, DY, DZ;
         int overflow, morton, ab[3], m;
+        int kb;
+        int narrow;
     };
     Key *keys;
     int32_t *err, *bits_out;
     __device__ __forceinline__ Grid grid(const VoxelBatch &b, const double *__restrict__ bbox, double voxel) const
     {
         __shared__ double dims[3];
-        __shared__ int overflow, axis_bits[3], cube_bits;
+        __shared__ int overflow, axis_bits[3], cube_bits, key_bits, narrow;
         if (threadIdx.x == 0) {
             double d[3];
             int ov;
@@ -192,18 +194,28 @@
             axis_bits[0] = ab[0]; axis_bits[1] = ab[1]; axis_bits[2] = ab[2];
             while ((1 << cb) < b.count) ++cb;
             cube_bits = voxel_hilbert_cube_bits(ab, cb);
-            overflow = (ov || (b.morton && voxel_hilbert_key_bits(ab, cube_bits) + cb > 64)) ? 1 : 0;
+            key_bits = voxel_hilbert_key_bits(ab, cube_bits);
+            overflow = (ov || (b.morton && key_bits + cb > 64)) ? 1 : 0;
+            if (b.morton) narrow = (!overflow && key_bits + cb <= 32 && key_bits <= 31) ? 1 : 0;
+            else narrow = (!ov && ((double)b.count * d[0]) * (d[1] * d[2]) < 4294967296.0) ? 1 : 0;
         }
         __syncthreads();
-        return Grid{ (uint64_t)dims[0], (uint64_t)dims[1], (uint64_t)dims[2], overflow, b.morton, { axis_bits[0], axis_bits[1], axis_bits[2] }, cube_bits };
+        return Grid{ (uint64_t)dims[0], (uint64_t)dims[1], (uint64_t)dims[2], overflow, b.morton, { axis_bits[0], axis_bits[1], axis_bits[2] }, cube_bits,
+                     key_bits, narrow };
     }
     __device__ __forceinline__ void put(const Grid &g, const double *__restrict__ bbox, double voxel, int64_t i, int c, const double q[3]) const
     {
         double f[3];
         const bool bad = voxel_cell(q, bbox + 8 * c, voxel, f) || g.overflow;
         if (bad) { err[c] = 1; f[0] = f[1] = f[2] = 0.0; }
-        if (g.morton)
-            keys[i] = (Key)(((uint64_t)c << voxel_hilbert_key_bits(g.ab, g.m)) | voxel_hilbert_key((uint64_t)f[0], (uint64_t)f[1], (uint64_t)f[2], g.ab, g.m));
+        if constexpr (sizeof(Key) == 4) {
+            if (g.narrow) {
+                if (g.morton) keys[i] = ((uint32_t)c << g.kb) | voxel_hilbert_key<uint32_t>((uint32_t)f[0], (uint32_t)f[1], (uint32_t)f[2], g.ab, g.m);
+                else keys[i] = (((uint32_t)c * (uint32_t)g.DX + (uint32_t)f[0]) * (uint32_t)g.DY + (uint32_t)f[1]) * (uint32_t)g.DZ + (uint32_t)f[2];
+                return;
+            }
+        }
+        if (g.morton) keys[i] = (Key)(((uint64_t)c << g.kb) | voxel_hilbert_key<uint64_t>((uint64_t)f[0], (uint64_t)f[1], (uint64_t)f[2], g.ab, g.m));
         else keys[i] = (Key)((((uint64_t)c * g.DX + (uint64_t)f[0]) * g.DY + (uint64_t)f[1]) * g.DZ + (uint64_t)f[2]);
     }
 };
diff --git a/kinectpy_amd/csrc/kpx_wave.h b/kinectpy_amd/csrc/kpx_wave.h
--- /dev/null
+++ b/kinectpy_amd/csrc/kpx_wave.h
@@ -0,0 +1,204 @@
+#pragma once
+#include <hip/hip_runtime.h>
+#include <stdint.h>
+
+#if defined(__HIP_DEVICE_COMPILE__) && defined(__gfx950__)
+#if __has_builtin(__builtin_amdgcn_permlane16_swap) && __has_builtin(__builtin_amdgcn_permlane32_swap) && __has_builtin(__builtin_amdgcn_update_dpp)
+#define KPX_WAVE_VALU 1
+#endif
+#endif
+#ifndef KPX_WAVE_VALU
+#define KPX_WAVE_VALU 0
+#endif
+
+namespace kpx {
+
+constexpr int kDppRowShl = 0x100, kDppRowShr = 0x110, kDppRowRor = 0x120, kDppRowBcast15 = 0x142, kDppRowBcast31 = 0x143;
+
+#if KPX_WAVE_VALU
+template <int CTRL, int ROW_MASK = 0xF, int BANK_MASK = 0xF> __device__ __forceinline__ unsigned wave_dpp_u32(unsigned old, unsigned v)
+{
+    return (unsigned)__builtin_amdgcn_update_dpp((int)old, (int)v, CTRL, ROW_MASK, BANK_MASK, false);
+}
+template <int CTRL> __device__ __forceinline__ double wave_dpp_f64(double v)
+{
+    const unsigned long long p = (unsigned long long)__double_as_longlong(v);
+    const unsigned lo = wave_dpp_u32<CTRL>((unsigned)p, (unsigned)p), hi = wave_dpp_u32<CTRL>((unsigned)(p >> 32), (unsigned)(p >> 32));
+    return __longlong_as_double((long long)(((unsigned long long)hi << 32) | lo));
+}
+__device__ __forceinline__ void wave_swap16_u32(unsigned v, unsigned &r0, unsigned &r1)
+{
+    const auto r = __builtin_amdgcn_permlane16_swap(v, v, false, false);
+    r0 = r[0]; r1 = r[1];
+}
+__device__ __forceinline__ void wave_swap32_u32(unsigned v, unsigned &r0, unsigned &r1)
+{
+    const auto r = __builtin_amdgcn_permlane32_swap(v, v, false, false);
+    r0 = r[0]; r1 = r[1];
+}
+__device__ __forceinline__ void wave_swap16_f64(double v, double &a, double &b)
+{
+    const unsigned long long p = (unsigned long long)__double_as_longlong(v);
+    unsigned l0, l1, h0, h1;
+    wave_swap16_u32((unsigned)p, l0, l1); wave_swap16_u32((unsigned)(p >> 32), h0, h1);
+    a = __longlong_as_double((long long)(((unsigned long long)h0 << 32) | l0));
+    b = __longlong_as_double((long long)(((unsigned long long)h1 << 32) | l1));
+}
+__device__ __forceinline__ void wave_swap32_f64(double v, double &a, double &b)
+{
+    const unsigned long long p = (unsigned long long)__double_as_longlong(v);
+    unsigned l0, l1, h0, h1;
+    wave_swap32_u32((unsigned)p, l0, l1); wave_swap32_u32((unsigned)(p >> 32), h0, h1);
+    a = __longlong_as_double((long long)(((unsigned long long)h0 << 32) | l0));
+    b = __longlong_as_double((long long)(((unsigned long long)h1 << 32) | l1));
+}
+#endif
+
+template <class Op> __device__ __forceinline__ unsigned wave_reduce_u32(unsigned v, Op op)
+{
+#if KPX_WAVE_VALU
+    v = op(v, wave_dpp_u32<kDppRowRor + 1>(v, v)); v = op(v, wave_dpp_u32<kDppRowRor + 2>(v, v));
+    v = op(v, wave_dpp_u32<kDppRowRor + 4>(v, v)); v = op(v, wave_dpp_u32<kDppRowRor + 8>(v, v));
+    unsigned a, b;
+    wave_swap16_u32(v, a, b); v = op(a, b);
+    wave_swap32_u32(v, a, b); v = op(a, b);
+    return (unsigned)__builtin_amdgcn_readfirstlane((int)v);
+#else
+#pragma unroll
+    for (int o = 32; o > 0; o >>= 1) v = op(v, (unsigned)__shfl_xor((int)v, o, 64));
+    return v;
+#endif
+}
+__device__ __forceinline__ int wave_sum_i32(int v)
+{
+    return (int)wave_reduce_u32((unsigned)v, [](unsigned a, unsigned b) { return a + b; });
+}
+__device__ __forceinline__ unsigned wave_min_u32(unsigned v)
+{
+    return wave_reduce_u32(v, [](unsigned a, unsigned b) { return a < b ? a : b; });
+}
+__device__ __forceinline__ unsigned wave_max_u32(unsigned v)
+{
+    return wave_reduce_u32(v, [](unsigned a, unsigned b) { return a > b ? a : b; });
+}
+__device__ __forceinline__ unsigned long long wave_max_u64(unsigned long long v)
+{
+    const unsigned hi = wave_max_u32((unsigned)(v >> 32));
+    const unsigned lo = wave_max_u32((unsigned)(v >> 32) == hi ? (unsigned)v : 0u);
+    return ((unsigned long long)hi << 32) | lo;
+}
+__device__ __forceinline__ double wave_max_f64(double v)
+{
+#if KPX_WAVE_VALU
+    v = fmax(v, wave_dpp_f64<kDppRowRor + 1>(v)); v = fmax(v, wave_dpp_f64<kDppRowRor + 2>(v));
+    v = fmax(v, wave_dpp_f64<kDppRowRor + 4>(v)); v = fmax(v, wave_dpp_f64<kDppRowRor + 8>(v));
+    double a, b;
+    wave_swap16_f64(v, a, b); v = fmax(a, b);
+    wave_swap32_f64(v, a, b); v = fmax(a, b);
+    const unsigned long long p = (unsigned long long)__double_as_longlong(v);
+    const unsigned lo = (unsigned)__builtin_amdgcn_readfirstlane((int)(unsigned)p), hi = (unsigned)__builtin_amdgcn_readfirstlane((int)(unsigned)(p >> 32));
+    return __longlong_as_double((long long)(((unsigned long long)hi << 32) | lo));
+#else
+#pragma unroll
+    for (int o = 32; o > 0; o >>= 1) v = fmax(v, __shfl_xor(v, o, 64));
+    return v;
+#endif
+}
+
+__device__ __forceinline__ int wave_incl_scan_i32(int v)
+{
+#if KPX_WAVE_VALU
+    unsigned t = (unsigned)v;
+    t += wave_dpp_u32<kDppRowShr + 1>(0u, (unsigned)v) + wave_dpp_u32<kDppRowShr + 2>(0u, (unsigned)v) + wave_dpp_u32<kDppRowShr + 3>(0u, (unsigned)v);
+    t += wave_dpp_u32<kDppRowShr + 4, 0xF, 0xE>(0u, t);
+    t += wave_dpp_u32<kDppRowShr + 8, 0xF, 0xC>(0u, t);
+    t += wave_dpp_u32<kDppRowBcast15, 0xA>(0u, t);
+    t += wave_dpp_u32<kDppRowBcast31, 0xC>(0u, t);
+    return (int)t;
+#else
+    const int l = threadIdx.x & 63;
+#pragma unroll
+    for (int o = 1; o < 64; o <<= 1) { const int t = __shfl_up(v, o, 64); if (l >= o) v += t; }
+    return v;
+#endif
+}
+
+__device__ __forceinline__ int wave_bcast(int v, int uniform_lane)
+{
+#if KPX_WAVE_VALU
+    return __builtin_amdgcn_readlane(v, uniform_lane);
+#else
+    return __shfl(v, uniform_lane, 64);
+#endif
+}
+__device__ __forceinline__ unsigned wave_bcast(unsigned v, int uniform_lane) { return (unsigned)wave_bcast((int)v, uniform_lane); }
+
+__device__ __forceinline__ double wave_sum_down_f64(double v)
+{
+#if KPX_WAVE_VALU
+    double a, b;
+    wave_swap32_f64(v, a, b); v = a + b;
+    wave_swap16_f64(v, a, b); v = a + b;
+    v += wave_dpp_f64<kDppRowShl + 8>(v); v += wave_dpp_f64<kDppRowShl + 4>(v);
+    v += wave_dpp_f64<kDppRowShl + 2>(v); v += wave_dpp_f64<kDppRowShl + 1>(v);
+    return v;
+#else
+#pragma unroll
+    for (int o = 32; o > 0; o >>= 1) v += __shfl_down(v, o, 64);
+    return v;
+#endif
+}
+__device__ __forceinline__ float wave_sum_down_f32(float v)
+{
+#if KPX_WAVE_VALU
+    unsigned a, b;
+    wave_swap32_u32(__float_as_uint(v), a, b); v = __uint_as_float(a) + __uint_as_float(b);
+    wave_swap16_u32(__float_as_uint(v), a, b); v = __uint_as_float(a) + __uint_as_float(b);
+    v += __uint_as_float(wave_dpp_u32<kDppRowShl + 8>(__float_as_uint(v), __float_as_uint(v)));
+    v += __uint_as_float(wave_dpp_u32<kDppRowShl + 4>(__float_as_uint(v), __float_as_uint(v)));
+    v += __uint_as_float(wave_dpp_u32<kDppRowShl + 2>(__float_as_uint(v), __float_as_uint(v)));
+    v += __uint_as_float(wave_dpp_u32<kDppRowShl + 1>(__float_as_uint(v), __float_as_uint(v)));
+    return v;
+#else
+#pragma unroll
+    for (int o = 32; o > 0; o >>= 1) v += __shfl_down(v, o, 64);
+    return v;
+#endif
+}
+
+__device__ __forceinline__ void wave_sum_down_f64x9(double c[9])
+{
+#if KPX_WAVE_VALU
+    auto pair32 = [](double p, double q) {
+        const unsigned long long pp = (unsigned long long)__double_as_longlong(p), qq = (unsigned long long)__double_as_longlong(q);
+        const auto l = __builtin_amdgcn_permlane32_swap((unsigned)pp, (unsigned)qq, false, false);
+        const auto h = __builtin_amdgcn_permlane32_swap((unsigned)(pp >> 32), (unsigned)(qq >> 32), false, false);
+        return __longlong_as_double((long long)(((unsigned long long)h[0] << 32) | l[0])) + __longlong_as_double((long long)(((unsigned long long)h[1] << 32) | l[1]));
+    };
+    auto pair16 = [](double p, double q) {
+        const unsigned long long pp = (unsigned long long)__double_as_longlong(p), qq = (unsigned long long)__double_as_longlong(q);
+        const auto l = __builtin_amdgcn_permlane16_swap((unsigned)pp, (unsigned)qq, false, false);
+        const auto h = __builtin_amdgcn_permlane16_swap((unsigned)(pp >> 32), (unsigned)(qq >> 32), false, false);
+        return __longlong_as_double((long long)(((unsigned long long)h[0] << 32) | l[0])) + __longlong_as_double((long long)(((unsigned long long)h[1] << 32) | l[1]));
+    };
+    const double r0 = pair32(c[0], c[5]), r1 = pair32(c[1], c[6]), r2 = pair32(c[2], c[7]), r3 = pair32(c[3], c[8]), r4 = pair32(c[4], c[4]);
+    double t0 = pair16(r0, r1), t1 = pair16(r2, r3), t2 = pair16(r4, r4);
+    t0 += wave_dpp_f64<kDppRowShl + 8>(t0); t1 += wave_dpp_f64<kDppRowShl + 8>(t1); t2 += wave_dpp_f64<kDppRowShl + 8>(t2);
+    t0 += wave_dpp_f64<kDppRowShl + 4>(t0); t1 += wave_dpp_f64<kDppRowShl + 4>(t1); t2 += wave_dpp_f64<kDppRowShl + 4>(t2);
+    t0 += wave_dpp_f64<kDppRowShl + 2>(t0); t1 += wave_dpp_f64<kDppRowShl + 2>(t1); t2 += wave_dpp_f64<kDppRowShl + 2>(t2);
+    t0 += wave_dpp_f64<kDppRowShl + 1>(t0); t1 += wave_dpp_f64<kDppRowShl + 1>(t1); t2 += wave_dpp_f64<kDppRowShl + 1>(t2);
+    auto from = [](double v, int lane) {
+        const unsigned long long p = (unsigned long long)__double_as_longlong(v);
+        const unsigned lo = (unsigned)__builtin_amdgcn_readlane((int)(unsigned)p, lane), hi = (unsigned)__builtin_amdgcn_readlane((int)(unsigned)(p >> 32), lane);
+        return __longlong_as_double((long long)(((unsigned long long)hi << 32) | lo));
+    };
+    c[0] = t0; c[1] = from(t0, 16); c[5] = from(t0, 32); c[6] = from(t0, 48);
+    c[2] = t1; c[3] = from(t1, 16); c[7] = from(t1, 32); c[8] = from(t1, 48);
+    c[4] = t2;
+#else
+#pragma unroll
+    for (int q = 0; q < 9; ++q) c[q] = wave_sum_down_f64(c[q]);
+#endif
+}
+
+}
diff --git a/kinectpy_amd/csrc/kpx_wave.hip b/kinectpy_amd/csrc/kpx_wave.hip
--- /dev/null
+++ b/kinectpy_amd/csrc/kpx_wave.hip
@@ -0,0 +1,54 @@
+#include "kpx_common.h"
+
+namespace kpx {
+
+__global__ __launch_bounds__(256) void wave_selftest_kernel(int kind, const unsigned long long *__restrict__ in, int64_t rows,
+                                                            unsigned long long *__restrict__ out)
+{
+    const int wave = threadIdx.x >> 6, lane = threadIdx.x & 63;
+    if (kind == KPX_WAVE_SUM_DOWN_F64X9) {
+        for (int64_t g = wave; 9 * g + 9 <= rows; g += 4) {
+            double c[9];
+#pragma unroll
+            for (int q = 0; q < 9; ++q) c[q] = __longlong_as_double((long long)in[(9 * g + q) * 64 + lane]);
+            wave_sum_down_f64x9(c);
+#pragma unroll
+            for (int q = 0; q < 9; ++q) out[(9 * g + q) * 64 + lane] = lane == 0 ? (unsigned long long)__double_as_longlong(c[q]) : 0ull;
+        }
+        return;
+    }
+    for (int64_t r = wave; r < rows; r += 4) {
+        const unsigned long long v = in[r * 64 + lane];
+        unsigned long long o = 0ull;
+        switch (kind) {
+        case KPX_WAVE_SUM_I32: o = (unsigned)wave_sum_i32((int)(unsigned)v); break;
+        case KPX_WAVE_MIN_U32: o = wave_min_u32((unsigned)v); break;
+        case KPX_WAVE_MAX_U32: o = wave_max_u32((unsigned)v); break;
+        case KPX_WAVE_MAX_U64: o = wave_max_u64(v); break;
+        case KPX_WAVE_MAX_F64: o = (unsigned long long)__double_as_longlong(wave_max_f64(__longlong_as_double((long long)v))); break;
+        case KPX_WAVE_INCL_SCAN_I32: o = (unsigned)wave_incl_scan_i32((int)(unsigned)v); break;
+        case KPX_WAVE_BCAST: o = wave_bcast((unsigned)v, (int)(r & 63)); break;
+        case KPX_WAVE_SUM_DOWN_F64: o = (unsigned long long)__double_as_longlong(wave_sum_down_f64(__longlong_as_double((long long)v))); break;
+        case KPX_WAVE_SUM_DOWN_F32: o = __float_as_uint(wave_sum_down_f32(__uint_as_float((unsigned)v))); break;
+        default: break;
+        }
+        out[r * 64 + lane] = o;
+    }
+}
+
+}
+
+using namespace kpx;
+
+KPX_EXPORT int kpx_wave_selftest(int32_t kind, const uint64_t *in, int64_t rows, uint64_t *out, void *stream)
+{
+    KPX_REQUIRE(kind >= KPX_WAVE_SUM_I32 && kind <= KPX_WAVE_SUM_DOWN_F64X9, "kpx_wave_selftest: unknown kind %d", kind);
+    KPX_REQUIRE(rows >= 0 && rows <= 65536, "kpx_wave_selftest: rows must be in [0, 65536]");
+    KPX_REQUIRE(kind != KPX_WAVE_SUM_DOWN_F64X9 || rows % 9 == 0, "kpx_wave_selftest: the nine-sum form takes groups of nine rows");
+    if (rows == 0) return KPX_OK;
+    KPX_REQUIRE(in && out, "kpx_wave_selftest: null pointer");
+    hipLaunchKernelGGL(wave_selftest_kernel, dim3(1), dim3(256), 0, (hipStream_t)stream, (int)kind, (const unsigned long long *)in, rows,
+                       (unsigned long long *)out);
+    KPX_LAUNCH_CHECK();
+    return KPX_OK;
+}
```
